# jpe17/TwoTowerMLRetrieval

Hardware: AMD Instinct MI355X
Metric: queries/sec top-k over 10M x 256-d docs (higher is better)
Workload: dtype f32 results (bit-identical to the fp32 FMA chain); f16-MFMA screen + fp32 rescoring; 1 GPU; exact cosine top-10 of B=1024 queries over 10000000 x 256 fp32 unit-norm passages resident in HBM (BASELINE configs[3]; configs[1] batch), row-sharded over 1 GPU(s), screened path (f16-MFMA filter + exact fp32 rescoring, bit-identical to the fp32 kernel); n_docs=10000000, dim=256, batch=1024, k=10, parallelism=rowshard1

## Files before the change

### include/tt.h

```cpp
#ifndef TT_H
#define TT_H

#include <stddef.h>
#include <stdint.h>

#ifdef __cplusplus
extern "C" {
#endif

typedef void *tt_stream_t;

#define TT_TOPK_INVALID_INDEX (1ll << 62)

enum tt_status {
    TT_OK = 0,
    TT_ERR_BAD_SHAPE = 1,
    TT_ERR_BAD_INDEX = 2,
    TT_ERR_ZERO_LENGTH = 3,
    TT_ERR_UNSUPPORTED = 4,
    TT_ERR_WORKSPACE = 5,
    TT_ERR_HIP = 6
};

const char *tt_version(void);
const char *tt_last_error(void);

int tt_event_create(void **ev);
int tt_event_destroy(void *ev);
int tt_event_elapsed_ms(void *start, void *stop, float *ms);


size_t tt_score_topk_redo_flags_offset(int B, int64_t N, int d, int k);
size_t tt_score_topk_pace_timeouts_offset(int B, int64_t N, int d, int k);
size_t tt_score_topk_workspace_bytes(int B, int64_t N, int d, int k);
int tt_score_topk_f32(const float *Q, int B, int d, const float *D, int64_t N, int k,
                      int64_t idx_offset, float *out_val, int64_t *out_idx, void *workspace,
                      size_t workspace_bytes, tt_stream_t stream);

size_t tt_score_topk_bf16_workspace_bytes(int B, int64_t N, int d, int k);
int tt_score_topk_bf16(const float *Q, int B, int d, const void *D_bf16, int64_t N, int k,
                       int64_t idx_offset, float *out_val, int64_t *out_idx, void *workspace,
                       size_t workspace_bytes, tt_stream_t stream);

#define TT_TOPK_LARGE_KMAX 1024
size_t tt_score_topk_large_workspace_bytes(int B, int64_t N, int d, int k, int bf16);
size_t tt_score_topk_large_tier_offset(int B, int64_t N, int d, int k, int bf16);
int tt_score_topk_large_f32(const float *Q, int B, int d, const float *D, int64_t N, int k,
                            int64_t idx_offset, float *out_val, int64_t *out_idx, void *workspace,
                            size_t workspace_bytes, tt_stream_t stream);
int tt_score_topk_large_bf16(const float *Q, int B, int d, const void *D_bf16, int64_t N, int k,
                             int64_t idx_offset, float *out_val, int64_t *out_idx, void *workspace,
                             size_t workspace_bytes, tt_stream_t stream);

size_t tt_score_topk_masked_workspace_bytes(int B, int64_t N, int d, int k, int bf16);
int tt_score_topk_masked_f32(const float *Q, int B, int d, const float *D, int64_t N, const uint32_t *keep, int k,
                             int64_t idx_offset, float *out_val, int64_t *out_idx, void *workspace,
                             size_t workspace_bytes, tt_stream_t stream);
int tt_score_topk_masked_bf16(const float *Q, int B, int d, const void *D_bf16, int64_t N, const uint32_t *keep, int k,
                              int64_t idx_offset, float *out_val, int64_t *out_idx, void *workspace,
                              size_t workspace_bytes, tt_stream_t stream);
int tt_keep_mask_pack(const uint8_t *keep_bool, int64_t N, uint32_t *keep, tt_stream_t stream);
int tt_keep_mask_clear_ids(uint32_t *keep, int64_t N, const int64_t *ids, int64_t n_ids, int64_t idx_offset,
                           tt_stream_t stream);

size_t tt_score_topk_tagged_workspace_bytes(int B, int64_t N, int d, int k, int bf16);
int tt_score_topk_tagged_f32(const float *Q, int B, int d, const float *D, int64_t N, const uint32_t *tags,
                             const uint32_t *match_mask, const uint32_t *match_value, const uint32_t *keep, int k,
                             int64_t idx_offset, float *out_val, int64_t *out_idx, void *workspace, size_t workspace_bytes,
                             tt_stream_t stream);
int tt_score_topk_tagged_bf16(const float *Q, int B, int d, const void *D_bf16, int64_t N, const uint32_t *tags,
                              const uint32_t *match_mask, const uint32_t *match_value, const uint32_t *keep, int k,
                              int64_t idx_offset, float *out_val, int64_t *out_idx, void *workspace, size_t workspace_bytes,
                              tt_stream_t stream);

size_t tt_score_topk_biased_workspace_bytes(int B, int64_t N, int d, int k, int bf16);
int tt_score_topk_biased_f32(const float *Q, int B, int d, const float *D, int64_t N, const float *bias, const uint32_t *keep,
                             int k, int64_t idx_offset, float *out_val, int64_t *out_idx, void *workspace,
                             size_t workspace_bytes, tt_stream_t stream);
int tt_score_topk_biased_bf16(const float *Q, int B, int d, const void *D_bf16, int64_t N, const float *bias,
                              const uint32_t *keep, int k, int64_t idx_offset, float *out_val, int64_t *out_idx, void *workspace,
                              size_t workspace_bytes, tt_stream_t stream);

size_t tt_score_topk_after_workspace_bytes(int B, int64_t N, int d, int k, int bf16);
int tt_score_topk_after_f32(const float *Q, int B, int d, const float *D, int64_t N, const float *after_val,
                            const int64_t *after_idx, const uint32_t *keep, int k, int64_t idx_offset, float *out_val,
                            int64_t *out_idx, void *workspace, size_t workspace_bytes, tt_stream_t stream);
int tt_score_topk_after_bf16(const float *Q, int B, int d, const void *D_bf16, int64_t N, const float *after_val,
                             const int64_t *after_idx, const uint32_t *keep, int k, int64_t idx_offset, float *out_val,
                             int64_t *out_idx, void *workspace, size_t workspace_bytes, tt_stream_t stream);
int tt_after_local_bound(int64_t after_idx, int64_t idx_offset, int N);

size_t tt_score_topk_screened_bf16_workspace_bytes(int B, int64_t N, int d, int k);
int tt_index_stats_bf16(const void *D_bf16, int64_t N, int d, float *stats, int reset_stats, tt_stream_t stream);
int tt_score_topk_screened_bf16(const float *Q, int B, int d, const void *D_bf16, int64_t N, int k, float dmax_norm,
                                int64_t idx_offset, float *out_val, int64_t *out_idx, int32_t *fallback_flag,
                                void *workspace, size_t workspace_bytes, void *const *prof_events, tt_stream_t stream);
int tt_score_topk_screened_seed_list_bf16(const float *Q, int B, int d, const void *D_bf16, int64_t N, int k, int k_seed,
                                          float dmax_norm, int32_t *fallback_flag, float *seed_list, void *workspace,
                                          size_t workspace_bytes, tt_stream_t stream);
int tt_score_topk_screened_seeded_bf16(const float *Q, int B, int d, const void *D_bf16, int64_t N, int k, float dmax_norm,
                                       int64_t idx_offset, float *out_val, int64_t *out_idx, int32_t *fallback_flag,
                                       const float *seed, void *workspace, size_t workspace_bytes,
                                       void *const *prof_events, tt_stream_t stream);

int tt_score_topk_partials_f32(const float *Q, int B, int d, const float *D, int64_t N, int k,
                               int64_t idx_offset, void *workspace, size_t workspace_bytes,
                               const float **part_val , const int64_t **part_idx ,
                               int *part_m , void *const *prof_events ,
                               tt_stream_t stream);

int tt_index_build_f16(const float *D, int64_t N, int d, void *D16, float *stats, tt_stream_t stream);
int tt_index_build_from_bf16(const void *D_bf16, int64_t N, int d, float *D32, void *D16, float *stats,
                             int reset_stats, tt_stream_t stream);
size_t tt_score_topk_screened_workspace_bytes(int B, int64_t N, int d, int k);
size_t tt_score_topk_screened_stats_offset(int B, int64_t N, int d, int k);
int tt_score_topk_screened_f32(const float *Q, int B, int d, const float *D32, const void *D16, int64_t N, int k,
                               float dmax_norm, int64_t idx_offset, float *out_val, int64_t *out_idx,
                               int32_t *fallback_flag, void *workspace, size_t workspace_bytes,
                               void *const *prof_events , tt_stream_t stream);

int tt_score_topk_screened_seed_f32(const float *Q, int B, int d, const void *D16, int64_t N, int k, int k_seed, float dmax_norm,
                                    int32_t *fallback_flag, float *seed , void *workspace, size_t workspace_bytes,
                                    tt_stream_t stream);
int tt_score_topk_screened_seed_list_f32(const float *Q, int B, int d, const void *D16, int64_t N, int k, int k_seed,
                                         float dmax_norm, int32_t *fallback_flag, float *seed_list ,
                                         void *workspace, size_t workspace_bytes, tt_stream_t stream);
int tt_seed_union_f32(const float *lists , int world, int B, int list_len, int kth,
                      float *seed , tt_stream_t stream);
int tt_score_topk_screened_seeded_f32(const float *Q, int B, int d, const float *D32, const void *D16, int64_t N, int k,
                                      float dmax_norm, int64_t idx_offset, float *out_val, int64_t *out_idx,
                                      int32_t *fallback_flag, const float *seed , void *workspace, size_t workspace_bytes,
                                      void *const *prof_events , tt_stream_t stream);

size_t tt_score_topk_screened_masked_workspace_bytes(int B, int64_t N, int d, int k, int bf16);
int tt_score_topk_screened_masked_f32(const float *Q, int B, int d, const float *D32, const void *D16, int64_t N,
                                      const uint32_t *keep, int k, float dmax_norm, int64_t idx_offset, float *out_val,
                                      int64_t *out_idx, int32_t *fallback_flag, void *workspace, size_t workspace_bytes,
                                      void *const *prof_events , tt_stream_t stream);
int tt_score_topk_screened_masked_bf16(const float *Q, int B, int d, const void *D_bf16, int64_t N, const uint32_t *keep,
                                       int k, float dmax_norm, int64_t idx_offset, float *out_val, int64_t *out_idx,
                                       int32_t *fallback_flag, void *workspace, size_t workspace_bytes,
                                       void *const *prof_events , tt_stream_t stream);
int tt_score_topk_screened_seed_list_masked_f32(const float *Q, int B, int d, const void *D16, int64_t N, const uint32_t *keep,
                                                int k, int k_seed, float dmax_norm, int32_t *fallback_flag,
                                                float *seed_list , void *workspace, size_t workspace_bytes,
                                                tt_stream_t stream);
int tt_score_topk_screened_seed_list_masked_bf16(const float *Q, int B, int d, const void *D_bf16, int64_t N,
                                                 const uint32_t *keep, int k, int k_seed, float dmax_norm,
                                                 int32_t *fallback_flag, float *seed_list , void *workspace,
                                                 size_t workspace_bytes, tt_stream_t stream);
int tt_score_topk_screened_seeded_masked_f32(const float *Q, int B, int d, const float *D32, const void *D16, int64_t N,
                                             const uint32_t *keep, int k, float dmax_norm, int64_t idx_offset, float *out_val,
                                             int64_t *out_idx, int32_t *fallback_flag, const float *seed ,
                                             void *workspace, size_t workspace_bytes,
                                             void *const *prof_events , tt_stream_t stream);
int tt_score_topk_screened_seeded_masked_bf16(const float *Q, int B, int d, const void *D_bf16, int64_t N,
                                              const uint32_t *keep, int k, float dmax_norm, int64_t idx_offset, float *out_val,
                                              int64_t *out_idx, int32_t *fallback_flag, const float *seed ,
                                              void *workspace, size_t workspace_bytes,
                                              void *const *prof_events , tt_stream_t stream);

int tt_topk_merge(const float *in_val, const int64_t *in_idx, int B, int M, int k, float *out_val,
                  int64_t *out_idx, tt_stream_t stream);

int tt_topk_merge_shards(const void *gathered, int world, size_t rank_stride, size_t idx_byte_offset,
                         int B, int kp, int k, float *out_val, int64_t *out_idx, tt_stream_t stream);

int tt_topk_merge_large(const float *in_val, const int64_t *in_idx, int B, int M, int k,
                        float *out_val, int64_t *out_idx, tt_stream_t stream);
int tt_topk_merge_shards_large(const void *gathered, int world, size_t rank_stride, size_t idx_byte_offset,
                               int B, int kp, int k, float *out_val, int64_t *out_idx, tt_stream_t stream);

int tt_topk_exclude_ids(const float *in_val, const int64_t *in_idx, int B, int M, const int64_t *exclude , int E,
                        int k, float *out_val, int64_t *out_idx, tt_stream_t stream);

int tt_topk_collapse_table(const float *in_val, const int64_t *in_idx, int B, int M, const int64_t *groups , int64_t N,
                           int64_t idx_offset, int max_per_group, int k, float *out_val, int64_t *out_idx, int64_t *out_gid,
                           int32_t *out_info , tt_stream_t stream);
int tt_topk_collapse_gids(const float *in_val, const int64_t *in_idx, const int64_t *in_gid , int B, int M,
                          int max_per_group, int k, float *out_val, int64_t *out_idx, int64_t *out_gid,
                          int32_t *out_info , tt_stream_t stream);

size_t tt_score_count_workspace_bytes(int B, int64_t N, int d, int bf16);
int tt_score_count_f32(const float *Q, int B, int d, const float *D, int64_t N, const uint32_t *keep,
                       const float *min_score, int64_t *count, int accumulate, void *workspace, size_t workspace_bytes,
                       tt_stream_t stream);
int tt_score_count_bf16(const float *Q, int B, int d, const void *D_bf16, int64_t N, const uint32_t *keep,
                        const float *min_score, int64_t *count, int accumulate, void *workspace, size_t workspace_bytes,
                        tt_stream_t stream);
int tt_topk_cut_below(float *val, int64_t *idx, int B, int k, const float *min_score, tt_stream_t stream);

int tt_score_rank_f32(const float *Q, int B, int d, const float *D, int64_t N, const int64_t *target,
                      int64_t *rank, tt_stream_t stream);

int tt_score_all_f32(const float *Q, int B, int d, const float *D, int64_t N, float *S, tt_stream_t stream);

int tt_score_ids_f32(const float *Q, int B, int d, const float *D, int64_t N, const uint32_t *keep ,
                     const int64_t *ids , int C, int64_t idx_offset, float *out_val ,
                     int64_t *out_idx , tt_stream_t stream);
int tt_score_ids_bf16(const float *Q, int B, int d, const void *D_bf16, int64_t N, const uint32_t *keep ,
                      const int64_t *ids , int C, int64_t idx_offset, float *out_val ,
                      int64_t *out_idx , tt_stream_t stream);

int tt_mmr_select_f32(const float *in_val , const int64_t *in_idx , int B, int C, const float *D, int64_t N,
                      int d, int64_t idx_offset, float lambda, int k, float *out_val , int64_t *out_idx ,
                      int32_t *out_pos , tt_stream_t stream);
int tt_mmr_select_bf16(const float *in_val , const int64_t *in_idx , int B, int C, const void *D_bf16,
                       int64_t N, int d, int64_t idx_offset, float lambda, int k, float *out_val ,
                       int64_t *out_idx , int32_t *out_pos , tt_stream_t stream);
int tt_mmr_select_rows_f32(const float *in_val , const int64_t *in_idx , int B, int C,
                           const float *rows , int d, float lambda, int k, float *out_val ,
                           int64_t *out_idx , int32_t *out_pos , tt_stream_t stream);

#define TT_LEXICAL_FMAX 20480
int tt_lexical_chunk_docs(void);
size_t tt_lexical_workspace_bytes(int B, int64_t N, int k);
int tt_lexical_score_topk_f32(const int64_t *indptr, const int32_t *cols, const float *vals, int64_t N, int F,
                              const int64_t *q_indptr, const int32_t *q_cols, const float *q_vals, int B,
                              const uint32_t *keep , const float *min_score ,
                              const float *base , int64_t base_stride, float w_base,
                              float w_lex, int k, int64_t idx_offset, float *out_val, int64_t *out_idx, void *workspace,
                              size_t workspace_bytes, tt_stream_t stream);
int tt_lexical_score_all_f32(const int64_t *indptr, const int32_t *cols, const float *vals, int64_t N, int F,
                             const int64_t *q_indptr, const int32_t *q_cols, const float *q_vals, int B, float *S ,
                             tt_stream_t stream);


typedef struct tt_enc_sync {
    void *wait_before_recurrence;
    void *record_after_recurrence;
} tt_enc_sync_t;

#define TT_ENC_TRAIN_MASK 0xff
#define TT_ENC_ONE_WORKGROUP 0x100
#define TT_ENC_PHASE_BEGIN 0x200
#define TT_ENC_PHASE_FINISH 0x400
#define TT_ENC_SEED_ON_DEVICE 0x800
#define TT_ENC_F32 0x1000
int tt_encoder_split_workgroups(int B, int H, int bidirectional, int rnn_type);
size_t tt_encoder_workspace_bytes(int B, int T, int E, int H, int num_layers, int bidirectional, int rnn_type,
                                  int train ,
                                  int dropout );
int tt_encoder_forward_f32(const int64_t *ids, int B, int T, const float *table, int64_t V, int E, int H,
                           int num_layers, int bidirectional, int rnn_type, const float *const *weights ,
                           const float *proj_w, const float *proj_b, int normalize, int train, float dropout_p,
                           uint64_t dropout_seed, float *out, void *workspace, size_t workspace_bytes,
                           int32_t *status, const tt_enc_sync_t *sync , tt_stream_t stream);

size_t tt_encoder_prepared_bytes(int E, int H, int num_layers, int bidirectional, int rnn_type);
int tt_encoder_prepare_f32(int E, int H, int num_layers, int bidirectional, int rnn_type,
                           const float *const *weights , void *prepared, size_t prepared_bytes,
                           tt_stream_t stream);
int tt_encoder_forward_prepared_f32(const int64_t *ids, int B, int T, const float *table, int64_t V, int E, int H,
                                    int num_layers, int bidirectional, int rnn_type,
                                    const float *const *weights , const void *prepared,
                                    const float *proj_w, const float *proj_b, int normalize, int opts, float *out,
                                    void *workspace, size_t workspace_bytes, int32_t *status, tt_stream_t stream);

#define TT_ENC_PROJECTED 0x2000
size_t tt_encoder_projected_bytes(int64_t V, int E, int H, int bidirectional, int rnn_type);
int tt_encoder_project_table_f32(const float *table, int64_t V, int E, int H, int num_layers, int bidirectional, int rnn_type,
                                 const float *const *weights , const void *prepared, void *projected,
                                 size_t projected_bytes, tt_stream_t stream);
int tt_encoder_forward_projected_f32(const int64_t *ids, int B, int T, const void *projected, int64_t V, int E, int H,
                                     int num_layers, int bidirectional, int rnn_type, const float *const *weights ,
                                     const void *prepared, const float *proj_w, const float *proj_b, int normalize, int opts,
                                     float *out, void *workspace, size_t workspace_bytes, int32_t *status, tt_stream_t stream);

int tt_concat_ids_i64(const int64_t *a, int Ba, int Ta, const int64_t *b, int Bb, int Tb, int64_t *out, int T,
                      tt_stream_t stream);

int tt_encoder_backward_f32(const int64_t *ids, int B, int T, const float *table, int64_t V, int E, int H,
// ... 82 lines not shown
```

### include/tt_debug.h

```cpp
#ifndef TT_DEBUG_H
#define TT_DEBUG_H

#include "tt.h"

#ifdef __cplusplus
extern "C" {
#endif

size_t tt_debug_screen_s16_workspace_bytes(int B, int64_t N, int form);
int tt_debug_screen_s16(const float *Q, int B, const void *D16, int64_t N, float dmax_norm, const float *thr, int form,
                        float *out_t, void *workspace, size_t workspace_bytes, tt_stream_t stream);

int tt_debug_screen_s16_bf16(const float *Q, int B, const void *D_bf16, int64_t N, float dmax_norm, const float *thr, int form,
                             float *out_t, void *workspace, size_t workspace_bytes, tt_stream_t stream);

#ifdef __cplusplus
}
#endif
#endif
```

### twotowermlretrieval_amd/_lib.py

```python
from __future__ import annotations

import ctypes as C
from pathlib import Path

_PKG = Path(__file__).resolve().parent
LIB_PATH = _PKG / "libtt.so"

TT_OK, TT_ERR_BAD_SHAPE, TT_ERR_BAD_INDEX, TT_ERR_ZERO_LENGTH, TT_ERR_UNSUPPORTED, TT_ERR_WORKSPACE, TT_ERR_HIP = range(7)
TT_ENC_ONE_WORKGROUP = 0x100
TT_ENC_PHASE_BEGIN, TT_ENC_PHASE_FINISH = 0x200, 0x400
TT_ENC_SEED_ON_DEVICE = 0x800
TT_ENC_F32 = 0x1000
TT_ENC_PROJECTED = 0x2000
TT_STEP_GATE_WORDS = 4


class EncSync(C.Structure):
    _fields_ = [("wait_before_recurrence", C.c_void_p), ("record_after_recurrence", C.c_void_p)]
TT_TOPK_INVALID_INDEX = 1 << 62


class TTError(RuntimeError):
    def __init__(self, code: int, msg: str):
        super().__init__(f"libtt error {code}: {msg}")
        self.code = code


_vp, _i, _i64, _sz, _f, _u64 = C.c_void_p, C.c_int, C.c_int64, C.c_size_t, C.c_float, C.c_uint64

SIGNATURES = {
    "tt_version": (C.c_char_p, []),
    "tt_last_error": (C.c_char_p, []),
    "tt_score_topk_workspace_bytes": (_sz, [_i, _i64, _i, _i]),
    "tt_score_topk_pace_timeouts_offset": (_sz, [_i, _i64, _i, _i]),
    "tt_score_topk_redo_flags_offset": (_sz, [_i, _i64, _i, _i]),
    "tt_score_topk_f32": (_i, [_vp, _i, _i, _vp, _i64, _i, _i64, _vp, _vp, _vp, _sz, _vp]),
    "tt_score_topk_bf16_workspace_bytes": (_sz, [_i, _i64, _i, _i]),
    "tt_score_topk_bf16": (_i, [_vp, _i, _i, _vp, _i64, _i, _i64, _vp, _vp, _vp, _sz, _vp]),
    "tt_score_topk_large_workspace_bytes": (_sz, [_i, _i64, _i, _i, _i]),
    "tt_score_topk_large_tier_offset": (_sz, [_i, _i64, _i, _i, _i]),
    "tt_score_topk_large_f32": (_i, [_vp, _i, _i, _vp, _i64, _i, _i64, _vp, _vp, _vp, _sz, _vp]),
    "tt_score_topk_large_bf16": (_i, [_vp, _i, _i, _vp, _i64, _i, _i64, _vp, _vp, _vp, _sz, _vp]),
    "tt_score_topk_masked_workspace_bytes": (_sz, [_i, _i64, _i, _i, _i]),
    "tt_score_topk_masked_f32": (_i, [_vp, _i, _i, _vp, _i64, _vp, _i, _i64, _vp, _vp, _vp, _sz, _vp]),
    "tt_score_topk_masked_bf16": (_i, [_vp, _i, _i, _vp, _i64, _vp, _i, _i64, _vp, _vp, _vp, _sz, _vp]),
    "tt_keep_mask_pack": (_i, [_vp, _i64, _vp, _vp]),
    "tt_keep_mask_clear_ids": (_i, [_vp, _i64, _vp, _i64, _i64, _vp]),
    "tt_score_topk_tagged_workspace_bytes": (_sz, [_i, _i64, _i, _i, _i]),
    "tt_score_topk_tagged_f32": (_i, [_vp, _i, _i, _vp, _i64, _vp, _vp, _vp, _vp, _i, _i64, _vp, _vp, _vp, _sz, _vp]),
    "tt_score_topk_tagged_bf16": (_i, [_vp, _i, _i, _vp, _i64, _vp, _vp, _vp, _vp, _i, _i64, _vp, _vp, _vp, _sz, _vp]),
    "tt_score_topk_biased_workspace_bytes": (_sz, [_i, _i64, _i, _i, _i]),
    "tt_score_topk_biased_f32": (_i, [_vp, _i, _i, _vp, _i64, _vp, _vp, _i, _i64, _vp, _vp, _vp, _sz, _vp]),
    "tt_score_topk_biased_bf16": (_i, [_vp, _i, _i, _vp, _i64, _vp, _vp, _i, _i64, _vp, _vp, _vp, _sz, _vp]),
    "tt_score_topk_after_workspace_bytes": (_sz, [_i, _i64, _i, _i, _i]),
    "tt_score_topk_after_f32": (_i, [_vp, _i, _i, _vp, _i64, _vp, _vp, _vp, _i, _i64, _vp, _vp, _vp, _sz, _vp]),
    "tt_score_topk_after_bf16": (_i, [_vp, _i, _i, _vp, _i64, _vp, _vp, _vp, _i, _i64, _vp, _vp, _vp, _sz, _vp]),
    "tt_after_local_bound": (_i, [_i64, _i64, _i]),
    "tt_score_topk_screened_bf16_workspace_bytes": (_sz, [_i, _i64, _i, _i]),
    "tt_index_stats_bf16": (_i, [_vp, _i64, _i, _vp, _i, _vp]),
    "tt_score_topk_screened_bf16": (_i, [_vp, _i, _i, _vp, _i64, _i, _f, _i64, _vp, _vp, _vp, _vp, _sz, _vp, _vp]),
    "tt_score_topk_screened_seed_list_bf16": (_i, [_vp, _i, _i, _vp, _i64, _i, _i, _f, _vp, _vp, _vp, _sz, _vp]),
    "tt_score_topk_screened_seeded_bf16": (_i, [_vp, _i, _i, _vp, _i64, _i, _f, _i64, _vp, _vp, _vp, _vp, _vp, _sz, _vp, _vp]),
    "tt_score_topk_partials_f32": (_i, [_vp, _i, _i, _vp, _i64, _i, _i64, _vp, _sz, _vp, _vp, _vp, _vp, _vp]),
    "tt_index_build_f16": (_i, [_vp, _i64, _i, _vp, _vp, _vp]),
    "tt_index_build_from_bf16": (_i, [_vp, _i64, _i, _vp, _vp, _vp, _i, _vp]),
    "tt_score_topk_screened_workspace_bytes": (_sz, [_i, _i64, _i, _i]),
    "tt_score_topk_screened_stats_offset": (_sz, [_i, _i64, _i, _i]),
    "tt_score_topk_screened_seed_f32": (_i, [_vp, _i, _i, _vp, _i64, _i, _i, _f, _vp, _vp, _vp, _sz, _vp]),
    "tt_score_topk_screened_seed_list_f32": (_i, [_vp, _i, _i, _vp, _i64, _i, _i, _f, _vp, _vp, _vp, _sz, _vp]),
    "tt_seed_union_f32": (_i, [_vp, _i, _i, _i, _i, _vp, _vp]),
    "tt_score_topk_screened_seeded_f32": (_i, [_vp, _i, _i, _vp, _vp, _i64, _i, _f, _i64, _vp, _vp, _vp, _vp, _vp, _sz, _vp, _vp]),
    "tt_score_topk_screened_f32": (_i, [_vp, _i, _i, _vp, _vp, _i64, _i, _f, _i64, _vp, _vp, _vp, _vp, _sz, _vp, _vp]),
    "tt_score_topk_screened_masked_workspace_bytes": (_sz, [_i, _i64, _i, _i, _i]),
    "tt_score_topk_screened_masked_f32": (_i, [_vp, _i, _i, _vp, _vp, _i64, _vp, _i, _f, _i64, _vp, _vp, _vp, _vp, _sz, _vp, _vp]),
    "tt_score_topk_screened_masked_bf16": (_i, [_vp, _i, _i, _vp, _i64, _vp, _i, _f, _i64, _vp, _vp, _vp, _vp, _sz, _vp, _vp]),
    "tt_score_topk_screened_seed_list_masked_f32": (_i, [_vp, _i, _i, _vp, _i64, _vp, _i, _i, _f, _vp, _vp, _vp, _sz, _vp]),
    "tt_score_topk_screened_seed_list_masked_bf16": (_i, [_vp, _i, _i, _vp, _i64, _vp, _i, _i, _f, _vp, _vp, _vp, _sz, _vp]),
    "tt_score_topk_screened_seeded_masked_f32": (_i, [_vp, _i, _i, _vp, _vp, _i64, _vp, _i, _f, _i64, _vp, _vp, _vp, _vp, _vp, _sz, _vp, _vp]),
    "tt_score_topk_screened_seeded_masked_bf16": (_i, [_vp, _i, _i, _vp, _i64, _vp, _i, _f, _i64, _vp, _vp, _vp, _vp, _vp, _sz, _vp, _vp]),
    "tt_event_create": (_i, [_vp]),
    "tt_event_destroy": (_i, [_vp]),
    "tt_event_elapsed_ms": (_i, [_vp, _vp, _vp]),
    "tt_topk_merge": (_i, [_vp, _vp, _i, _i, _i, _vp, _vp, _vp]),
    "tt_topk_merge_shards": (_i, [_vp, _i, _sz, _sz, _i, _i, _i, _vp, _vp, _vp]),
    "tt_topk_merge_large": (_i, [_vp, _vp, _i, _i, _i, _vp, _vp, _vp]),
    "tt_topk_merge_shards_large": (_i, [_vp, _i, _sz, _sz, _i, _i, _i, _vp, _vp, _vp]),
    "tt_topk_exclude_ids": (_i, [_vp, _vp, _i, _i, _vp, _i, _i, _vp, _vp, _vp]),
    "tt_topk_collapse_table": (_i, [_vp, _vp, _i, _i, _vp, _i64, _i64, _i, _i, _vp, _vp, _vp, _vp, _vp]),
    "tt_topk_collapse_gids": (_i, [_vp, _vp, _vp, _i, _i, _i, _i, _vp, _vp, _vp, _vp, _vp]),
    "tt_score_count_workspace_bytes": (_sz, [_i, _i64, _i, _i]),
    "tt_score_count_f32": (_i, [_vp, _i, _i, _vp, _i64, _vp, _vp, _vp, _i, _vp, _sz, _vp]),
    "tt_score_count_bf16": (_i, [_vp, _i, _i, _vp, _i64, _vp, _vp, _vp, _i, _vp, _sz, _vp]),
    "tt_topk_cut_below": (_i, [_vp, _vp, _i, _i, _vp, _vp]),
    "tt_score_rank_f32": (_i, [_vp, _i, _i, _vp, _i64, _vp, _vp, _vp]),
    "tt_score_all_f32": (_i, [_vp, _i, _i, _vp, _i64, _vp, _vp]),
    "tt_score_ids_f32": (_i, [_vp, _i, _i, _vp, _i64, _vp, _vp, _i, _i64, _vp, _vp, _vp]),
    "tt_score_ids_bf16": (_i, [_vp, _i, _i, _vp, _i64, _vp, _vp, _i, _i64, _vp, _vp, _vp]),
    "tt_mmr_select_f32": (_i, [_vp, _vp, _i, _i, _vp, _i64, _i, _i64, _f, _i, _vp, _vp, _vp, _vp]),
    "tt_mmr_select_bf16": (_i, [_vp, _vp, _i, _i, _vp, _i64, _i, _i64, _f, _i, _vp, _vp, _vp, _vp]),
    "tt_mmr_select_rows_f32": (_i, [_vp, _vp, _i, _i, _vp, _i, _f, _i, _vp, _vp, _vp, _vp]),
    "tt_lexical_chunk_docs": (_i, []),
    "tt_lexical_workspace_bytes": (_sz, [_i, _i64, _i]),
    "tt_lexical_score_topk_f32": (_i, [_vp, _vp, _vp, _i64, _i, _vp, _vp, _vp, _i, _vp, _vp, _vp, _i64, _f, _f, _i, _i64,
                                       _vp, _vp, _vp, _sz, _vp]),
    "tt_lexical_score_all_f32": (_i, [_vp, _vp, _vp, _i64, _i, _vp, _vp, _vp, _i, _vp, _vp]),
    "tt_tok_create": (_i, [_vp, _vp, _vp, _i64, _i64, _vp]),
    "tt_tok_destroy": (None, [_vp]),
    "tt_tok_encode": (_i, [_vp, _vp, _vp, _i64, _vp, _vp, _vp, _i]),
    "tt_tok_encode_sep": (_i, [_vp, _vp, _i64, C.c_char, _i64, _vp, _vp, _vp, _vp, _i]),
    "tt_tok_encode_ptrs": (_i, [_vp, _vp, _vp, _i64, _vp, _vp, _vp, _vp, _i]),
    "tt_tok_set_unicode": (_i, [_vp, _vp, _vp, _i64]),
    "tt_tok_encode_units": (_i, [_vp, _vp, _vp, _vp, _i64, _vp, _vp, _vp, _vp, _i]),
    "tt_tok_pad": (_i, [_vp, _vp, _vp, _i64, _i64, _vp, _i]),
    "tt_tok_pad_i32": (_i, [_vp, _vp, _vp, _i64, _i64, _vp, _i]),
    "tt_encoder_split_workgroups": (_i, [_i, _i, _i, _i]),
    "tt_encoder_workspace_bytes": (_sz, [_i, _i, _i, _i, _i, _i, _i, _i, _i]),
    "tt_encoder_forward_f32": (_i, [_vp, _i, _i, _vp, _i64, _i, _i, _i, _i, _i, _vp, _vp, _vp, _i, _i, _f, _u64, _vp, _vp,
                                    _sz, _vp, _vp, _vp]),
    "tt_concat_ids_i64": (_i, [_vp, _i, _i, _vp, _i, _i, _vp, _i, _vp]),
    "tt_encoder_prepared_bytes": (_sz, [_i, _i, _i, _i, _i]),
    "tt_encoder_prepare_f32": (_i, [_i, _i, _i, _i, _i, _vp, _vp, _sz, _vp]),
    "tt_encoder_forward_prepared_f32": (_i, [_vp, _i, _i, _vp, _i64, _i, _i, _i, _i, _i, _vp, _vp, _vp, _vp, _i, _i, _vp, _vp,
                                             _sz, _vp, _vp]),
    "tt_encoder_projected_bytes": (_sz, [_i64, _i, _i, _i, _i]),
    "tt_encoder_project_table_f32": (_i, [_vp, _i64, _i, _i, _i, _i, _i, _vp, _vp, _vp, _sz, _vp]),
    "tt_encoder_forward_projected_f32": (_i, [_vp, _i, _i, _vp, _i64, _i, _i, _i, _i, _i, _vp, _vp, _vp, _vp, _i, _i, _vp, _vp,
                                              _sz, _vp, _vp]),
    "tt_encoder_backward_f32": (_i, [_vp, _i, _i, _vp, _i64, _i, _i, _i, _i, _i, _vp, _vp, _vp, _i, _f, _u64, _vp, _vp,
                                     _vp, _vp, _vp, _vp, _sz, _i, _vp, _vp, _vp]),
    "tt_triplet_loss_f32": (_i, [_vp, _vp, _vp, _i, _i, _f, _vp, _vp, _vp, _vp, _vp, _vp]),
    "tt_in_batch_loss_workspace_bytes": (_sz, [_i, _i]),
    "tt_in_batch_loss_f32": (_i, [_vp, _vp, _vp, _i, _i, _f, _vp, _vp, _vp, _vp, _vp, _sz, _vp]),
    "tt_contrastive_loss_workspace_bytes": (_sz, [_i, _i, _i]),
    "tt_contrastive_loss_f32": (_i, [_vp, _i, _vp, _i, _i, _i, _f, _vp, _vp, _vp, _vp, _sz, _vp]),
    "tt_contrastive_loss_grouped_f32": (_i, [_vp, _i, _vp, _i, _i, _i, _vp, _vp, _f, _vp, _vp, _vp, _vp, _sz, _vp]),
    "tt_contrastive_loss_soft_workspace_bytes": (_sz, [_i, _i, _i]),
    "tt_contrastive_loss_soft_f32": (_i, [_vp, _i, _vp, _i, _i, _vp, _f, _vp, _vp, _vp, _vp, _sz, _vp]),
    "tt_contrastive_loss_sym_workspace_bytes": (_sz, [_i, _i, _i]),
    "tt_contrastive_loss_sym_f32": (_i, [_vp, _i, _vp, _i, _i, _i, _vp, _vp, _f, _f, _vp, _vp, _vp, _vp, _vp, _sz, _vp]),
    "tt_allgather_topk":(_i, [_vp, _vp, _vp, _sz, _vp]),
    "tt_allreduce_grads": (_i, [_vp, _vp, _i64, _vp]),
    "tt_comm_library": (C.c_char_p, []),
    "tt_comm_unique_id": (_i, [_vp]),
    "tt_comm_init_rank": (_i, [_vp, _i, _vp, _i]),
    "tt_comm_info": (_i, [_vp, _vp, _vp]),
    "tt_comm_destroy": (_i, [_vp]),
    "tt_clip_adam_scratch_bytes": (_sz, []),
    "tt_clip_adam_step_f32": (_i, [_vp, _vp, _vp, _vp, _i64, _i64, _f, _f, _f, _f, _f, _f, _vp, _vp, _vp]),
    "tt_clip_adam_step_gated_f32": (_i, [_vp, _vp, _vp, _vp, _i64, _vp, _f, _f, _f, _f, _f, _f, _vp, _vp, _vp, _vp]),
    "tt_step_gate_f32": (_i, [_vp, _i, _vp, _vp]),
}

_lib = None


def lib() -> C.CDLL:
    global _lib
    if _lib is None:
        if not LIB_PATH.exists():
            raise ImportError(
                f"{LIB_PATH} is missing: build it with `python -m twotowermlretrieval_amd.build` "
                "(hipcc, gfx950).  There is no CPU or PyTorch fallback for this path.")
        l = C.CDLL(str(LIB_PATH))
        for name, (res, args) in SIGNATURES.items():
            fn = getattr(l, name)
            fn.restype = res
            fn.argtypes = args
        _lib = l
    return _lib


def check(rc: int) -> None:
    if rc != TT_OK:
        msg = lib().tt_last_error().decode("utf-8", "replace")
        if rc == TT_ERR_BAD_INDEX:
            raise IndexError(msg)
        if rc == TT_ERR_BAD_SHAPE:
            raise ValueError(msg)
        raise TTError(rc, msg)
```

### twotowermlretrieval_amd/csrc/screen.hip

```cpp
#include "score_topk.h"
#include "keep_word.h"
#include <cmath>

#include <hip/hip_fp16.h>
#include <limits.h>
#include <math.h>

namespace {

typedef _Float16 h8 __attribute__((ext_vector_type(8)));
typedef _Float16 h4 __attribute__((ext_vector_type(4)));
typedef unsigned u32x4 __attribute__((ext_vector_type(4)));
typedef __attribute__((address_space(3))) void lds_void;
typedef const __attribute__((address_space(1))) void gbl_void;

#ifndef TT_SCREEN_STAGGER
#define TT_SCREEN_STAGGER 1
#endif
constexpr int SW = 8;
constexpr int STILE_BYTES = 32 * 512;
constexpr int SRING = 8;
constexpr int STPB = 2;
constexpr int SCAP = 128;
constexpr int SURV_MAX = 1024;
constexpr int POOL_MAX = 8192;
constexpr int FIN_MAX_CHUNKS = 2048;
constexpr int STOP = 2;
constexpr int STOP_MIN_CHUNKS = 64;
constexpr int REFRESH_LEVELS = 16;
constexpr int REFRESH_STEP = 2;
constexpr int REFRESH_FIRST_SHIFT = 5;
constexpr int REFRESH_MIN_TILES = 1024;

struct SCand {
    float v;
    int x;
};

__device__ __forceinline__ float screen_eps(float qnorm, float dmax)
{
    return 1.10e-3f * qnorm * dmax + 1e-6f * (qnorm + dmax);
}

template <int NCH>
__device__ __forceinline__ void bf16_to_f16_lds(char *base, int lane)
{
    uint4 v[NCH];
#pragma unroll
    for (int i = 0; i < NCH; ++i)
        v[i] = *(const uint4 *)(base + (i * 64 + lane) * 16);
#pragma unroll
    for (int i = 0; i < NCH; ++i) {
        unsigned w[4] = {v[i].x, v[i].y, v[i].z, v[i].w};
#pragma unroll
        for (int e = 0; e < 4; ++e) {
            const _Float16 lo = (_Float16)__uint_as_float(w[e] << 16);
            const _Float16 hi = (_Float16)__uint_as_float(w[e] & 0xffff0000u);
            w[e] = (unsigned)__builtin_bit_cast(unsigned short, lo) | ((unsigned)__builtin_bit_cast(unsigned short, hi) << 16);
        }
        *(uint4 *)(base + (i * 64 + lane) * 16) = uint4{w[0], w[1], w[2], w[3]};
    }
}

__device__ __forceinline__ SCand scand_load_l2(const SCand *p)
{
    unsigned long long u = __hip_atomic_load((const unsigned long long *)p, __ATOMIC_RELAXED, __HIP_MEMORY_SCOPE_AGENT);
    SCand c;
    c.v = __uint_as_float((unsigned)u);
    c.x = (int)(u >> 32);
    return c;
}

struct ScreenParams {
    const float *Q = nullptr;
    const _Float16 *D16 = nullptr;
    int B = 0, N = 0, k = 0;
    int n_chunks = 0, tiles_per_chunk = 0, n_tiles = 0;
    int static_tiles = 0, tail_g = 1, tail_blocks = 0;
    int *tail_ctr = nullptr;
    unsigned *hist = nullptr;
    float dmax = 0.0f;
    SCand *cand = nullptr;
    int *pcnt = nullptr;
    int *flag = nullptr;
    float *max_val = nullptr;
    float *top_val = nullptr;
    const float *thr0 = nullptr;
    int thr0_stride = 1;
    const h8 *qimg = nullptr;
    const float *qnorm = nullptr;
    const float *dbg_thr = nullptr;
    const unsigned *keep = nullptr;
};

__device__ __forceinline__ void scand_store_async(const SCand *base, unsigned byte_off, float v, int x)
{
    const unsigned long long bits = ((unsigned long long)(unsigned)x << 32) | (unsigned long long)__float_as_uint(v);
    asm volatile("global_store_dwordx2 %0, %1, %2\n\ts_nop 1" ::"v"(byte_off), "v"(bits), "s"(base) : "memory");
}

__device__ __forceinline__ void u32_inc_async(const unsigned *base, unsigned byte_off)
{
    asm volatile("global_atomic_add %0, %1, %2\n\ts_nop 0" ::"v"(byte_off), "v"(1u), "s"(base) : "memory");
}

__device__ __forceinline__ float refresh_edge(int j, float width, float base) { return __fmaf_rn((float)j - 0.25f, width, base); }
__device__ __forceinline__ int refresh_level(float v, float base, float inv_width)
{
    return (int)fminf((v - base) * inv_width, (float)(REFRESH_LEVELS - 1));
}
constexpr float REFRESH_MIN_WIDTH = 1e-30f;

__device__ __forceinline__ void f32_store_async(float *dst, float v)
{
    asm volatile("global_store_dword %0, %1, off\n\ts_nop 0" ::"v"(dst), "v"(v) : "memory");
}

constexpr int SQUART = SCAP / 4;
constexpr int SQ_TRIGGER = SQUART - 10;
constexpr int SQ_KEEP_MAX = 4 * SQ_TRIGGER - 4;

__device__ __forceinline__ void screen_compact(SCand *base, const int (&n)[4], int k, float slack, int lane, int &n_new,
                                               float &thr_new, bool &have, bool &overflow)
{
    float v[2];
    int x[2], rank[2];
    bool live[2];
#pragma unroll
    for (int i = 0; i < 2; ++i) {
        v[i] = -INFINITY;
        x[i] = INT_MAX;
        rank[i] = 0;
        live[i] = (lane & 31) < ((lane >> 5) ? n[2 * i + 1] : n[2 * i]);
        if (live[i]) {
            const SCand c = scand_load_l2(base + 64 * i + lane);
            v[i] = c.v;
            x[i] = c.x;
        }
    }
#pragma unroll
    for (int i2 = 0; i2 < 2; ++i2) {
#pragma unroll
        for (int sub = 0; sub < 2; ++sub) {
            const int lim = n[2 * i2 + sub];
            for (int l2 = 0; l2 < lim; ++l2) {
                const float sv = __builtin_bit_cast(float, __builtin_amdgcn_readlane(__builtin_bit_cast(int, v[i2]), 32 * sub + l2));
                const int sx = __builtin_amdgcn_readlane(x[i2], 32 * sub + l2);
#pragma unroll
                for (int i = 0; i < 2; ++i)
                    rank[i] += (sv > v[i] || (sv == v[i] && sx < x[i])) ? 1 : 0;
            }
        }
    }
    const int total = n[0] + n[1] + n[2] + n[3];
    have = total >= k;
    overflow = false;
    n_new = total;
    thr_new = -INFINITY;
    if (have) {
        float kth = -INFINITY;
#pragma unroll
        for (int i = 0; i < 2; ++i) {
            const unsigned long long bk = __ballot(live[i] && rank[i] == k - 1);
            if (bk)
                kth = __builtin_bit_cast(float, __builtin_amdgcn_readlane(__builtin_bit_cast(int, v[i]), __ffsll((long long)bk) - 1));
        }
        thr_new = kth - slack;
        n_new = 0;
#pragma unroll
        for (int i = 0; i < 2; ++i)
            n_new += __popcll(__ballot(live[i] && v[i] >= thr_new));
        if (n_new > SQ_KEEP_MAX) {
            overflow = true;
            n_new = k;
        }
    }
#pragma unroll
    for (int i = 0; i < 2; ++i)
        if (live[i] && rank[i] < n_new) {
            SCand c;
            c.v = v[i];
            c.x = x[i];
            base[SQUART * (rank[i] & 3) + (rank[i] >> 2)] = c;
        }
}

__global__ __launch_bounds__(128) void q_image_kernel(const float *__restrict__ Q, int B, h8 *__restrict__ img,
                                                      float *__restrict__ qnorm, int *__restrict__ flag, int n_flags,
                                                      int *__restrict__ tail_ctr, int n_ctr, unsigned *__restrict__ hist)
{
    __shared__ int any_bad[2];
    if (blockIdx.x == 0)
        for (int i = threadIdx.x; i < n_ctr; i += 128)
            tail_ctr[i] = 0;
    if (hist)
        for (int i = threadIdx.x; i < 32 * REFRESH_LEVELS; i += 128)
            hist[(size_t)blockIdx.x * (32 * REFRESH_LEVELS) + i] = 0u;
    const int lane = threadIdx.x & 63, wv = threadIdx.x >> 6;
    const int S = blockIdx.x * 2 + wv;
    const int g = lane >> 4, n = lane & 15;
    const int qrow = 16 * S + n;
    const bool live = qrow < B;
    const float *qp = Q + (size_t)min(qrow, B - 1) * 256 + 8 * g;
    float ss = 0.0f;
    bool bad = false;
#pragma unroll
    for (int s = 0; s < 8; ++s) {
        const f32x4 a = *(const f32x4 *)(qp + 32 * s);
        const f32x4 b = *(const f32x4 *)(qp + 32 * s + 4);
        h8 hv;
#pragma unroll
        for (int e = 0; e < 4; ++e) {
            const float x0 = live ? a[e] : 0.0f, x1 = live ? b[e] : 0.0f;
            ss += x0 * x0 + x1 * x1;
            bad |= !(fabsf(x0) <= 60000.0f) || !(fabsf(x1) <= 60000.0f);
            hv[e] = (_Float16)x0;
            hv[4 + e] = (_Float16)x1;
        }
        img[((size_t)S * 8 + s) * 64 + lane] = hv;
    }
    ss += __shfl_xor(ss, 16);
    ss += __shfl_xor(ss, 32);
    if (g == 0)
        qnorm[qrow] = sqrtf(ss);
    const bool wave_bad = __ballot(bad && live) != 0ull;
    if (lane == 0)
        any_bad[wv] = wave_bad ? 1 : 0;
    __syncthreads();
    if (threadIdx.x == 0 && (int)blockIdx.x < n_flags)
        flag[blockIdx.x] = (any_bad[0] | any_bad[1]) ? 2 : 0;
}

template <bool MAXONLY, int NSET, bool BF = false, bool MASKED = false, bool ONCHIP = false>
__global__ __launch_bounds__(SW * 64, 2) void screen_kernel(ScreenParams p)
{
    extern __shared__ __attribute__((aligned(16))) char ring[];
    constexpr int DMA_AUX = NSET < 3 ? 2 : 0;
    const int lane = threadIdx.x & 63;
    const int w = __builtin_amdgcn_readfirstlane(threadIdx.x >> 6);
    const int chunk = blockIdx.x % p.n_chunks;
    const int qgroup = blockIdx.x / p.n_chunks;
    int t0 = chunk * p.tiles_per_chunk;
    int t1 = min(t0 + p.tiles_per_chunk, p.static_tiles);
    __shared__ int next_block;
    const int k = p.k;
    const int g = lane >> 4, n = lane & 15;
    constexpr int QW = 16 * NSET, QB = SW * QW;
    const int qbase = qgroup * QB + w * QW;
    const bool wave_live = qbase < p.B;
    __shared__ float ladder_base[SW * 64];
    const bool refresh = !MAXONLY && p.hist != nullptr;
    const unsigned *const hwave = p.hist + (size_t)qbase * REFRESH_LEVELS;

    h8 qreg[NSET][8];
    float eps2[NSET];
    f32x4 negthr[NSET];
    int cnt[NSET];
#pragma unroll
    for (int c = 0; c < NSET; ++c)
        cnt[c] = 0;
#pragma unroll
    for (int c = 0; c < NSET; ++c) {
        const int qrow = qbase + 16 * c + n;
        const bool live = qrow < p.B;
        float qn = 0.0f;
        if (wave_live) {
            const h8 *src = p.qimg + ((size_t)(qbase / 16 + c) * 8) * 64 + lane;
#pragma unroll
            for (int s = 0; s < 8; ++s)
                qreg[c][s] = src[s * 64];
            qn = p.qnorm[qrow];
        }
        eps2[c] = 2.0f * screen_eps(qn, p.dmax);
        const float floor_thr = -(1.01f * qn * p.dmax + 1e-30f);
        const float t_init = live ? ((!MAXONLY && p.thr0) ? fmaxf(p.thr0[(size_t)qrow * p.thr0_stride + p.thr0_stride - 1] - eps2[c], floor_thr)
                                                    : floor_thr)
                            : INFINITY;
        float c_init = -t_init;
        if (MAXONLY)
            c_init = (p.dbg_thr && live) ? -p.dbg_thr[qrow] : 0.0f;
        negthr[c] = f32x4{c_init, c_init, c_init, c_init};
        if (!MAXONLY && g == 0)
            ladder_base[w * QW + 16 * c + n] = t_init + eps2[c];
    }

    SCand *const cwave = p.cand + ((size_t)blockIdx.x * QB + w * QW) * SCAP;

    auto compact_where = [&](int c, unsigned qmask) {
        asm volatile("s_waitcnt vmcnt(0)" ::: "memory");
        while (qmask) {
            const int q = __ffs((int)qmask) - 1;
            qmask &= qmask - 1;
            const int nq[4] = {__builtin_amdgcn_readlane(cnt[c], q), __builtin_amdgcn_readlane(cnt[c], q + 16),
                               __builtin_amdgcn_readlane(cnt[c], q + 32), __builtin_amdgcn_readlane(cnt[c], q + 48)};
            const float slack = __builtin_bit_cast(float, __builtin_amdgcn_readlane(__builtin_bit_cast(int, eps2[c]), q));
            int n_new;
            float tn;
            bool have, ovf;
            screen_compact(cwave + (size_t)(16 * c + q) * SCAP, nq, k, slack, lane, n_new, tn, have, ovf);
            if (ovf && lane == 0)
                atomicOr(p.flag + ((qbase + 16 * c) >> 5), 1);
            if (n == q) {
                cnt[c] = (n_new - g + 3) >> 2;
                if (have) {
                    const float nt = fminf(negthr[c][0], -tn);
                    negthr[c] = f32x4{nt, nt, nt, nt};
                }
            }
        }
    };

    auto refresh_thresholds = [&]() {
        asm volatile("s_waitcnt vmcnt(0)" ::: "memory");
        int ln = lane;
        asm volatile("" : "+v"(ln));
        const int n = ln & 15, g = ln >> 4;
#pragma unroll
        for (int c = 0; c < NSET; ++c) {
            const unsigned *hp = hwave + (unsigned)((16 * c + n) * REFRESH_LEVELS + 4 * g);
            int sfx[4];
            int run = 0;
#pragma unroll
            for (int i = 3; i >= 0; --i) {
                run += (int)__hip_atomic_load(hp + i, __ATOMIC_RELAXED, __HIP_MEMORY_SCOPE_AGENT);
                sfx[i] = run;
            }
            const int x16 = (ln ^ 16) << 2, x32 = (ln ^ 32) << 2;
            const int t16 = __builtin_amdgcn_ds_bpermute(x16, run), t32 = __builtin_amdgcn_ds_bpermute(x32, run),
                      t48 = __builtin_amdgcn_ds_bpermute(x32, t16);
            const int above = ((g ^ 1) > g ? t16 : 0) + ((g ^ 2) > g ? t32 : 0) + ((g ^ 3) > g ? t48 : 0);
            int jtop = -1;
#pragma unroll
            for (int i = 0; i < 4; ++i)
                if (above + sfx[i] >= k)
                    jtop = 4 * g + i;
            jtop = max(jtop, __builtin_amdgcn_ds_bpermute(x16, jtop));
            jtop = max(jtop, __builtin_amdgcn_ds_bpermute(x32, jtop));
            if (jtop > 0) {
                const float base = ladder_base[w * QW + 16 * c + n];
                float le = eps2[c];
                asm volatile("" : "+v"(le));
                const float nt = fminf(negthr[c][0], le - refresh_edge(jtop, (float)REFRESH_STEP * le, base));
                negthr[c] = f32x4{nt, nt, nt, nt};
            }
            __builtin_amdgcn_sched_barrier(0);
        }
    };

    const char *D = (const char *)p.D16;
    const char *rowp[2];
    auto set_rows = [&](int tile) {
#pragma unroll
        for (int i = 0; i < 2; ++i) {
            const int row = 2 * (2 * w + i) + (lane >> 5);
            const int doc = min(tile * 32 + row, p.N - 1);
            const int chunk16 = (lane & 31) ^ (row & 15);
            rowp[i] = D + (size_t)doc * 512 + chunk16 * 16;
        }
    };
    auto dma_issue = [&](int tile, int stage) {
        set_rows(min(tile, t1 - 1));
        char *dst = ring + stage * STILE_BYTES + (2 * w) * 1024;
        __builtin_amdgcn_global_load_lds((gbl_void *)rowp[0], (lds_void *)dst, 16, 0, DMA_AUX);
        __builtin_amdgcn_global_load_lds((gbl_void *)rowp[1], (lds_void *)(dst + 1024), 16, 0, DMA_AUX);
    };
    auto dma_piece = [&](int i, int stage) {
        char *dst = ring + stage * STILE_BYTES + (2 * w + i) * 1024;
        __builtin_amdgcn_global_load_lds((gbl_void *)rowp[i], (lds_void *)dst, 16, 0, DMA_AUX);
    };

    float top[ONCHIP ? NSET : 1][STOP];
#pragma unroll
    for (int c = 0; c < (ONCHIP ? NSET : 1); ++c)
#pragma unroll
        for (int j = 0; j < STOP; ++j)
            top[c][j] = -INFINITY;

    for (;;) {
    if (t0 < t1) {
#pragma unroll
        for (int gi = 0; gi < SRING - STPB; ++gi)
            dma_issue(t0 + gi, gi);
        int stage = 0;
        const int rd_base = n * 512;
        f32x4 acc[2][NSET];
        const bool late = TT_SCREEN_STAGGER && w >= 4;
        bool pending = false;
        int ptile = 0;
        unsigned pkw = 0xffffffffu;
        auto epilogue = [&](int tile, unsigned kw) {
                const int tile_base = tile * 32;
            const bool partial = tile_base + 32 > p.N;
            const bool holes = MASKED && kw != 0xffffffffu;
            const unsigned kwg = MASKED ? kw >> (4 * g) : 0xffffffffu;
            auto dropped = [&](int u, int r) {
                return tile_base + 16 * u + 4 * g + r >= p.N || (MASKED && ((kwg >> (16 * u + r)) & 1u) == 0u);
            };
            if (!MAXONLY) {
                if (partial || holes) {
#pragma unroll
                    for (int u = 0; u < 2; ++u)
#pragma unroll
                        for (int r = 0; r < 4; ++r)
                            if (dropped(u, r)) {
#pragma unroll
                                for (int c = 0; c < NSET; ++c)
                                    acc[u][c][r] = -INFINITY;
                            }
                }
                int mall = INT_MIN;
#pragma unroll
                for (int u = 0; u < 2; ++u)
#pragma unroll
                    for (int c = 0; c < NSET; ++c)
#pragma unroll
                        for (int r = 0; r < 4; ++r)
                            mall = max(mall, __float_as_int(acc[u][c][r]));
                if (__ballot(mall >= 0) != 0ull) {
#pragma unroll
                    for (int c = 0; c < NSET; ++c) {
                        int mu[2];
#pragma unroll
                        for (int u = 0; u < 2; ++u)
                            mu[u] = max(max(__float_as_int(acc[u][c][0]), __float_as_int(acc[u][c][1])),
                                        max(__float_as_int(acc[u][c][2]), __float_as_int(acc[u][c][3])));
                        if (__ballot(max(mu[0], mu[1]) >= 0) == 0ull)
                            continue;
                        const unsigned mine = (unsigned)(((16 * c + n) * SCAP + SQUART * g) * sizeof(SCand));
                        const float thr_c = -negthr[c][0];
#pragma unroll
                        for (int u = 0; u < 2; ++u) {
                            if (__ballot(mu[u] >= 0) == 0ull)
                                continue;
// ... 55 lines not shown
                            t = hi;
                        }
                        continue;
                    }
                    m = fmaxf(m, __shfl_xor(m, 16));
                    m = fmaxf(m, __shfl_xor(m, 32));
                    const int qrow = qbase + 16 * c + n;
                    if (g == 0 && qrow < p.B)
                        f32_store_async(p.max_val + (size_t)qrow * p.n_tiles + tile, m);
                }
            }
                };
        int cp_shift = refresh && t0 < p.static_tiles ? REFRESH_FIRST_SHIFT : 0;
        int tile = t0;
        for (;;) {
        int tend = t1;
        while (cp_shift > 0) {
            const int cp = t0 + (((t1 - t0) >> cp_shift) & ~(STPB - 1));
            --cp_shift;
            if (cp > tile) {
                tend = cp;
                break;
            }
        }
        for (; tile < tend; ++tile) {
            if ((tile - t0) % STPB == 0) {
                asm volatile("s_waitcnt vmcnt(%0)" ::"n"(2 * (SRING - 2 * STPB)) : "memory");
                if (BF && tile == t0) {
#pragma unroll
                    for (int i = 0; i < STPB; ++i)
                        bf16_to_f16_lds<2>(ring + ((stage + i) % SRING) * STILE_BYTES + (2 * w) * 1024, lane);
                    asm volatile("s_waitcnt lgkmcnt(0)" ::: "memory");
                }
                __builtin_amdgcn_s_barrier();
            } else if (BF && (tile - t0) % STPB == STPB - 1) {
                asm volatile("s_waitcnt vmcnt(%0)" ::"n"(2 * (SRING - 3 * STPB + 1)) : "memory");
#pragma unroll
                for (int i = 1; i <= STPB; ++i)
                    bf16_to_f16_lds<2>(ring + ((stage + i) % SRING) * STILE_BYTES + (2 * w) * 1024, lane);
                asm volatile("s_waitcnt lgkmcnt(0)" ::: "memory");
            }
            const int fill_stage = (stage + SRING - STPB) % SRING;
            set_rows(min(tile + SRING - STPB, t1 - 1));
            if (!wave_live) {
                dma_piece(0, fill_stage);
                dma_piece(1, fill_stage);
            }
            if (wave_live) {
                if (late && pending)
                    epilogue(ptile, pkw);
                const char *buf = ring + stage * STILE_BYTES + rd_base;
                h8 a0[3], a1[3];
                auto a_read = [&](int s) {
                    const int off = ((4 * s + g) ^ n) << 4;
                    a0[s % 3] = *(const h8 *)(buf + off);
                    a1[s % 3] = *(const h8 *)(buf + 16 * 512 + off);
                };
                a_read(0);
                a_read(1);
                unsigned kw = 0xffffffffu;
#pragma unroll
                for (int s = 0; s < 8; ++s) {
                    if (s + 2 < 8)
                        a_read(s + 2);
                    if (MASKED && s == 0)
                        keep_word_issue(p.keep + __builtin_amdgcn_readfirstlane(tile), kw, a0[0]);
                    if (s == 2)
                        dma_piece(0, fill_stage);
                    if (s == 6)
                        dma_piece(1, fill_stage);
                    __builtin_amdgcn_sched_barrier(0);
#pragma unroll
                    for (int c = 0; c < NSET; ++c) {
                        const f32x4 c0 = s == 0 ? negthr[c] : acc[0][c];
                        const f32x4 c1 = s == 0 ? negthr[c] : acc[1][c];
                        acc[0][c] = __builtin_amdgcn_mfma_f32_16x16x32_f16(a0[s % 3], qreg[c][s], c0, 0, 0, 0);
                        acc[1][c] = __builtin_amdgcn_mfma_f32_16x16x32_f16(a1[s % 3], qreg[c][s], c1, 0, 0, 0);
                    }
                    __builtin_amdgcn_sched_barrier(0);
                }
                if (MASKED)
                    keep_word_wait(kw, acc[1][NSET - 1]);
                if (late) {
                    pending = true;
                    ptile = tile;
                    pkw = kw;
                } else {
                    epilogue(tile, kw);
                }
            }
            stage = (stage + 1) % SRING;
        }
        if (wave_live && late && pending) {
            epilogue(ptile, pkw);
            pending = false;
        }
        if (tend == t1)
            break;
        if (wave_live)
            refresh_thresholds();
        }
    }
    if (MAXONLY || p.tail_blocks == 0)
        break;
    asm volatile("s_waitcnt vmcnt(0)" ::: "memory");
    __builtin_amdgcn_s_barrier();
    if (refresh && wave_live)
        refresh_thresholds();
    if (threadIdx.x == 0)
        next_block = atomicAdd(p.tail_ctr + qgroup, 1);
    __syncthreads();
    const int blk = next_block;
    if (blk >= p.tail_blocks)
        break;
    t0 = p.static_tiles + blk * p.tail_g;
    t1 = min(t0 + p.tail_g, p.n_tiles);
    }
    asm volatile("s_waitcnt vmcnt(0)" ::: "memory");
    __builtin_amdgcn_s_barrier();

    if (MAXONLY) {
        if (ONCHIP) {
#pragma unroll
            for (int c = 0; c < NSET; ++c) {
                const int qrow = qbase + 16 * c + n;
                if (qrow < p.B) {
                    float *dst = p.top_val + ((size_t)qrow * p.n_chunks + chunk) * (4 * STOP) + g * STOP;
#pragma unroll
                    for (int j = 0; j < STOP; ++j)
                        dst[j] = top[ONCHIP ? c : 0][j];
                }
            }
        }
        return;
    }
    int nf = n;
    asm volatile("" : "+v"(nf));
#pragma unroll
    for (int c = 0; c < NSET; ++c) {
        int tot = cnt[c] + __shfl_xor(cnt[c], 16);
        tot += __shfl_xor(tot, 32);
        const unsigned long long over = __ballot(tot > k) & 0xffffull;
        if (over)
            compact_where(c, (unsigned)over);
        int packed = cnt[c] << (8 * g);
        packed |= __shfl_xor(packed, 16);
        packed |= __shfl_xor(packed, 32);
        const int qrow = qbase + 16 * c + nf;
        if (g == 0 && qrow < p.B)
            p.pcnt[(size_t)qrow * p.n_chunks + chunk] = packed;
    }
}

constexpr int TW = 4;
constexpr int TSLAB_BYTES = 32 * 128;
constexpr int TSTAGE = 4;
constexpr int TDMA = 4;
constexpr int TSTREAM_AUX = 2;

template <bool MAXONLY, int NQS = 2, bool BF = false, bool MASKED = false>
__global__ __launch_bounds__(TW * 64, 2) void screen_stream_kernel(ScreenParams p)
{
    constexpr int QPT = 16 * NQS;
    extern __shared__ __attribute__((aligned(16))) char ring_all[];
    const int lane = threadIdx.x & 63;
    const int w = __builtin_amdgcn_readfirstlane(threadIdx.x >> 6);
    char *const ring = ring_all + w * (TSTAGE * TSLAB_BYTES);
    const int task = blockIdx.x * TW + w;
    const int n_qtiles = (p.B + QPT - 1) / QPT;
    if (task >= n_qtiles * p.n_chunks)
        return;
    const int qtile = task / p.n_chunks, chunk = task % p.n_chunks;
    const int t0 = chunk * p.tiles_per_chunk;
    const int t1 = min(t0 + p.tiles_per_chunk, p.n_tiles);
    const int k = p.k;
    const int g = lane >> 4, n = lane & 15;
    const int qbase = qtile * QPT;

    h8 qreg[NQS][8];
    float eps2[NQS];
    f32x4 negthr[NQS];
    int cnt[NQS];
#pragma unroll
    for (int c = 0; c < NQS; ++c) {
        cnt[c] = 0;
        const int qrow = qbase + 16 * c + n;
        const bool live = qrow < p.B;
        const h8 *src = p.qimg + ((size_t)(qbase / 16 + c) * 8) * 64 + lane;
#pragma unroll
        for (int s = 0; s < 8; ++s)
            qreg[c][s] = src[s * 64];
        const float qn = p.qnorm[qrow];
        eps2[c] = 2.0f * screen_eps(qn, p.dmax);
        const float floor_thr = -(1.01f * qn * p.dmax + 1e-30f);
        const float t_init = live ? ((!MAXONLY && p.thr0) ? fmaxf(p.thr0[(size_t)qrow * p.thr0_stride + p.thr0_stride - 1] - eps2[c], floor_thr)
                                                    : floor_thr)
                            : INFINITY;
        float c_init = -t_init;
        if (MAXONLY)
            c_init = (p.dbg_thr && live) ? -p.dbg_thr[qrow] : 0.0f;
        negthr[c] = f32x4{c_init, c_init, c_init, c_init};
    }

    SCand *const cwave = p.cand + (size_t)task * QPT * SCAP;

    auto compact_where = [&](int c, unsigned qmask) {
        asm volatile("s_waitcnt vmcnt(0)" ::: "memory");
        while (qmask) {
            const int q = __ffs((int)qmask) - 1;
            qmask &= qmask - 1;
            const int nq[4] = {__builtin_amdgcn_readlane(cnt[c], q), __builtin_amdgcn_readlane(cnt[c], q + 16),
                               __builtin_amdgcn_readlane(cnt[c], q + 32), __builtin_amdgcn_readlane(cnt[c], q + 48)};
            const float slack = __builtin_bit_cast(float, __builtin_amdgcn_readlane(__builtin_bit_cast(int, eps2[c]), q));
            int n_new;
            float tn;
            bool have, ovf;
            screen_compact(cwave + (size_t)(16 * c + q) * SCAP, nq, k, slack, lane, n_new, tn, have, ovf);
            if (ovf && lane == 0)
                atomicOr(p.flag + ((qbase + 16 * c) >> 5), 1);
            if (n == q) {
                cnt[c] = (n_new - g + 3) >> 2;
                if (have)
                    negthr[c] = f32x4{-tn, -tn, -tn, -tn};
            }
        }
    };

    const char *D = (const char *)p.D16;
    int dma_tile = t0, dma_kq = 0;
    const char *rowp[TDMA];
    auto set_rows = [&](int tile) {
#pragma unroll
        for (int jj = 0; jj < TDMA; ++jj) {
            const int row = 8 * jj + (lane >> 3);
            const int doc = min(tile * 32 + row, p.N - 1);
            rowp[jj] = D + (size_t)doc * 512 + (((lane & 7) ^ (row & 7)) << 4);
        }
    };
    auto dma_issue = [&](int stage) {
        char *dst = ring + stage * TSLAB_BYTES;
#pragma unroll
        for (int jj = 0; jj < TDMA; ++jj)
            __builtin_amdgcn_global_load_lds((gbl_void *)(rowp[jj] + dma_kq * 128), (lds_void *)(dst + jj * 1024), 16, 0, TSTREAM_AUX);
        if (++dma_kq == 4) {
            dma_kq = 0;
            dma_tile = min(dma_tile + 1, t1 - 1);
            set_rows(dma_tile);
        }
    };

    if (t0 < t1) {
        set_rows(t0);
#pragma unroll
        for (int i = 0; i < TSTAGE - 1; ++i)
            dma_issue(i);
        int stage = 0;
        const char *rd_row = ring + n * 128;
        const int rsw = n & 7;
        for (int tile = t0; tile < t1; ++tile) {
            f32x4 acc[2][NQS];
            unsigned kw = 0xffffffffu;
#pragma unroll
            for (int kq = 0; kq < 4; ++kq) {
                asm volatile("s_waitcnt vmcnt(%0)" ::"n"(TDMA * (TSTAGE - 2)) : "memory");
                if (BF) {
                    bf16_to_f16_lds<TSLAB_BYTES / 1024>(ring + stage * TSLAB_BYTES, lane);
                    asm volatile("s_waitcnt lgkmcnt(0)" ::: "memory");
                }
                const char *buf = rd_row + stage * TSLAB_BYTES;
                h8 a[2][2];
#pragma unroll
                for (int s2 = 0; s2 < 2; ++s2)
#pragma unroll
                    for (int u = 0; u < 2; ++u)
                        a[u][s2] = *(const h8 *)(buf + u * 2048 + (((4 * s2 + g) ^ rsw) << 4));
                asm volatile("s_waitcnt lgkmcnt(0)" ::: "memory");
                if (MASKED && kq == 3)
                    keep_word_issue(p.keep + tile, kw, a[0][0]);
                dma_issue((stage + TSTAGE - 1) % TSTAGE);
#pragma unroll
                for (int s2 = 0; s2 < 2; ++s2)
#pragma unroll
                    for (int c = 0; c < NQS; ++c)
#pragma unroll
                        for (int u = 0; u < 2; ++u) {
                            const f32x4 cin = (kq == 0 && s2 == 0) ? negthr[c] : acc[u][c];
                            acc[u][c] = __builtin_amdgcn_mfma_f32_16x16x32_f16(a[u][s2], qreg[c][2 * kq + s2], cin, 0, 0, 0);
                        }
                stage = (stage + 1) % TSTAGE;
            }
            const int tile_base = tile * 32;
            const bool partial = tile_base + 32 > p.N;
            if (MASKED)
                keep_word_wait(kw, acc[1][NQS - 1]);
            const bool holes = MASKED && kw != 0xffffffffu;
            const unsigned kwg = MASKED ? kw >> (4 * g) : 0xffffffffu;
            auto dropped = [&](int u, int r) {
                return tile_base + 16 * u + 4 * g + r >= p.N || (MASKED && ((kwg >> (16 * u + r)) & 1u) == 0u);
            };
            if (!MAXONLY) {
                if (MASKED && kw == 0u)
                    continue;
                if (partial || holes) {
#pragma unroll
                    for (int u = 0; u < 2; ++u)
#pragma unroll
// ... 259 lines not shown
    for (int sidx = tid; sidx < ns; sidx += 256) {
        float acc = 0.0f;
        if (p.Dbf) {
            const unsigned *brow = p.Dbf + (size_t)sv_x[sidx] * 128;
#pragma unroll 1
            for (int x0 = 0; x0 < 256; x0 += 64) {
                u32x4 dv[8];
#pragma unroll
                for (int i = 0; i < 8; ++i)
                    dv[i] = __builtin_nontemporal_load((const u32x4 *)(brow + x0 / 2 + 4 * i));
#pragma unroll
                for (int i = 0; i < 8; ++i) {
                    const unsigned wv[4] = {dv[i].x, dv[i].y, dv[i].z, dv[i].w};
#pragma unroll
                    for (int e = 0; e < 4; ++e) {
                        acc = fmaf(qs[x0 + 8 * i + 2 * e], __uint_as_float(wv[e] << 16), acc);
                        acc = fmaf(qs[x0 + 8 * i + 2 * e + 1], __uint_as_float(wv[e] & 0xffff0000u), acc);
                    }
                }
            }
            sv_v[sidx] = acc;
            continue;
        }
        const float *drow = p.D32 + (size_t)sv_x[sidx] * 256;
#pragma unroll 1
        for (int x0 = 0; x0 < 256; x0 += 64) {
            f32x4 dv[16];
#pragma unroll
            for (int i = 0; i < 16; ++i)
                dv[i] = __builtin_nontemporal_load((const f32x4 *)(drow + x0 + 4 * i));
#pragma unroll
            for (int i = 0; i < 16; ++i) {
                acc = fmaf(qs[x0 + 4 * i], dv[i].x, acc);
                acc = fmaf(qs[x0 + 4 * i + 1], dv[i].y, acc);
                acc = fmaf(qs[x0 + 4 * i + 2], dv[i].z, acc);
                acc = fmaf(qs[x0 + 4 * i + 3], dv[i].w, acc);
            }
        }
        sv_v[sidx] = acc;
    }
    if (tid == 0) {
        p.stats[2 * row] = n_pool;
        p.stats[2 * row + 1] = n_surv;
    }
    if (__syncthreads_or(too_many) && tid == 0)
        atomicOr(p.flag + (row >> 5), 4);
    __syncthreads();
    for (int sidx = tid; sidx < ns; sidx += 256) {
        const float mv = sv_v[sidx];
        const int mx = sv_x[sidx];
        int rank = 0;
        for (int u = 0; u < ns; ++u)
            rank += before_f(sv_v[u], sv_x[u], mv, mx) ? 1 : 0;
        if (rank < p.k) {
            p.out_val[(size_t)row * p.k + rank] = mv;
            p.out_idx[(size_t)row * p.k + rank] = p.idx_offset + mx;
        }
    }
    for (int r = ns + tid; r < p.k; r += 256) {
        p.out_val[(size_t)row * p.k + r] = -INFINITY;
        p.out_idx[(size_t)row * p.k + r] = -1;
    }
}

__global__ __launch_bounds__(256) void build_f16_kernel(const float *__restrict__ D, int64_t N, int d,
                                                        _Float16 *__restrict__ out, unsigned *__restrict__ stats)
{
    __shared__ float red[8];
    const int lane = threadIdx.x & 63, wave = threadIdx.x >> 6;
    float nmax = 0.0f, amax = 0.0f;
    for (int64_t row = (int64_t)blockIdx.x * 4 + wave; row < N; row += (int64_t)gridDim.x * 4) {
        float ss = 0.0f;
        for (int x = lane * 4; x < d; x += 256) {
            const f32x4 v = *(const f32x4 *)(D + row * d + x);
            h4 hv;
#pragma unroll
            for (int e = 0; e < 4; ++e) {
                ss += v[e] * v[e];
                amax = fmaxf(amax, fabsf(v[e]));
                if (!(fabsf(v[e]) <= 3.0e38f))
                    amax = INFINITY;
                hv[e] = (_Float16)v[e];
            }
            *(h4 *)(out + row * d + x) = hv;
        }
#pragma unroll
        for (int off = 32; off >= 1; off >>= 1)
            ss += __shfl_xor(ss, off);
        nmax = fmaxf(nmax, sqrtf(ss));
    }
#pragma unroll
    for (int off = 32; off >= 1; off >>= 1)
        amax = fmaxf(amax, __shfl_xor(amax, off));
    if (lane == 0) {
        red[wave] = nmax;
        red[4 + wave] = amax;
    }
    __syncthreads();
    if (threadIdx.x == 0) {
        atomicMax(stats, __float_as_uint(fmaxf(fmaxf(red[0], red[1]), fmaxf(red[2], red[3]))));
        atomicMax(stats + 1, __float_as_uint(fmaxf(fmaxf(red[4], red[5]), fmaxf(red[6], red[7]))));
    }
}

__global__ __launch_bounds__(256) void build_from_bf16_kernel(const unsigned short *__restrict__ S, int64_t N, int d,
                                                              float *__restrict__ out32, _Float16 *__restrict__ out16,
                                                              unsigned *__restrict__ stats)
{
    __shared__ float red[8];
    const int lane = threadIdx.x & 63, wave = threadIdx.x >> 6;
    float nmax = 0.0f, amax = 0.0f;
    for (int64_t row = (int64_t)blockIdx.x * 4 + wave; row < N; row += (int64_t)gridDim.x * 4) {
        float ss = 0.0f;
        for (int x = lane * 4; x < d; x += 256) {
            const uint2 raw = *(const uint2 *)(S + row * d + x);
            f32x4 v;
            v[0] = __uint_as_float(raw.x << 16);
            v[1] = __uint_as_float(raw.x & 0xffff0000u);
            v[2] = __uint_as_float(raw.y << 16);
            v[3] = __uint_as_float(raw.y & 0xffff0000u);
            h4 hv;
#pragma unroll
            for (int e = 0; e < 4; ++e) {
                ss += v[e] * v[e];
                amax = fmaxf(amax, fabsf(v[e]));
                if (!(fabsf(v[e]) <= 3.0e38f))
                    amax = INFINITY;
                hv[e] = (_Float16)v[e];
            }
            if (out32)
                *(f32x4 *)(out32 + row * d + x) = v;
            if (out16)
                *(h4 *)(out16 + row * d + x) = hv;
        }
#pragma unroll
        for (int off = 32; off >= 1; off >>= 1)
            ss += __shfl_xor(ss, off);
        nmax = fmaxf(nmax, sqrtf(ss));
    }
#pragma unroll
    for (int off = 32; off >= 1; off >>= 1)
        amax = fmaxf(amax, __shfl_xor(amax, off));
    if (lane == 0) {
        red[wave] = nmax;
        red[4 + wave] = amax;
    }
    __syncthreads();
    if (threadIdx.x == 0 && stats) {
        atomicMax(stats, __float_as_uint(fmaxf(fmaxf(red[0], red[1]), fmaxf(red[2], red[3]))));
        atomicMax(stats + 1, __float_as_uint(fmaxf(fmaxf(red[4], red[5]), fmaxf(red[6], red[7]))));
    }
}

struct SPlan {
    bool stream;
    int nset;
    int n_qgroups;
    int q_per_block;
    int n_tiles, n_chunks, tiles_per_chunk;
    int static_tiles, tail_g, tail_blocks;
    size_t tailctr_off;
    bool refresh;
    size_t hist_off;
    bool sample;
    int s_tiles, s_chunks, s_tiles_per_chunk;
    int64_t s_docs;
    bool s_onchip;
    int s_vals;
    size_t cand_off, pcnt_off, smax_val_off, sthr_val_off, qimg_off, qnorm_off, stats_off, ws_bytes;
    int rows_pad;
};

constexpr int64_t SAMPLE_MIN_N = 65536;
constexpr int STREAM_MAX_B = 64;

int one_round(bool stream, int n_qgroups)
{
    return stream ? (tt_device_cus() * 2 * TW + n_qgroups - 1) / n_qgroups : (tt_device_cus() + n_qgroups - 1) / n_qgroups;
}

SPlan make_splan(int B, int64_t N, int k)
{
    SPlan pl;
    pl.stream = B <= STREAM_MAX_B;
    if (B <= SW * 32) {
        pl.nset = B <= SW * 16 ? 1 : 2;
    } else {
        const int groups = (B + SW * 64 - 1) / (SW * 64);
        pl.nset = (B + groups - 1) / groups <= SW * 48 ? 3 : 4;
    }
    pl.q_per_block = pl.stream ? (B <= 32 ? 32 : 64) : SW * 16 * pl.nset;
    pl.n_qgroups = (B + pl.q_per_block - 1) / pl.q_per_block;
    pl.n_tiles = (int)((N + 31) / 32);
    int max_chunks = pl.stream && N >= SAMPLE_MIN_N ? FIN_MAX_CHUNKS : POOL_MAX / (k + 16);
    if (!pl.stream)
        max_chunks = max_chunks > 255 ? 255 : max_chunks;
    const TTChunks c = tt_chunks(pl.n_tiles, one_round(pl.stream, pl.n_qgroups), max_chunks);
    pl.n_chunks = c.n_chunks;
    const TTTailSplit t = tt_tail_split(c.tiles_per_chunk, c.n_chunks, pl.n_tiles,
                                        pl.stream ? 0 : TT_AB_SWITCH(TT_SCREEN_TAIL_DIV, 8), 16, 8, 32);
    pl.tiles_per_chunk = t.own;
    pl.static_tiles = t.static_tiles;
    pl.tail_g = t.tail_g;
    pl.tail_blocks = t.tail_blocks;
    const int n_tasks = pl.n_qgroups * pl.n_chunks;
    const size_t rows = (size_t)pl.n_qgroups * pl.q_per_block;
    pl.rows_pad = (int)rows;
    pl.sample = N >= SAMPLE_MIN_N;
    int64_t s_docs = N / 64;
    const int per_k = k <= 16 ? 4096 : 2048;
    const int64_t s_min = (int64_t)k * per_k < N / 4 ? (int64_t)k * per_k : N / 4;
    s_docs = s_docs < s_min ? s_min : s_docs;
    s_docs = s_docs < 32 ? 32 : s_docs;
    pl.s_docs = (s_docs + 31) / 32 * 32;
    pl.s_tiles = (int)(pl.s_docs / 32);
    const TTChunks sc = tt_chunks(pl.s_tiles, one_round(pl.stream, pl.n_qgroups), INT_MAX);
    pl.s_tiles_per_chunk = sc.tiles_per_chunk;
    pl.s_chunks = pl.sample ? sc.n_chunks : 0;
    const size_t cand_bytes = (size_t)n_tasks * pl.q_per_block * SCAP * sizeof(SCand);
    pl.s_onchip = pl.sample && !pl.stream && pl.s_chunks >= STOP_MIN_CHUNKS && TT_AB_SWITCH(TT_SCREEN_SAMPLE_ONCHIP, 1) != 0 &&
                  rows * (size_t)pl.s_chunks * 4 * STOP * sizeof(float) <= cand_bytes;
    pl.s_vals = pl.s_onchip ? pl.s_chunks * 4 * STOP : pl.s_tiles;
    TTWorkspace ws;
    pl.cand_off = ws.take(cand_bytes);
    pl.pcnt_off = ws.take(rows * pl.n_chunks * sizeof(int));
    pl.sthr_val_off = ws.take(rows * sizeof(float));
    pl.qimg_off = ws.take(rows * 256 * sizeof(_Float16));
    pl.qnorm_off = ws.take(rows * sizeof(float));
    pl.tailctr_off = ws.take((size_t)pl.n_qgroups * sizeof(int));
    pl.stats_off = ws.take(rows * 2 * sizeof(int));
    pl.hist_off = pl.stream ? 0 : ws.take(rows * REFRESH_LEVELS * sizeof(unsigned));
    const int refresh_min = TT_AB_SWITCH(TT_SCREEN_REFRESH_MIN_TILES, REFRESH_MIN_TILES);
    pl.refresh = !pl.stream && TT_AB_SWITCH(TT_SCREEN_THR_REFRESH, 1) != 0 && c.tiles_per_chunk >= (refresh_min < 8 ? 8 : refresh_min);
    pl.smax_val_off = pl.s_onchip ? pl.cand_off : ws.take(rows * (size_t)(pl.sample ? pl.s_tiles : 1) * sizeof(float));
    pl.ws_bytes = ws.off;
    return pl;
}

enum ScreenKind { KIND_MAIN, KIND_MAXONLY, KIND_ONCHIP };
#define SCREEN_FORMS(MAXONLY, BF, MASKED, ONCHIP)                                                                             \
    {(const void *)screen_stream_kernel<MAXONLY, 2, BF, MASKED>, (const void *)screen_stream_kernel<MAXONLY, 4, BF, MASKED>, \
     (const void *)screen_kernel<MAXONLY, 1, BF, MASKED, ONCHIP>, (const void *)screen_kernel<MAXONLY, 2, BF, MASKED, ONCHIP>, \
     (const void *)screen_kernel<MAXONLY, 3, BF, MASKED, ONCHIP>, (const void *)screen_kernel<MAXONLY, 4, BF, MASKED, ONCHIP>}
#define SCREEN_KIND(MAXONLY, ONCHIP)                                                             \
    {{SCREEN_FORMS(MAXONLY, false, false, ONCHIP), SCREEN_FORMS(MAXONLY, false, true, ONCHIP)}, \
     {SCREEN_FORMS(MAXONLY, true, false, ONCHIP), SCREEN_FORMS(MAXONLY, true, true, ONCHIP)}}
const void *const SCREEN_FN[3][2][2][6] = {SCREEN_KIND(false, false), SCREEN_KIND(true, false), SCREEN_KIND(true, true)};
#undef SCREEN_KIND
#undef SCREEN_FORMS

int launch_screen(const SPlan &pl, ScreenParams p, bool bf16, hipStream_t st)
{
    if (p.top_val && pl.stream)
        return tt_fail(TT_ERR_UNSUPPORTED, "launch_screen: top_val outside the shared-tile sample pass");
    const ScreenKind kind = p.top_val ? KIND_ONCHIP : p.max_val ? KIND_MAXONLY : KIND_MAIN;
    const void *fn = SCREEN_FN[kind][bf16][p.keep != nullptr][pl.stream ? pl.q_per_block == 64 : 1 + pl.nset];
    const int n_tasks = pl.n_qgroups * p.n_chunks;
    const size_t lds = pl.stream ? (size_t)TW * TSTAGE * TSLAB_BYTES : (size_t)SRING * STILE_BYTES;
    const int blocks = pl.stream ? (n_tasks + TW - 1) / TW : n_tasks;
    TT_HIP_CHECK(hipFuncSetAttribute(fn, hipFuncAttributeMaxDynamicSharedMemorySize, (int)lds));
    void *args[] = {&p};
    TT_HIP_CHECK(hipLaunchKernel(fn, dim3(blocks), dim3((pl.stream ? TW : SW) * 64), args, lds, st));
    return TT_OK;
}

size_t fallback_ws_bytes(int B, int64_t N, int d, int k, bool bf16)
{
    return bf16 ? tt_score_topk_bf16_workspace_bytes(B, N, d, k) : tt_score_topk_workspace_bytes(B, N, d, k);
}

size_t splan_query(int B, int64_t N, int k, size_t SPlan::*what, size_t behind)
{
    return B <= 0 || N <= 0 ? 0 : make_splan(B, N, k).*what + behind;
}

}

TT_EXPORT int tt_index_build_f16(const float *D, int64_t N, int d, void *D16, float *stats, tt_stream_t stream)
{
    if (N < 0 || d <= 0 || (d & 3))
        return tt_fail(TT_ERR_BAD_SHAPE, "tt_index_build_f16: N=%lld d=%d", (long long)N, d);
    if (!stats || (N > 0 && (!D || !D16)))
        return tt_fail(TT_ERR_BAD_SHAPE, "tt_index_build_f16: null pointer");
    hipStream_t st = (hipStream_t)stream;
    TT_RC_CHECK(tt_zero_async(stats, 2 * sizeof(float), st));
    if (N == 0)
        return TT_OK;
    const int64_t want_blocks = (N + 3) / 4;
    hipLaunchKernelGGL(build_f16_kernel, dim3((unsigned)(want_blocks > 8192 ? 8192 : want_blocks)), dim3(256), 0, st, D,
                       N, d, (_Float16 *)D16, (unsigned *)stats);
    TT_LAUNCH_CHECK();
    return TT_OK;
}

TT_EXPORT int tt_index_build_from_bf16(const void *D_bf16, int64_t N, int d, float *D32, void *D16, float *stats,
                                       int reset_stats, tt_stream_t stream)
{
    if (N < 0 || d <= 0 || (d & 3))
        return tt_fail(TT_ERR_BAD_SHAPE, "tt_index_build_from_bf16: N=%lld d=%d", (long long)N, d);
    if (N > 0 && (!D_bf16 || !D32))
        return tt_fail(TT_ERR_BAD_SHAPE, "tt_index_build_from_bf16: null pointer");
    hipStream_t st = (hipStream_t)stream;
    if (stats && reset_stats)
        TT_RC_CHECK(tt_zero_async(stats, 2 * sizeof(float), st));
    if (N == 0)
        return TT_OK;
    const int64_t want_blocks = (N + 3) / 4;
    hipLaunchKernelGGL(build_from_bf16_kernel, dim3((unsigned)(want_blocks > 8192 ? 8192 : want_blocks)), dim3(256), 0,
                       st, (const unsigned short *)D_bf16, N, d, D32, (_Float16 *)D16, (unsigned *)stats);
    TT_LAUNCH_CHECK();
    return TT_OK;
}

TT_EXPORT size_t tt_score_topk_screened_workspace_bytes(int B, int64_t N, int d, int k)
{
    return splan_query(B, N, k, &SPlan::ws_bytes, fallback_ws_bytes(B, N, d, k, false));
}

TT_EXPORT size_t tt_score_topk_screened_bf16_workspace_bytes(int B, int64_t N, int d, int k)
{
    return splan_query(B, N, k, &SPlan::ws_bytes, fallback_ws_bytes(B, N, d, k, true));
}

TT_EXPORT size_t tt_score_topk_screened_masked_workspace_bytes(int B, int64_t N, int d, int k, int bf16)
{
    return splan_query(B, N, k, &SPlan::ws_bytes, fallback_ws_bytes(B, N, d, k, bf16 != 0));
}

TT_EXPORT size_t tt_score_topk_screened_stats_offset(int B, int64_t N, int d, int k)
{
    (void)d;
    return splan_query(B, N, k, &SPlan::stats_off, 0);
}

namespace {
__global__ void seed_fill_kernel(float *seed, int n)
{
    const int i = blockIdx.x * 256 + threadIdx.x;
    if (i < n)
        seed[i] = -3.0e38f;
}

enum class Phase {
    Whole,
    SeedThreshold,
    SeedList,
    Seeded,
};

struct QueryArgs { const float *Q; int B, d, k; float dmax_norm; };
struct RowArgs {
    const void *D16;
    const void *D32;
    bool bf16;
    int64_t N;
    const unsigned *keep;
};
struct OutArgs { int64_t idx_offset; float *out_val; int64_t *out_idx; void *const *prof_events; };
struct ScratchArgs { int32_t *fallback_flag; void *workspace; size_t workspace_bytes; hipStream_t stream; };
struct ScreenedCall : QueryArgs, RowArgs, OutArgs, ScratchArgs {
    const char *who;
    Phase phase;
    int k_seed;
    float *seed;
};

RowArgs f32_rows(const float *D32, const void *D16, int64_t N, const unsigned *keep) { return {D16, D32, false, N, keep}; }
RowArgs bf16_rows(const void *D_bf16, int64_t N, const unsigned *keep) { return {D_bf16, D_bf16, true, N, keep}; }

int screened_validate(const ScreenedCall &c, SPlan *pl)
{
    const char *who = c.who;
    if (c.B <= 0 || c.N <= 0 || c.k <= 0)
        return tt_fail(TT_ERR_BAD_SHAPE, "%s: B=%d N=%lld k=%d", who, c.B, (long long)c.N, c.k);
    if (c.d != 256)
        return tt_fail(TT_ERR_UNSUPPORTED, "%s: d=%d (supported: 256)", who, c.d);
    if (c.k > 64)
        return tt_fail(TT_ERR_UNSUPPORTED, "%s: k=%d > 64", who, c.k);
    if (c.N >= (int64_t)INT_MAX - 64)
        return tt_fail(TT_ERR_UNSUPPORTED, "%s: N too large; shard the corpus", who);
    if (!(c.dmax_norm >= 0.0f) || !(c.dmax_norm < 60000.0f))
        return tt_fail(TT_ERR_UNSUPPORTED, "%s: corpus norm %g outside the fp16 range", who, c.dmax_norm);
    const bool seed_only = c.phase == Phase::SeedThreshold || c.phase == Phase::SeedList;
    if (!c.Q || !c.D16 || !c.fallback_flag || (!seed_only && (!c.D32 || !c.out_val || !c.out_idx)) ||
        (c.phase != Phase::Whole && !c.seed))
        return tt_fail(TT_ERR_BAD_SHAPE, "%s: null pointer", who);
    if (seed_only && (c.k_seed < 1 || c.k_seed > c.k))
        return tt_fail(TT_ERR_BAD_SHAPE, "%s: k_seed=%d outside [1, k=%d]", who, c.k_seed, c.k);
    if ((uintptr_t)c.keep & 3)
        return tt_fail(TT_ERR_BAD_SHAPE, "%s: keep must be 4-byte aligned", who);
    *pl = make_splan(c.B, c.N, c.k);
    const size_t need = pl->ws_bytes + fallback_ws_bytes(c.B, c.N, c.d, c.k, c.bf16);
    if (!c.workspace || c.workspace_bytes < need || ((uintptr_t)c.workspace & 255) || (c.bf16 && ((uintptr_t)c.D16 & 15)))
        return tt_fail(TT_ERR_WORKSPACE, "%s: workspace %zu < %zu bytes", who, c.workspace_bytes, need);
    return TT_OK;
}

ScreenParams screen_params(const ScreenedCall &c, const SPlan &pl)
{
    char *ws = (char *)c.workspace;
    ScreenParams sp;
    sp.Q = c.Q;
    sp.D16 = (const _Float16 *)c.D16;
    sp.B = c.B;
    sp.N = (int)c.N;
    sp.k = c.k;
    sp.n_chunks = pl.n_chunks;
    sp.tiles_per_chunk = pl.tiles_per_chunk;
    sp.n_tiles = pl.n_tiles;
    sp.static_tiles = pl.static_tiles;
    sp.tail_g = pl.tail_g;
    sp.tail_blocks = pl.tail_blocks;
    sp.dmax = c.dmax_norm;
    sp.flag = c.fallback_flag;
    sp.thr0_stride = c.k;
    sp.qimg = (const h8 *)(ws + pl.qimg_off);
    sp.qnorm = (const float *)(ws + pl.qnorm_off);
    sp.keep = c.keep;
    return sp;
}

ScreenParams search_params(const ScreenedCall &c, const SPlan &pl)
{
    char *ws = (char *)c.workspace;
    ScreenParams sp = screen_params(c, pl);
    sp.tail_ctr = (int *)(ws + pl.tailctr_off);
    sp.hist = pl.refresh && (pl.sample || c.phase == Phase::Seeded) ? (unsigned *)(ws + pl.hist_off) : nullptr;
    sp.cand = (SCand *)(ws + pl.cand_off);
    sp.pcnt = (int *)(ws + pl.pcnt_off);
    return sp;
}

int query_image(const ScreenedCall &c, const SPlan &pl)
{
    char *ws = (char *)c.workspace;
    hipLaunchKernelGGL(q_image_kernel, dim3(pl.rows_pad / 32), dim3(128), 0, c.stream, c.Q, c.B, (h8 *)(ws + pl.qimg_off),
                       (float *)(ws + pl.qnorm_off), c.fallback_flag, (c.B + 31) / 32, (int *)(ws + pl.tailctr_off),
                       pl.n_qgroups, pl.hist_off ? (unsigned *)(ws + pl.hist_off) : nullptr);
    TT_LAUNCH_CHECK();
    return TT_OK;
}

float *sample_values(const ScreenedCall &c, const SPlan &pl) { return (float *)((char *)c.workspace + pl.smax_val_off); }

ScreenParams sample_params(ScreenParams ss, const SPlan &pl, float *s_val)
{
    ss.N = (int)pl.s_docs;
    ss.n_tiles = pl.s_tiles;
    ss.n_chunks = pl.s_chunks;
    ss.tiles_per_chunk = pl.s_tiles_per_chunk;
    ss.static_tiles = pl.s_tiles;
    ss.tail_blocks = 0;
    (pl.s_onchip ? ss.top_val : ss.max_val) = s_val;
    return ss;
}

int sample_pass(const ScreenedCall &c, const SPlan &pl, const ScreenParams &sp)
{
    return launch_screen(pl, sample_params(sp, pl, sample_values(c, pl)), c.bf16, c.stream);
}

int select_thresholds(const ScreenedCall &c, const SPlan &pl)
{
    const bool list = c.phase == Phase::SeedList;
    if (!pl.sample) {
        if (c.phase == Phase::Whole)
            return TT_OK;
        const int n = list ? c.B * c.k_seed : c.B;
        hipLaunchKernelGGL(seed_fill_kernel, dim3((n + 255) / 256), dim3(256), 0, c.stream, c.seed, n);
        TT_LAUNCH_CHECK();
        return TT_OK;
    }
    if (list)
        return tt_k_largest_list(sample_values(c, pl), c.B, pl.s_vals, c.k_seed, c.seed, c.stream);
    float *thr = c.phase == Phase::SeedThreshold ? c.seed : (float *)((char *)c.workspace + pl.sthr_val_off);
    return tt_kth_largest(sample_values(c, pl), c.B, pl.s_vals, c.phase == Phase::SeedThreshold ? c.k_seed : c.k, thr, c.stream);
}

int main_pass(const ScreenedCall &c, const SPlan &pl, ScreenParams sp)
{
    if (c.phase == Phase::Seeded || pl.sample) {
        sp.thr0 = c.phase == Phase::Seeded ? c.seed : (const float *)((char *)c.workspace + pl.sthr_val_off);
        sp.thr0_stride = 1;
    }
    if (c.prof_events)
        TT_HIP_CHECK(hipEventRecord((hipEvent_t)c.prof_events[0], c.stream));
    TT_RC_CHECK(launch_screen(pl, sp, c.bf16, c.stream));
    if (c.prof_events)
        TT_HIP_CHECK(hipEventRecord((hipEvent_t)c.prof_events[1], c.stream));
    return TT_OK;
}

int finish(const ScreenedCall &c, const SPlan &pl)
{
    char *ws = (char *)c.workspace;
    FinishParams fp;
    fp.Q = c.Q;
    fp.D32 = c.bf16 ? nullptr : (const float *)c.D32;
    fp.Dbf = c.bf16 ? (const unsigned *)c.D32 : nullptr;
    fp.B = c.B;
    fp.N = (int)c.N;
    fp.k = c.k;
    fp.n_chunks = pl.n_chunks;
    fp.q_per_block = pl.q_per_block;
    fp.dmax = c.dmax_norm;
    fp.cand = (const SCand *)(ws + pl.cand_off);
    fp.pcnt = (const int *)(ws + pl.pcnt_off);
    fp.flag = c.fallback_flag;
    fp.idx_offset = c.idx_offset;
    fp.out_val = c.out_val;
    fp.out_idx = c.out_idx;
    fp.stats = (int *)(ws + pl.stats_off);
    hipLaunchKernelGGL(screen_finish_kernel, dim3(c.B), dim3(256), (size_t)(2 * pl.n_chunks + 1) * sizeof(int), c.stream, fp);
    TT_LAUNCH_CHECK();
    return TT_OK;
}

int fallback(const ScreenedCall &c, const SPlan &pl)
{
    const char *who = c.keep ? (c.bf16 ? "tt_score_topk_masked_bf16" : "tt_score_topk_masked_f32")
                             : (c.bf16 ? "tt_score_topk_bf16" : "tt_score_topk_f32");
    return exact_small(ExactCall{c.Q, c.B, c.d, c.D32, c.bf16, c.N, c.k, c.idx_offset, c.keep, c.out_val, c.out_idx,
                                 (char *)c.workspace + pl.ws_bytes, c.workspace_bytes - pl.ws_bytes, c.stream, who},
                       c.fallback_flag);
}

int screened(const ScreenedCall &c)
{
    SPlan pl;
    TT_RC_CHECK(screened_validate(c, &pl));
    const ScreenParams sp = search_params(c, pl);
    if (c.phase != Phase::Seeded) {
        TT_RC_CHECK(query_image(c, pl));
        if (pl.sample)
            TT_RC_CHECK(sample_pass(c, pl, sp));
        TT_RC_CHECK(select_thresholds(c, pl));
    }
    if (c.phase == Phase::SeedThreshold || c.phase == Phase::SeedList)
        return TT_OK;
    TT_RC_CHECK(main_pass(c, pl, sp));
    TT_RC_CHECK(finish(c, pl));
    return fallback(c, pl);
}

int whole_call(const char *who, const QueryArgs &q, const RowArgs &rows, const OutArgs &out, const ScratchArgs &s)
{
    return screened(ScreenedCall{q, rows, out, s, who, Phase::Whole, q.k, nullptr});
}

int seed_list_call(const char *who, const QueryArgs &q, const RowArgs &rows, int k_seed, float *list, const ScratchArgs &s)
{
    return screened(ScreenedCall{q, rows, OutArgs{}, s, who, Phase::SeedList, k_seed, list});
}

int seeded_call(const char *who, const QueryArgs &q, const RowArgs &rows, const OutArgs &out, const float *seed, const ScratchArgs &s)
{
    return screened(ScreenedCall{q, rows, out, s, who, Phase::Seeded, q.k, (float *)seed});
}
}

TT_EXPORT int tt_index_stats_bf16(const void *D_bf16, int64_t N, int d, float *stats, int reset_stats, tt_stream_t stream)
{
    hipStream_t st = (hipStream_t)stream;
    if (N < 0 || d <= 0 || d % 4 != 0 || d > 4096)
        return tt_fail(TT_ERR_BAD_SHAPE, "tt_index_stats_bf16: N=%lld d=%d", (long long)N, d);
    if (!stats || (N > 0 && !D_bf16))
        return tt_fail(TT_ERR_BAD_SHAPE, "tt_index_stats_bf16: null pointer");
    if (reset_stats)
        TT_RC_CHECK(tt_zero_async(stats, 2 * sizeof(float), st));
    if (N == 0)
        return TT_OK;
    const int64_t want_blocks = (N + 3) / 4;
    hipLaunchKernelGGL(build_from_bf16_kernel, dim3((unsigned)(want_blocks > 8192 ? 8192 : want_blocks)), dim3(256), 0,
                       st, (const unsigned short *)D_bf16, N, d, (float *)nullptr, (_Float16 *)nullptr, (unsigned *)stats);
    TT_LAUNCH_CHECK();
    return TT_OK;
}

TT_EXPORT int tt_score_topk_screened_f32(const float *Q, int B, int d, const float *D32, const void *D16, int64_t N,
                                         int k, float dmax_norm, int64_t idx_offset, float *out_val, int64_t *out_idx,
                                         int32_t *fallback_flag, void *workspace, size_t workspace_bytes,
                                         void *const *prof_events, tt_stream_t stream)
{
    return whole_call("tt_score_topk_screened_f32", {Q, B, d, k, dmax_norm}, f32_rows(D32, D16, N, nullptr),
                 {idx_offset, out_val, out_idx, prof_events}, {fallback_flag, workspace, workspace_bytes, (hipStream_t)stream});
}

TT_EXPORT int tt_score_topk_screened_seed_f32(const float *Q, int B, int d, const void *D16, int64_t N, int k, int k_seed,
                                              float dmax_norm, int32_t *fallback_flag, float *seed, void *workspace,
                                              size_t workspace_bytes, tt_stream_t stream)
{
    return screened(ScreenedCall{{Q, B, d, k, dmax_norm}, f32_rows(nullptr, D16, N, nullptr), OutArgs{},
                                 {fallback_flag, workspace, workspace_bytes, (hipStream_t)stream},
                                 "tt_score_topk_screened_seed_f32", Phase::SeedThreshold, k_seed, seed});
}

TT_EXPORT int tt_score_topk_screened_seed_list_f32(const float *Q, int B, int d, const void *D16, int64_t N, int k, int k_seed,
                                                   float dmax_norm, int32_t *fallback_flag, float *seed_list, void *workspace,
                                                   size_t workspace_bytes, tt_stream_t stream)
{
    return seed_list_call("tt_score_topk_screened_seed_list_f32", {Q, B, d, k, dmax_norm}, f32_rows(nullptr, D16, N, nullptr), k_seed,
                       seed_list, {fallback_flag, workspace, workspace_bytes, (hipStream_t)stream});
}

TT_EXPORT int tt_score_topk_screened_seeded_f32(const float *Q, int B, int d, const float *D32, const void *D16, int64_t N,
                                                int k, float dmax_norm, int64_t idx_offset, float *out_val, int64_t *out_idx,
                                                int32_t *fallback_flag, const float *seed, void *workspace,
                                                size_t workspace_bytes, void *const *prof_events, tt_stream_t stream)
{
    return seeded_call("tt_score_topk_screened_seeded_f32", {Q, B, d, k, dmax_norm}, f32_rows(D32, D16, N, nullptr),
                  {idx_offset, out_val, out_idx, prof_events}, seed, {fallback_flag, workspace, workspace_bytes, (hipStream_t)stream});
}

TT_EXPORT int tt_score_topk_screened_bf16(const float *Q, int B, int d, const void *D_bf16, int64_t N, int k, float dmax_norm,
                                          int64_t idx_offset, float *out_val, int64_t *out_idx, int32_t *fallback_flag,
                                          void *workspace, size_t workspace_bytes, void *const *prof_events, tt_stream_t stream)
{
    return whole_call("tt_score_topk_screened_bf16", {Q, B, d, k, dmax_norm}, bf16_rows(D_bf16, N, nullptr),
                 {idx_offset, out_val, out_idx, prof_events}, {fallback_flag, workspace, workspace_bytes, (hipStream_t)stream});
}

TT_EXPORT int tt_score_topk_screened_seed_list_bf16(const float *Q, int B, int d, const void *D_bf16, int64_t N, int k,
                                                    int k_seed, float dmax_norm, int32_t *fallback_flag, float *seed_list,
                                                    void *workspace, size_t workspace_bytes, tt_stream_t stream)
{
    return seed_list_call("tt_score_topk_screened_seed_list_bf16", {Q, B, d, k, dmax_norm}, bf16_rows(D_bf16, N, nullptr), k_seed,
                       seed_list, {fallback_flag, workspace, workspace_bytes, (hipStream_t)stream});
}

TT_EXPORT int tt_score_topk_screened_seeded_bf16(const float *Q, int B, int d, const void *D_bf16, int64_t N, int k,
                                                 float dmax_norm, int64_t idx_offset, float *out_val, int64_t *out_idx,
                                                 int32_t *fallback_flag, const float *seed, void *workspace,
                                                 size_t workspace_bytes, void *const *prof_events, tt_stream_t stream)
{
    return seeded_call("tt_score_topk_screened_seeded_bf16", {Q, B, d, k, dmax_norm}, bf16_rows(D_bf16, N, nullptr),
                  {idx_offset, out_val, out_idx, prof_events}, seed, {fallback_flag, workspace, workspace_bytes, (hipStream_t)stream});
}

TT_EXPORT int tt_score_topk_screened_masked_f32(const float *Q, int B, int d, const float *D32, const void *D16, int64_t N,
                                                const uint32_t *keep, int k, float dmax_norm, int64_t idx_offset, float *out_val,
                                                int64_t *out_idx, int32_t *fallback_flag, void *workspace, size_t workspace_bytes,
                                                void *const *prof_events, tt_stream_t stream)
{
    return whole_call("tt_score_topk_screened_masked_f32", {Q, B, d, k, dmax_norm}, f32_rows(D32, D16, N, keep),
                 {idx_offset, out_val, out_idx, prof_events}, {fallback_flag, workspace, workspace_bytes, (hipStream_t)stream});
}

TT_EXPORT int tt_score_topk_screened_masked_bf16(const float *Q, int B, int d, const void *D_bf16, int64_t N, const uint32_t *keep,
                                                 int k, float dmax_norm, int64_t idx_offset, float *out_val, int64_t *out_idx,
                                                 int32_t *fallback_flag, void *workspace, size_t workspace_bytes,
                                                 void *const *prof_events, tt_stream_t stream)
{
    return whole_call("tt_score_topk_screened_masked_bf16", {Q, B, d, k, dmax_norm}, bf16_rows(D_bf16, N, keep),
                 {idx_offset, out_val, out_idx, prof_events}, {fallback_flag, workspace, workspace_bytes, (hipStream_t)stream});
}

TT_EXPORT int tt_score_topk_screened_seed_list_masked_f32(const float *Q, int B, int d, const void *D16, int64_t N,
                                                          const uint32_t *keep, int k, int k_seed, float dmax_norm,
                                                          int32_t *fallback_flag, float *seed_list, void *workspace,
                                                          size_t workspace_bytes, tt_stream_t stream)
{
    return seed_list_call("tt_score_topk_screened_seed_list_masked_f32", {Q, B, d, k, dmax_norm}, f32_rows(nullptr, D16, N, keep), k_seed,
                       seed_list, {fallback_flag, workspace, workspace_bytes, (hipStream_t)stream});
}

TT_EXPORT int tt_score_topk_screened_seed_list_masked_bf16(const float *Q, int B, int d, const void *D_bf16, int64_t N,
                                                           const uint32_t *keep, int k, int k_seed, float dmax_norm,
                                                           int32_t *fallback_flag, float *seed_list, void *workspace,
                                                           size_t workspace_bytes, tt_stream_t stream)
{
    return seed_list_call("tt_score_topk_screened_seed_list_masked_bf16", {Q, B, d, k, dmax_norm}, bf16_rows(D_bf16, N, keep), k_seed,
                       seed_list, {fallback_flag, workspace, workspace_bytes, (hipStream_t)stream});
}

TT_EXPORT int tt_score_topk_screened_seeded_masked_f32(const float *Q, int B, int d, const float *D32, const void *D16, int64_t N,
                                                       const uint32_t *keep, int k, float dmax_norm, int64_t idx_offset,
                                                       float *out_val, int64_t *out_idx, int32_t *fallback_flag, const float *seed,
                                                       void *workspace, size_t workspace_bytes, void *const *prof_events,
                                                       tt_stream_t stream)
{
    return seeded_call("tt_score_topk_screened_seeded_masked_f32", {Q, B, d, k, dmax_norm}, f32_rows(D32, D16, N, keep),
                  {idx_offset, out_val, out_idx, prof_events}, seed, {fallback_flag, workspace, workspace_bytes, (hipStream_t)stream});
}

TT_EXPORT int tt_score_topk_screened_seeded_masked_bf16(const float *Q, int B, int d, const void *D_bf16, int64_t N,
                                                        const uint32_t *keep, int k, float dmax_norm, int64_t idx_offset,
                                                        float *out_val, int64_t *out_idx, int32_t *fallback_flag,
                                                        const float *seed, void *workspace, size_t workspace_bytes,
                                                        void *const *prof_events, tt_stream_t stream)
{
    return seeded_call("tt_score_topk_screened_seeded_masked_bf16", {Q, B, d, k, dmax_norm}, bf16_rows(D_bf16, N, keep),
                  {idx_offset, out_val, out_idx, prof_events}, seed, {fallback_flag, workspace, workspace_bytes, (hipStream_t)stream});
}

namespace {
struct DbgPlan {
    SPlan s;
    size_t flag_off;
};
bool make_dbg_plan(int B, int64_t N, int form, DbgPlan *dp)
{
    if (B <= 0 || N <= 0 || (form != 0 && form != 1 && form != 2 && form != 4))
        return false;
    SPlan pl = {};
    pl.stream = form == 0;
    pl.nset = form;
    pl.q_per_block = form == 0 ? 32 : SW * 16 * form;
    pl.n_qgroups = (B + pl.q_per_block - 1) / pl.q_per_block;
    pl.rows_pad = pl.n_qgroups * pl.q_per_block;
    pl.n_tiles = (int)((N + 31) / 32);
    const TTChunks c = tt_chunks(pl.n_tiles, one_round(pl.stream, pl.n_qgroups), INT_MAX);
    pl.tiles_per_chunk = c.tiles_per_chunk;
    pl.n_chunks = c.n_chunks;
    pl.static_tiles = pl.n_tiles;
    pl.tail_g = 1;
    TTWorkspace ws;
    pl.qimg_off = ws.take((size_t)pl.rows_pad * 256 * sizeof(_Float16));
    pl.qnorm_off = ws.take((size_t)pl.rows_pad * sizeof(float));
    dp->flag_off = ws.take((size_t)(pl.rows_pad / 32 + 1) * sizeof(int));
    pl.ws_bytes = ws.off;
    dp->s = pl;
    return true;
}

int debug_screen(const QueryArgs &q, const RowArgs &rows, const ScratchArgs &s, const float *thr, int form, float *out_t)
{
    DbgPlan dp;
    if (rows.N >= (int64_t)INT_MAX - 64 || !make_dbg_plan(q.B, rows.N, form, &dp))
        return tt_fail(TT_ERR_BAD_SHAPE, "tt_debug_screen_s16: B=%d N=%lld form=%d", q.B, (long long)rows.N, form);
    if (!q.Q || !rows.D16 || !out_t)
        return tt_fail(TT_ERR_BAD_SHAPE, "tt_debug_screen_s16: null pointer");
    if (!s.workspace || s.workspace_bytes < dp.s.ws_bytes || ((uintptr_t)s.workspace & 255))
        return tt_fail(TT_ERR_WORKSPACE, "tt_debug_screen_s16: workspace %zu < %zu bytes", s.workspace_bytes, dp.s.ws_bytes);
    char *ws = (char *)s.workspace;
    ScreenParams sp = screen_params(ScreenedCall{q, rows, OutArgs{}, s, "tt_debug_screen_s16", Phase::Whole, q.k, nullptr}, dp.s);
    sp.flag = (int *)(ws + dp.flag_off);
    sp.max_val = out_t;
    sp.dbg_thr = thr;
    hipLaunchKernelGGL(q_image_kernel, dim3(dp.s.rows_pad / 32), dim3(128), 0, s.stream, q.Q, q.B, (h8 *)(ws + dp.s.qimg_off),
                       (float *)(ws + dp.s.qnorm_off), sp.flag, dp.s.rows_pad / 32, (int *)nullptr, 0, (unsigned *)nullptr);
    TT_LAUNCH_CHECK();
    return launch_screen(dp.s, sp, rows.bf16, s.stream);
}
}

TT_EXPORT size_t tt_debug_screen_s16_workspace_bytes(int B, int64_t N, int form)
{
    DbgPlan dp;
    return make_dbg_plan(B, N, form, &dp) ? dp.s.ws_bytes : 0;
}

TT_EXPORT int tt_debug_screen_s16(const float *Q, int B, const void *D16, int64_t N, float dmax_norm, const float *thr,
                                  int form, float *out_t, void *workspace, size_t workspace_bytes, tt_stream_t stream)
{
    return debug_screen({Q, B, 256, 1, dmax_norm}, {D16, nullptr, false, N, nullptr},
                        {nullptr, workspace, workspace_bytes, (hipStream_t)stream}, thr, form, out_t);
}

TT_EXPORT int tt_debug_screen_s16_bf16(const float *Q, int B, const void *D_bf16, int64_t N, float dmax_norm, const float *thr,
                                       int form, float *out_t, void *workspace, size_t workspace_bytes, tt_stream_t stream)
{
    return debug_screen({Q, B, 256, 1, dmax_norm}, {D_bf16, nullptr, true, N, nullptr},
                        {nullptr, workspace, workspace_bytes, (hipStream_t)stream}, thr, form, out_t);
}
```

### twotowermlretrieval_amd/index.py

```python
from __future__ import annotations

from functools import lru_cache
from typing import Callable, NamedTuple, Optional, Tuple

import torch

from . import _lib

__all__ = ["GraphedSearch", "score_topk", "pack_keep_mask", "topk_merge", "topk_exclude", "score_rank", "score_all", "score_ids", "mmr_select", "topk_collapse", "BruteForceIndex", "ShardedIndex", "PendingSearch", "StreamedIndex",
           "shard_bounds", "seed_union", "score_count", "topk_cut_below", "score_topk_tagged", "score_topk_biased", "l2_bias", "l2_distances", "score_topk_after"]


def _stream(t: torch.Tensor) -> int:
    return torch.cuda.current_stream(t.device).cuda_stream


def _need_cuda(*ts: torch.Tensor) -> None:
    for t in ts:
        if not t.is_cuda:
            raise RuntimeError("twotowermlretrieval_amd: this path runs only on an AMD GPU via libtt.so; "
                               f"got a {t.device} tensor (no CPU fallback exists)")


def _f32c(t: torch.Tensor) -> torch.Tensor:
    if t.dtype != torch.float32:
        raise TypeError(f"expected float32, got {t.dtype}")
    return t if t.is_contiguous() else t.contiguous()


def _docs_c(t: torch.Tensor) -> torch.Tensor:
    if t.dtype == torch.bfloat16:
        return t if t.is_contiguous() else t.contiguous()
    return _f32c(t)


SMALL_KMAX = 64


class _ExactRoute(NamedTuple):
    fn: str
    ws_fn: str
    ws_takes_dtype: bool
    masked: bool

    def workspace_bytes(self, B: int, N: int, d: int, k: int, dtype: torch.dtype) -> int:
        tail = (int(dtype == torch.bfloat16),) if self.ws_takes_dtype else ()
        return getattr(_lib.lib(), self.ws_fn)(B, N, d, k, *tail)

    def args(self, q_ptr: int, B: int, d: int, docs_ptr: int, N: int, keep_ptr: Optional[int], k: int, tail: tuple) -> tuple:
        return (q_ptr, B, d, docs_ptr, N, *((keep_ptr,) if self.masked else ()), k, *tail)


@lru_cache(maxsize=None)
def _exact_route(dtype: torch.dtype, k: int, masked: bool) -> _ExactRoute:
    t = "bf16" if dtype == torch.bfloat16 else "f32"
    if masked:
        return _ExactRoute(f"tt_score_topk_masked_{t}", "tt_score_topk_masked_workspace_bytes", True, True)
    if k > SMALL_KMAX:
        return _ExactRoute(f"tt_score_topk_large_{t}", "tt_score_topk_large_workspace_bytes", True, False)
    return _ExactRoute(f"tt_score_topk_{t}", "tt_score_topk_bf16_workspace_bytes" if t == "bf16" else "tt_score_topk_workspace_bytes",
                       False, False)


def _merge_fn(k: int, kp: int = 0, shards: bool = False) -> str:
    large = k > SMALL_KMAX or kp > SMALL_KMAX
    if shards:
        return "tt_topk_merge_shards_large" if large else "tt_topk_merge_shards"
    return "tt_topk_merge_large" if large else "tt_topk_merge"


@lru_cache(maxsize=None)
def _screened_fn(phase: str, bf16: bool, masked: bool = False) -> str:
    infix = {"whole": "", "seed_list": "seed_list_", "seeded": "seeded_"}[phase]
    return f"tt_score_topk_screened_{infix}{'masked_' if masked else ''}{'bf16' if bf16 else 'f32'}"


def _out_pair(B: int, k: int, device, out=None) -> Tuple[torch.Tensor, torch.Tensor]:
    if out is not None:
        return out
    return (torch.empty((B, k), dtype=torch.float32, device=device), torch.empty((B, k), dtype=torch.int64, device=device))


def _squeezed(search: Callable, q: torch.Tensor, *args) -> Tuple[torch.Tensor, torch.Tensor]:
    vals, idx = search(q.unsqueeze(0), *args)
    return vals[0], idx[0]


def _keep_words(n: int) -> int:
    return (n + 31) // 32


_KEEP_DTYPES = tuple(t for t in (torch.int32, getattr(torch, "uint32", None)) if t is not None)


def _check_keep(keep: torch.Tensor, n: int, device) -> torch.Tensor:
    if keep.dtype not in _KEEP_DTYPES:
        raise TypeError(f"keep must be a packed int32 / uint32 bitmask (pack_keep_mask), got {keep.dtype}")
    if keep.device != device:
        raise ValueError(f"keep on {keep.device} but the documents live on {device}")
    if keep.dim() != 1 or keep.numel() != _keep_words(n):
        raise ValueError(f"keep must hold exactly ceil(N/32) = {_keep_words(n)} words for N = {n}, got {tuple(keep.shape)}")
    keep = keep if keep.is_contiguous() else keep.contiguous()
    return keep if keep.dtype == torch.int32 else keep.view(torch.int32)


def pack_keep_mask(keep_bool: torch.Tensor) -> torch.Tensor:
    _need_cuda(keep_bool)
    if keep_bool.dim() != 1:
        raise ValueError(f"pack_keep_mask wants a [N] vector, got {tuple(keep_bool.shape)}")
    b = keep_bool if keep_bool.dtype in (torch.bool, torch.uint8) else keep_bool != 0
    b = b.contiguous().view(torch.uint8)
    n = b.numel()
    keep = torch.empty(_keep_words(n), dtype=torch.int32, device=b.device)
    with torch.cuda.device(b.device):
        _lib.check(_lib.lib().tt_keep_mask_pack(b.data_ptr(), n, keep.data_ptr(), _stream(b)))
    return keep


def _clear_ids(keep: Optional[torch.Tensor], n: int, device, ids, idx_offset: int) -> torch.Tensor:
    if keep is None:
        keep = torch.full((_keep_words(n),), -1, dtype=torch.int32, device=device)
        if n % 32:
            keep[-1] = (1 << (n % 32)) - 1
    ids = torch.as_tensor(ids, dtype=torch.int64, device=device).reshape(-1).contiguous()
    with torch.cuda.device(device):
        _lib.check(_lib.lib().tt_keep_mask_clear_ids(keep.data_ptr(), n, ids.data_ptr(), ids.numel(), idx_offset, _stream(keep)))
    return keep


def _and_keep(persistent: Optional[torch.Tensor], keep: Optional[torch.Tensor], n: int, device) -> Optional[torch.Tensor]:
    if keep is None:
        return persistent
    keep = _check_keep(keep, n, device)
    return keep if persistent is None else keep & persistent


def score_topk(q: torch.Tensor, docs: torch.Tensor, k: int, idx_offset: int = 0,
               workspace: Optional[torch.Tensor] = None, keep: Optional[torch.Tensor] = None) -> Tuple[torch.Tensor, torch.Tensor]:
    if q.dim() == 1:
        return _squeezed(score_topk, q, docs, k, idx_offset, workspace, keep)
    _need_cuda(q, docs)
    q, docs = _f32c(q), _docs_c(docs)
    B, d = q.shape
    N = docs.shape[0]
    if docs.dim() != 2 or docs.shape[1] != d:
        raise ValueError(f"shape mismatch: q {tuple(q.shape)} vs docs {tuple(docs.shape)}")
    if keep is not None:
        keep = _check_keep(keep, N, docs.device)
    vals, idx = _out_pair(B, k, q.device)
    with torch.cuda.device(q.device):
        route = _exact_route(docs.dtype, k, keep is not None)
        need = route.workspace_bytes(B, N, d, k, docs.dtype)
        if workspace is None or workspace.numel() < need:
            workspace = torch.empty(max(need, 16), dtype=torch.uint8, device=q.device)
# ... 601 lines not shown
    if src.dtype != torch.int64 or src.device != vals.device:
        raise ValueError(f"topk_collapse wants int64 group ids on {vals.device}, got {src.dtype} on {src.device}")
    if gids is not None and tuple(gids.shape) != (B, M):
        raise ValueError(f"gids must be [B,M] = [{B},{M}] (one id per entry), got {tuple(gids.shape)}")
    if groups is not None and groups.dim() != 1:
        raise ValueError(f"groups must be [N] (one id per row of the index), got {tuple(groups.shape)}")
    src = src.contiguous()
    dev = vals.device
    if out is None:
        out = (*_out_pair(B, k, dev), torch.empty((B, k), dtype=torch.int64, device=dev),
               torch.empty((B, 2), dtype=torch.int32, device=dev))
    ov, oi, og, info = out
    L = _lib.lib()
    with torch.cuda.device(dev):
        if gids is None:
            _lib.check(L.tt_topk_collapse_table(vals.data_ptr(), idx.data_ptr(), B, M, src.data_ptr() if src.numel() else None,
                                                src.numel(), int(idx_offset), m, k, ov.data_ptr(), oi.data_ptr(), og.data_ptr(),
                                                info.data_ptr(), _stream(vals)))
        else:
            _lib.check(L.tt_topk_collapse_gids(vals.data_ptr(), idx.data_ptr(), src.data_ptr(), B, M, m, k, ov.data_ptr(),
                                               oi.data_ptr(), og.data_ptr(), info.data_ptr(), _stream(vals)))
    return ov, oi, og, info


def _collapse_fetch_k(k: int, ntotal: Optional[int] = None, fetch_k: Optional[int] = None, E: int = 0) -> int:
    k = int(k)
    if k < 1:
        raise ValueError(f"collapsed_search: k = {k} < 1")
    if fetch_k is None:
        fk = max(k, min(SMALL_KMAX, 4 * k)) if k <= SMALL_KMAX else min(COLLAPSE_MMAX, 2 * k)
        fk = max(k, min(fk, COLLAPSE_MMAX - E))
        if ntotal is not None:
            fk = min(fk, max(int(ntotal), 1))
    else:
        fk = int(fetch_k)
        if fk < k:
            raise ValueError(f"collapsed_search needs fetch_k >= k, got fetch_k = {fk} < k = {k}")
    if fk + E > COLLAPSE_MMAX:
        raise ValueError(f"collapsed_search: fetch_k + E = {fk} + {E} = {fk + E} > {COLLAPSE_MMAX}")
    return fk


def _collapse_rounds(search_fn: Callable, collapse_fn: Callable, mask_fn: Callable, max_per_group: int, fetch_k: int, E: int,
                     ntotal: Optional[int], exact: bool, stats: Optional[dict] = None):
    width = COLLAPSE_MMAX - E
    whole = (lambda kk: ntotal is not None and kk >= ntotal)
    counts = {"batched_rounds": 1, "masked_rounds": 0}
    ov, oi, og, info = collapse_fn(*search_fn(None, fetch_k, None))
    complete = info[:, 1].clone()
    if whole(fetch_k):
        complete.fill_(1)
    if exact:
        todo = torch.nonzero(complete == 0).flatten()
        if todo.numel() and width > fetch_k:
            counts["batched_rounds"] += 1
            rv, ri, rg, rinfo = collapse_fn(*search_fn(todo, width, None))
            ov[todo], oi[todo], og[todo], info[todo] = rv, ri, rg, rinfo
            done = rinfo[:, 1] != 0 if not whole(width) else torch.ones_like(rinfo[:, 1], dtype=torch.bool)
            complete[todo] = done.to(complete.dtype)
            todo = todo[~done]
        for b in todo.tolist():
            while True:
                j = int(info[b, 0])
                g = og[b, :j]
                uniq, cnt = torch.unique(g[g >= 0], return_counts=True)
                kk = width - j
                nv, ni = search_fn(todo.new_tensor([b]), kk, mask_fn(uniq[cnt >= max_per_group], oi[b, :j]))
                counts["masked_rounds"] += 1
                rv, ri, rg, rinfo = collapse_fn(torch.cat([ov[b:b + 1, :j], nv], 1), torch.cat([oi[b:b + 1, :j], ni], 1))
                ov[b], oi[b], og[b], info[b] = rv[0], ri[0], rg[0], rinfo[0]
                if whole(kk) or int(rinfo[0, 1]):
                    complete[b] = 1
                    break
    if stats is not None:
        stats.update(counts)
    return ov, oi, og, complete


def _owned_gids(groups: torch.Tensor, ids: torch.Tensor, idx_offset: int) -> torch.Tensor:
    N = groups.numel()
    n = ids - idx_offset
    own = (ids >= 0) & (n >= 0) & (n < N)
    if N == 0:
        return torch.zeros_like(ids)
    return groups[torch.where(own, n, torch.zeros_like(n))].masked_fill_(~own, 0)


def _collapsed_search(index, q: torch.Tensor, k: int, max_per_group: int, fetch_k: Optional[int], keep, exclude, exact: bool,
                      groups: Optional[torch.Tensor], n_rows: int, idx_offset: int, device, ntotal: Optional[int], gid_fn=None):
    if groups is None:
        raise ValueError("collapsed_search: this index has no groups (set_groups)")
    if q.dim() == 1:
        res = _collapsed_search(index, q.unsqueeze(0), k, max_per_group, fetch_k, keep, _exclude_row(exclude), exact, groups, n_rows,
                                idx_offset, device, ntotal, gid_fn)
        return tuple(t[0] for t in res)
    _need_cuda(q)
    k, m = int(k), int(max_per_group)
    if m < 1:
        raise ValueError(f"collapsed_search: max_per_group = {m} < 1")
    E = 0
    if exclude is not None:
        exclude, _ = _check_exclude(exclude, q.shape[0], 1, device)
        E = exclude.shape[1]
    fk = _collapse_fetch_k(k, ntotal, fetch_k, E)
    if exact and k + E > COLLAPSE_EXACT_KMAX:
        raise ValueError(f"an exact collapsed search answers k + E <= {COLLAPSE_EXACT_KMAX}, got {k} + {E} (exact=False has no such bound)")

    def search_fn(rows, kk, keep_r):
        return index.search(q if rows is None else q[rows], kk, keep=keep if keep_r is None else keep_r,
                            exclude=exclude if exclude is None or rows is None else exclude[rows])

    def collapse_fn(v, i):
        if v.shape[1] < k:
            pad = k - v.shape[1]
            v = torch.cat([v, v.new_full((v.shape[0], pad), float("-inf"))], 1)
            i = torch.cat([i, i.new_full((i.shape[0], pad), -1)], 1)
        if gid_fn is not None:
            return topk_collapse(v, i, k, gids=gid_fn(i), max_per_group=m)
        return topk_collapse(v, i, k, groups=groups, max_per_group=m, idx_offset=idx_offset)

    def mask_fn(saturated, selected):
        keep_r = pack_keep_mask(~torch.isin(groups, saturated))
        if keep is not None:
            keep_r &= _check_keep(keep, n_rows, device)
        return _clear_ids(keep_r, n_rows, device, selected, idx_offset)

    stats = {}
    res = _collapse_rounds(search_fn, collapse_fn, mask_fn, m, fk, E, ntotal, exact, stats)
    index.collapse_rounds = (stats["batched_rounds"], stats["masked_rounds"])
    return res


_COLLAPSED_DOC = """(values f32 [B,k], ids int64 [B,k], group ids int64 [B,k], complete int32 [B]): the best k rows with at most
        max_per_group rows per document group (set_groups; a negative group id = ungrouped, never collapsed) -- field collapsing.
        The eligible rows (not removed, kept by keep=, not in exclude=) in (score desc, index asc) order are walked, a row is
        kept if it is ungrouped or fewer than max_per_group rows of its group were kept before it, and the result is the
        first k kept rows, tail (-inf, -1, -1).  Values and ids are the search's own, copied.  It is search(q, fetch_k, keep=,
        exclude=) followed by one filter launch (topk_collapse).  fetch_k defaults to min(ntotal, max(k, min(64, 4 k))) up to
        k = 64 and to min(ntotal, 1024, 2 k) above; fetch_k + E <= 1024.
        exact=False returns that one round and does NOT synchronise with the host: complete[b] = 1 says the row is the answer
        (k rows kept, or the fetch saw every eligible row), 0 that it is an exact PREFIX of it (a group owned the head of the
        list; values beyond `kept` are the tail).  exact=True (the default) goes on by rounds until every query is complete,
        and SYNCHRONISES with the host once per round: the incomplete queries once more as a batch for 1024 - E rows, then
        each still incomplete query alone under a keep-bitmask without its saturated groups and selected rows (torch.isin
        over the group table: a pass over N ids per round).  It needs k + E <= 512.  collapse_rounds afterwards holds
        (batched rounds, masked rounds) of the most recent call."""


SCREEN_MIN_BATCH = 1
SCREEN_PADDED_MIN_BATCH = 33
SCREEN_MIN_DOCS = 65536


def _fp16_range_ok(dmax: float, amax: float) -> bool:
    return dmax == dmax and amax < 6.0e4 and dmax < 6.0e4


class _Screen:

    def __init__(self, rows: torch.Tensor, filt: torch.Tensor, bf16: bool, dmax_norm: float):
        self.rows, self.filt, self.bf16, self.dmax_norm = rows, filt, bool(bf16), float(dmax_norm)
        self.n = rows.shape[0]

    @classmethod
    def for_f32(cls, docs: torch.Tensor) -> Optional["_Screen"]:
        N, d = docs.shape
        if not (d == 256 or (d < 256 and d % 4 == 0)):
            return None
        rows = docs
        if d < 256:
            rows = torch.zeros((N, 256), dtype=torch.float32, device=docs.device)
            rows[:, :d] = docs
        filt = torch.empty((N, 256), dtype=torch.float16, device=docs.device)
        stats = torch.zeros(2, dtype=torch.float32, device=docs.device)
        with torch.cuda.device(docs.device):
            _lib.check(_lib.lib().tt_index_build_f16(rows.data_ptr(), N, 256, filt.data_ptr(), stats.data_ptr(), _stream(docs)))
        dmax, amax = (float(x) for x in stats.tolist())
        return cls(rows, filt, False, dmax) if _fp16_range_ok(dmax, amax) else None

    @classmethod
    def for_bf16(cls, docs: torch.Tensor) -> Optional["_Screen"]:
        N, d = docs.shape
        if d == 256:
            stats = torch.zeros(2, dtype=torch.float32, device=docs.device)
            with torch.cuda.device(docs.device):
                _lib.check(_lib.lib().tt_index_stats_bf16(docs.data_ptr(), N, d, stats.data_ptr(), 1, _stream(docs)))
            dmax, amax = (float(x) for x in stats.tolist())
            if _fp16_range_ok(dmax, amax):
                return cls(docs, docs, True, dmax)
        import warnings
        warnings.warn(f"BruteForceIndex: a bf16 [{N},{d}] corpus is screened only at d = 256 within the fp16 range; "
                      "this index runs the exact bf16 kernel", RuntimeWarning, stacklevel=3)
        return None

    def workspace_bytes(self, B: int, k: int, masked: bool = False) -> int:
        if masked:
            return _lib.lib().tt_score_topk_screened_masked_workspace_bytes(B, self.n, 256, k, int(self.bf16))
        name = "tt_score_topk_screened_bf16_workspace_bytes" if self.bf16 else "tt_score_topk_screened_workspace_bytes"
        return getattr(_lib.lib(), name)(B, self.n, 256, k)

    def seed_list(self, q: torch.Tensor, k: int, ks: int, flags: torch.Tensor, ws: torch.Tensor,
                  keep: Optional[torch.Tensor] = None) -> torch.Tensor:
        B, d = q.shape
        lst = torch.empty((B, ks), dtype=torch.float32, device=q.device)
        fn = getattr(_lib.lib(), _screened_fn("seed_list", self.bf16, keep is not None))
        mask = () if keep is None else (keep.data_ptr(),)
        _lib.check(fn(q.data_ptr(), B, d, self.filt.data_ptr(), self.n, *mask, k, ks, self.dmax_norm, flags.data_ptr(),
                      lst.data_ptr(), ws.data_ptr(), ws.numel(), _stream(q)))
        return lst

    def run(self, q: torch.Tensor, k: int, idx_offset: int, vals: torch.Tensor, idx: torch.Tensor, flags: torch.Tensor,
            ws: torch.Tensor, seed: Optional[torch.Tensor] = None, prof_events=None, keep: Optional[torch.Tensor] = None) -> None:
        B, d = q.shape
        fn = getattr(_lib.lib(), _screened_fn("whole" if seed is None else "seeded", self.bf16, keep is not None))
        corpus = (self.rows.data_ptr(),) if self.bf16 else (self.rows.data_ptr(), self.filt.data_ptr())
        mask = () if keep is None else (keep.data_ptr(),)
        thr = () if seed is None else (seed.data_ptr(),)
        _lib.check(fn(q.data_ptr(), B, d, *corpus, self.n, *mask, k, self.dmax_norm, idx_offset, vals.data_ptr(),
                      idx.data_ptr(), flags.data_ptr(), *thr, ws.data_ptr(), ws.numel(), prof_events, _stream(q)))


class BruteForceIndex(_CursorSearch):

    def __init__(self, doc_embeddings: torch.Tensor, idx_offset: int = 0, screen: bool = False, screen_masked: bool = False):
        _need_cuda(doc_embeddings)
        self.docs = _docs_c(doc_embeddings)
        self.idx_offset = int(idx_offset)
        if not isinstance(screen, _Screen):
            build = _Screen.for_bf16 if self.docs.dtype == torch.bfloat16 else _Screen.for_f32
            screen = build(self.docs) if screen and self.docs.shape[0] > 0 else None
        self._screen: Optional[_Screen] = screen
        self.screen_masked = bool(screen_masked)
        self.docs16 = screen.filt if screen is not None and not screen.bf16 else None
        self.dmax_norm = screen.dmax_norm if screen is not None else float("nan")
        self.fallback_flags = torch.zeros(1, dtype=torch.int32, device=self.docs.device)
        self.keep_stats = False
        self._last_ws = None
        self._keep: Optional[torch.Tensor] = None
        self._tags: Optional[torch.Tensor] = None
        self._bias: Optional[torch.Tensor] = None
        self._groups: Optional[torch.Tensor] = None
        self.collapse_rounds = (0, 0)

    @classmethod
    def _from_buffers(cls, docs32: torch.Tensor, docs16: Optional[torch.Tensor], dmax_norm: float, idx_offset: int,
                      screen_masked: bool = False):
        return cls(docs32, idx_offset, _Screen(docs32, docs16, False, dmax_norm) if docs16 is not None else False,
                   screen_masked=screen_masked)

    @property
    def _screen_bf16(self) -> bool:
        return self._screen is not None and self._screen.bf16

    @property
    def ntotal(self) -> int:
        return self.docs.shape[0]

    @property
    def device(self) -> torch.device:
        return self.docs.device

    @property
    def keep_mask(self) -> Optional[torch.Tensor]:
        return self._keep

    def remove_ids(self, ids) -> None:
        self._keep = _clear_ids(self._keep, self.docs.shape[0], self.docs.device, ids, self.idx_offset)

    def search_stats(self) -> Optional[torch.Tensor]:
        if self._last_ws is None:
            return None
        ws, B, k = self._last_ws
        with torch.cuda.device(self.docs.device):
            off = _lib.lib().tt_score_topk_screened_stats_offset(B, self.docs.shape[0], 256, k)
        return ws[off:off + 8 * B].view(torch.int32).view(B, 2).clone()

    def search(self, q: torch.Tensor, k: int = 10, _prof_events=None, out=None, _seed_union=None,
               _k_seed: int = 0, _k_list: int = 0, keep: Optional[torch.Tensor] = None,
               exclude: Optional[torch.Tensor] = None, candidates: Optional[torch.Tensor] = None) -> Tuple[torch.Tensor, torch.Tensor]:
        if q.dim() == 1:
            return _squeezed(self.search, q, k, _prof_events, None, None, 0, 0, keep, _exclude_row(exclude),
                             _ids_row(candidates, "candidates"))
        _need_cuda(q)
        if q.device != self.docs.device:
            raise ValueError(f"queries on {q.device} but the index lives on {self.docs.device}")
        if q.shape[-1] != self.docs.shape[1]:
            raise ValueError(f"shape mismatch: q {tuple(q.shape)} vs docs {tuple(self.docs.shape)}")
        if exclude is not None:
            exclude, kk = _check_exclude(exclude, q.shape[0], k, self.docs.device)
            v, i = self.search(q, kk, _prof_events, None, _seed_union, _k_seed, _k_list, keep, None, candidates)
            return topk_exclude(v, i, exclude, k, out)
        keep = _and_keep(self._keep, keep, self.docs.shape[0], self.docs.device)
        if candidates is not None:
            return _merge_candidates(*self._score_ids(q, candidates, keep, True, "candidates"), k, out)
        if self._screens(q.shape[0], k, keep is not None):
            return self._search_screened(q, k, _prof_events, out, _seed_union, _k_seed, _k_list, keep)
        if keep is not None and self._screen is not None:
            self.fallback_flags = torch.ones((q.shape[0] + 31) // 32, dtype=torch.int32, device=self.docs.device)
        v, i = score_topk(q, self.docs, k, self.idx_offset, keep=keep)
        if out is not None:
            out[0].copy_(v)
            out[1].copy_(i)
            return out
        return v, i

    @property
    def tags(self) -> Optional[torch.Tensor]:
        return self._tags

    def set_tags(self, tags: torch.Tensor) -> None:
        self._tags = _check_tags(tags, self.docs.shape[0], self.docs.device)

    def tagged_search(self, q: torch.Tensor, k: int = 10, match_mask=0xffffffff, match_value=0,
                      keep: Optional[torch.Tensor] = None, out=None) -> Tuple[torch.Tensor, torch.Tensor]:
        if self._tags is None:
            raise ValueError("tagged_search: this index has no tags (set_tags)")
        if q.dim() == 1:
            return _squeezed(self.tagged_search, q, k, match_mask, match_value, keep)
        _need_cuda(q)
        if q.device != self.docs.device:
            raise ValueError(f"queries on {q.device} but the index lives on {self.docs.device}")
        if q.shape[-1] != self.docs.shape[1]:
            raise ValueError(f"shape mismatch: q {tuple(q.shape)} vs docs {tuple(self.docs.shape)}")
        B = q.shape[0]
        mm = _match_words(match_mask, B, self.docs.device, "match_mask")
        mv = _match_words(match_value, B, self.docs.device, "match_value")
        keep = _and_keep(self._keep, keep, self.docs.shape[0], self.docs.device)
        res = _tagged_into(_f32c(q), self.docs, self._tags, mm, mv, keep, k, self.idx_offset, out)
        if self._screen is not None:
            self.fallback_flags = torch.ones((B + 31) // 32, dtype=torch.int32, device=self.docs.device)
        return res

    @property
    def bias(self) -> Optional[torch.Tensor]:
        return self._bias

    def set_bias(self, bias: Optional[torch.Tensor]) -> None:
        if bias is None:
            self._bias = None
            return
        bias = _check_bias(bias, self.docs.shape[0], self.docs.device)
        _finite_bias(bias, self.docs.shape[0])
        self._bias = bias

    def biased_search(self, q: torch.Tensor, k: int = 10, keep: Optional[torch.Tensor] = None,
                      exclude: Optional[torch.Tensor] = None, out=None, candidates=None) -> Tuple[torch.Tensor, torch.Tensor]:
        if self._bias is None:
            raise ValueError("biased_search: this index has no bias (set_bias)")
        if candidates is not None:
            raise ValueError("biased_search takes no candidates=: the candidate scores (score_ids) carry no bias")
        if q.dim() == 1:
            return _squeezed(self.biased_search, q, k, keep, _exclude_row(exclude))
        _need_cuda(q)
        if q.device != self.docs.device:
            raise ValueError(f"queries on {q.device} but the index lives on {self.docs.device}")
        if q.shape[-1] != self.docs.shape[1]:
            raise ValueError(f"shape mismatch: q {tuple(q.shape)} vs docs {tuple(self.docs.shape)}")
        B = q.shape[0]
        if exclude is not None:
            exclude, kk = _check_exclude(exclude, B, k, self.docs.device)
            if kk > BIASED_KMAX:
                raise ValueError(f"a biased search with an exclusion list runs for k + E = {kk} > {BIASED_KMAX}")
            v, i = self.biased_search(q, kk, keep)
            return topk_exclude(v, i, exclude, k, out)
        keep = _and_keep(self._keep, keep, self.docs.shape[0], self.docs.device)
        res = _biased_into(_f32c(q), self.docs, self._bias, keep, k, self.idx_offset, out)
        if self._screen is not None:
            self.fallback_flags = torch.ones((B + 31) // 32, dtype=torch.int32, device=self.docs.device)
        return res

    def _cursor_device(self) -> torch.device:
        return self.docs.device

    def _search_after(self, q: torch.Tensor, k: int, av: torch.Tensor, ai: torch.Tensor, keep: Optional[torch.Tensor], out=None):
        if q.device != self.docs.device:
            raise ValueError(f"queries on {q.device} but the index lives on {self.docs.device}")
        if q.shape[-1] != self.docs.shape[1]:
            raise ValueError(f"shape mismatch: q {tuple(q.shape)} vs docs {tuple(self.docs.shape)}")
        keep = _and_keep(self._keep, keep, self.docs.shape[0], self.docs.device)
        res = _after_into(_f32c(q), self.docs, av, ai, keep, k, self.idx_offset, out)
        if self._screen is not None:
            self.fallback_flags = torch.ones((q.shape[0] + 31) // 32, dtype=torch.int32, device=self.docs.device)
        return res

    def _score_ids(self, q: torch.Tensor, ids: torch.Tensor, keep: Optional[torch.Tensor], want_idx: bool, what: str = "ids"):
        q = _f32c(q)
        ids = _check_ids(ids, q.shape[0], self.docs.device, what)
        vals = torch.empty(ids.shape, dtype=torch.float32, device=q.device)
        idx = torch.empty_like(ids) if want_idx else None
        _score_ids_into(q, self.docs, ids, self.idx_offset, keep, vals, idx)
        return vals, idx

    def score_ids(self, q: torch.Tensor, ids: torch.Tensor, keep: Optional[torch.Tensor] = None) -> torch.Tensor:
        if q.dim() == 1:
            return self.score_ids(q.unsqueeze(0), _ids_row(ids), keep)[0]
        _need_cuda(q)
        if q.device != self.docs.device:
            raise ValueError(f"queries on {q.device} but the index lives on {self.docs.device}")
        if q.shape[-1] != self.docs.shape[1]:
            raise ValueError(f"shape mismatch: q {tuple(q.shape)} vs docs {tuple(self.docs.shape)}")
        return self._score_ids(q, ids, _and_keep(self._keep, keep, self.docs.shape[0], self.docs.device), False)[0]

    def diverse_search(self, q: torch.Tensor, k: int = 10, lambda_: float = 0.5, fetch_k: Optional[int] = None,
                       keep: Optional[torch.Tensor] = None, exclude: Optional[torch.Tensor] = None) -> Tuple[torch.Tensor, torch.Tensor]:
        if q.dim() == 1:
            return _squeezed(self.diverse_search, q, k, lambda_, fetch_k, keep, _exclude_row(exclude))
        fk, lam = _mmr_fetch_k(k, fetch_k), _check_lambda(lambda_)
        v, i = self.search(q, fk, keep=keep, exclude=exclude)
        return mmr_select(v, i, self.docs, k, lam, self.idx_offset)

    def _candidate_rows(self, ids: torch.Tensor) -> torch.Tensor:
        return _owned_rows(self.docs, ids, self.idx_offset)

    diverse_search.__doc__ = _DIVERSE_DOC + """
        The candidates' rows are gathered from this index's own rows (fp32, or bf16 widened exactly) by the kernel, whichever
        layout searched: the screened and the exact route return the same list, so the result does not depend on it."""

    @property
    def groups(self) -> Optional[torch.Tensor]:
        return self._groups

    def set_groups(self, groups: Optional[torch.Tensor]) -> None:
        self._groups = None if groups is None else _check_groups(groups, self.docs.shape[0], self.docs.device)

    def collapsed_search(self, q: torch.Tensor, k: int = 10, max_per_group: int = 1, fetch_k: Optional[int] = None,
                         keep: Optional[torch.Tensor] = None, exclude: Optional[torch.Tensor] = None, exact: bool = True):
        return _collapsed_search(self, q, k, max_per_group, fetch_k, keep, exclude, exact, self._groups, self.docs.shape[0],
                                 self.idx_offset, self.docs.device, self.docs.shape[0])
# ... 934 lines not shown
```

Before: 268,200 queries/s.

## Add int8 pre-screen gating ahead of f16 MFMA screen with resume fallback

Builds an int8-quantized copy of the corpus and a per-query int8 image with error bounds, then runs an int8 dot-product screen that gates tiles before the f16 screen and exact fp32 rescoring. The aim is to cut HBM bytes read per document (256 B instead of 512 B) and use faster int8 matrix ops for most tiles. Candidates that cannot be ruled out are handed to the existing f16 screen through a resumable screen body. It adds a one-time index build, extra memory for the int8 copy, more complex error bounds, and abandon/fallback paths.

```diff
diff --git a/include/tt.h b/include/tt.h
--- a/include/tt.h
+++ b/include/tt.h
@@ -118,6 +118,14 @@
                                float dmax_norm, int64_t idx_offset, float *out_val, int64_t *out_idx,
                                int32_t *fallback_flag, void *workspace, size_t workspace_bytes,
                                void *const *prof_events , tt_stream_t stream);
+
+int tt_index_build_i8(const void *D16, int64_t N, int d, const float *stats16, void *D8, float *stats8, tt_stream_t stream);
+int tt_score_topk_screened_i8_eligible(int B, int64_t N, int d, int k);
+size_t tt_score_topk_screened_i8_stats_offset(int B, int64_t N, int d, int k);
+int tt_score_topk_screened_i8_f32(const float *Q, int B, int d, const float *D32, const void *D16, const void *D8, int64_t N,
+                                  int k, float dmax_norm, float delta_d, float e8, float dn8, int64_t idx_offset,
+                                  float *out_val, int64_t *out_idx, int32_t *fallback_flag, void *workspace,
+                                  size_t workspace_bytes, void *const *prof_events , tt_stream_t stream);
 
 int tt_score_topk_screened_seed_f32(const float *Q, int B, int d, const void *D16, int64_t N, int k, int k_seed, float dmax_norm,
                                     int32_t *fallback_flag, float *seed , void *workspace, size_t workspace_bytes,
diff --git a/include/tt_debug.h b/include/tt_debug.h
--- a/include/tt_debug.h
+++ b/include/tt_debug.h
@@ -14,6 +14,11 @@
 int tt_debug_screen_s16_bf16(const float *Q, int B, const void *D_bf16, int64_t N, float dmax_norm, const float *thr, int form,
                              float *out_t, void *workspace, size_t workspace_bytes, tt_stream_t stream);
 
+size_t tt_debug_screen_s8_workspace_bytes(int B);
+int tt_debug_screen_s8(const float *Q, int B, const void *D8, int64_t N, float dmax_norm, float delta_d, float e8, float dn8,
+                       const float *thr, int32_t *out_s8, float *out_aux, int32_t *out_gate, void *workspace,
+                       size_t workspace_bytes, tt_stream_t stream);
+
 #ifdef __cplusplus
 }
 #endif
diff --git a/twotowermlretrieval_amd/_lib.py b/twotowermlretrieval_amd/_lib.py
--- a/twotowermlretrieval_amd/_lib.py
+++ b/twotowermlretrieval_amd/_lib.py
@@ -71,6 +71,10 @@
     "tt_seed_union_f32": (_i, [_vp, _i, _i, _i, _i, _vp, _vp]),
     "tt_score_topk_screened_seeded_f32": (_i, [_vp, _i, _i, _vp, _vp, _i64, _i, _f, _i64, _vp, _vp, _vp, _vp, _vp, _sz, _vp, _vp]),
     "tt_score_topk_screened_f32": (_i, [_vp, _i, _i, _vp, _vp, _i64, _i, _f, _i64, _vp, _vp, _vp, _vp, _sz, _vp, _vp]),
+    "tt_index_build_i8": (_i, [_vp, _i64, _i, _vp, _vp, _vp, _vp]),
+    "tt_score_topk_screened_i8_eligible": (_i, [_i, _i64, _i, _i]),
+    "tt_score_topk_screened_i8_stats_offset": (_sz, [_i, _i64, _i, _i]),
+    "tt_score_topk_screened_i8_f32": (_i, [_vp, _i, _i, _vp, _vp, _vp, _i64, _i, _f, _f, _f, _f, _i64, _vp, _vp, _vp, _vp, _sz, _vp, _vp]),
     "tt_score_topk_screened_masked_workspace_bytes": (_sz, [_i, _i64, _i, _i, _i]),
     "tt_score_topk_screened_masked_f32": (_i, [_vp, _i, _i, _vp, _vp, _i64, _vp, _i, _f, _i64, _vp, _vp, _vp, _vp, _sz, _vp, _vp]),
     "tt_score_topk_screened_masked_bf16": (_i, [_vp, _i, _i, _vp, _i64, _vp, _i, _f, _i64, _vp, _vp, _vp, _vp, _sz, _vp, _vp]),
diff --git a/twotowermlretrieval_amd/csrc/screen.hip b/twotowermlretrieval_amd/csrc/screen.hip
--- a/twotowermlretrieval_amd/csrc/screen.hip
+++ b/twotowermlretrieval_amd/csrc/screen.hip
@@ -11,6 +11,7 @@
 typedef _Float16 h8 __attribute__((ext_vector_type(8)));
 typedef _Float16 h4 __attribute__((ext_vector_type(4)));
 typedef unsigned u32x4 __attribute__((ext_vector_type(4)));
+typedef int i32x4 __attribute__((ext_vector_type(4)));
 typedef __attribute__((address_space(3))) void lds_void;
 typedef const __attribute__((address_space(1))) void gbl_void;
 
@@ -41,6 +42,12 @@
 {
     return 1.10e-3f * qnorm * dmax + 1e-6f * (qnorm + dmax);
 }
+
+__device__ __forceinline__ float screen_eps8(float q16n, float eqn, float qn, float e8, float dn8, float dmax)
+{
+    return 1.0001f * (q16n * e8 + eqn * dn8) + 3.1e-5f * qn * dmax + 2e-6f * (qn + dmax);
+}
+constexpr int I8_NSTATS = 8;
 
 template <int NCH>
 __device__ __forceinline__ void bf16_to_f16_lds(char *base, int lane)
@@ -91,6 +98,7 @@
     const float *qnorm = nullptr;
     const float *dbg_thr = nullptr;
     const unsigned *keep = nullptr;
+    int *resume = nullptr;
 };
 
 __device__ __forceinline__ void scand_store_async(const SCand *base, unsigned byte_off, float v, int x)
@@ -185,14 +193,25 @@
         }
 }
 
+struct QImageI8 {
+    i32x4 *img8 = nullptr;
+    float2 *qaux = nullptr;
+    int *i8stats = nullptr;
+    float dd = 0.0f, e8 = 0.0f, dn8 = 0.0f, dmax = 0.0f;
+};
+
 __global__ __launch_bounds__(128) void q_image_kernel(const float *__restrict__ Q, int B, h8 *__restrict__ img,
                                                       float *__restrict__ qnorm, int *__restrict__ flag, int n_flags,
-                                                      int *__restrict__ tail_ctr, int n_ctr, unsigned *__restrict__ hist)
+                                                      int *__restrict__ tail_ctr, int n_ctr, unsigned *__restrict__ hist,
+                                                      QImageI8 q8)
 {
     __shared__ int any_bad[2];
-    if (blockIdx.x == 0)
+    if (blockIdx.x == 0) {
         for (int i = threadIdx.x; i < n_ctr; i += 128)
             tail_ctr[i] = 0;
+        if (q8.i8stats && threadIdx.x < I8_NSTATS)
+            q8.i8stats[threadIdx.x] = 0;
+    }
     if (hist)
         for (int i = threadIdx.x; i < 32 * REFRESH_LEVELS; i += 128)
             hist[(size_t)blockIdx.x * (32 * REFRESH_LEVELS) + i] = 0u;
@@ -202,7 +221,7 @@
     const int qrow = 16 * S + n;
     const bool live = qrow < B;
     const float *qp = Q + (size_t)min(qrow, B - 1) * 256 + 8 * g;
-    float ss = 0.0f;
+    float ss = 0.0f, ss16 = 0.0f, amax16 = 0.0f;
     bool bad = false;
 #pragma unroll
     for (int s = 0; s < 8; ++s) {
@@ -216,6 +235,9 @@
             bad |= !(fabsf(x0) <= 60000.0f) || !(fabsf(x1) <= 60000.0f);
             hv[e] = (_Float16)x0;
             hv[4 + e] = (_Float16)x1;
+            const float h0 = (float)hv[e], h1 = (float)hv[4 + e];
+            ss16 += h0 * h0 + h1 * h1;
+            amax16 = fmaxf(amax16, fmaxf(fabsf(h0), fabsf(h1)));
         }
         img[((size_t)S * 8 + s) * 64 + lane] = hv;
     }
@@ -223,6 +245,39 @@
     ss += __shfl_xor(ss, 32);
     if (g == 0)
         qnorm[qrow] = sqrtf(ss);
+    if (q8.img8) {
+        ss16 += __shfl_xor(ss16, 16);
+        ss16 += __shfl_xor(ss16, 32);
+        amax16 = fmaxf(amax16, __shfl_xor(amax16, 16));
+        amax16 = fmaxf(amax16, __shfl_xor(amax16, 32));
+        const float dq = amax16 / 127.0f;
+        const float inv = dq > 0.0f && dq < 3.0e38f ? 1.0f / dq : 0.0f;
+        const float *qp8 = Q + (size_t)min(qrow, B - 1) * 256 + 16 * g;
+        float se = 0.0f;
+#pragma unroll
+        for (int s = 0; s < 4; ++s) {
+            i32x4 pk;
+#pragma unroll
+            for (int j = 0; j < 4; ++j) {
+                const f32x4 a = *(const f32x4 *)(qp8 + 64 * s + 4 * j);
+                unsigned wd = 0u;
+#pragma unroll
+                for (int e = 0; e < 4; ++e) {
+                    const float x16 = (float)(_Float16)(live ? a[e] : 0.0f);
+                    const float qi = fminf(fmaxf(rintf(x16 * inv), -127.0f), 127.0f);
+                    const float err = __fmaf_rn(-dq, qi, x16);
+                    se += err * err;
+                    wd |= ((unsigned)(int)qi & 0xffu) << (8 * e);
+                }
+                pk[j] = (int)wd;
+            }
+            q8.img8[((size_t)S * 4 + s) * 64 + lane] = pk;
+        }
+        se += __shfl_xor(se, 16);
+        se += __shfl_xor(se, 32);
+        if (g == 0)
+            q8.qaux[qrow] = float2{dq * q8.dd, screen_eps8(sqrtf(ss16), sqrtf(se), sqrtf(ss), q8.e8, q8.dn8, q8.dmax)};
+    }
     const bool wave_bad = __ballot(bad && live) != 0ull;
     if (lane == 0)
         any_bad[wv] = wave_bad ? 1 : 0;
@@ -231,10 +286,15 @@
         flag[blockIdx.x] = (any_bad[0] | any_bad[1]) ? 2 : 0;
 }
 
-template <bool MAXONLY, int NSET, bool BF = false, bool MASKED = false, bool ONCHIP = false>
-__global__ __launch_bounds__(SW * 64, 2) void screen_kernel(ScreenParams p)
-{
-    extern __shared__ __attribute__((aligned(16))) char ring[];
+struct ScreenResume {
+    int t0 = 0, t1 = 0;
+    int cnt[4] = {};
+    float negthr[4] = {};
+};
+
+template <bool MAXONLY, int NSET, bool BF, bool MASKED, bool ONCHIP, bool RESUME = false>
+__device__ __forceinline__ void screen_body(const ScreenParams &p, char *ring , const ScreenResume &rs)
+{
     constexpr int DMA_AUX = NSET < 3 ? 2 : 0;
     const int lane = threadIdx.x & 63;
     const int w = __builtin_amdgcn_readfirstlane(threadIdx.x >> 6);
@@ -242,6 +302,10 @@
     const int qgroup = blockIdx.x / p.n_chunks;
     int t0 = chunk * p.tiles_per_chunk;
     int t1 = min(t0 + p.tiles_per_chunk, p.static_tiles);
+    if (RESUME) {
+        t0 = rs.t0;
+        t1 = rs.t1;
+    }
     __shared__ int next_block;
     const int k = p.k;
     const int g = lane >> 4, n = lane & 15;
@@ -258,7 +322,7 @@
     int cnt[NSET];
 #pragma unroll
     for (int c = 0; c < NSET; ++c)
-        cnt[c] = 0;
+        cnt[c] = RESUME ? rs.cnt[c < 4 ? c : 0] : 0;
 #pragma unroll
     for (int c = 0; c < NSET; ++c) {
         const int qrow = qbase + 16 * c + n;
@@ -279,6 +343,8 @@
         float c_init = -t_init;
         if (MAXONLY)
             c_init = (p.dbg_thr && live) ? -p.dbg_thr[qrow] : 0.0f;
+        if (RESUME)
+            c_init = rs.negthr[c < 4 ? c : 0];
         negthr[c] = f32x4{c_init, c_init, c_init, c_init};
         if (!MAXONLY && g == 0)
             ladder_base[w * QW + 16 * c + n] = t_init + eps2[c];
@@ -640,6 +706,495 @@
     }
 }
 
+template <bool MAXONLY, int NSET, bool BF = false, bool MASKED = false, bool ONCHIP = false>
+__global__ __launch_bounds__(SW * 64, 2) void screen_kernel(ScreenParams p)
+{
+    extern __shared__ __attribute__((aligned(16))) char ring[];
+    screen_body<MAXONLY, NSET, BF, MASKED, ONCHIP>(p, ring, ScreenResume{});
+}
+
+constexpr int I8_TILE_BYTES = 32 * 256;
+constexpr int I8_LCAP = 2048;
+constexpr int I8_MAX_K = 16;
+constexpr int I8_ABANDON_DIV = 8;
+constexpr int I8_RW = 4;
+
+struct I8Params {
+    const signed char *D8 = nullptr;
+    const i32x4 *qimg8 = nullptr;
+    const float2 *qaux = nullptr;
+    int *i8stats = nullptr;
+    int gate_lower = 0;
+};
+
+__device__ __forceinline__ int i8_gate_c(float thr, float eps8, float scale, bool live)
+{
+    if (!live)
+        return -(1 << 30);
+    if (!(scale > 0.0f))
+        return 1 << 30;
+    const float x = fminf(fmaxf((thr - eps8) / scale, -1.0e9f), 1.0e9f);
+    return 2 - (int)floorf(x);
+}
+
+__global__ __launch_bounds__(SW * 64, 2) void screen_i8_kernel(ScreenParams p, I8Params p8)
+{
+    extern __shared__ __attribute__((aligned(16))) char ring[];
+    constexpr int NSET = 4;
+    const int lane = threadIdx.x & 63;
+    const int w = __builtin_amdgcn_readfirstlane(threadIdx.x >> 6);
+    unsigned *const list = (unsigned *)(ring + SRING * I8_TILE_BYTES) + w * I8_LCAP;
+    const int chunk = blockIdx.x % p.n_chunks;
+    const int qgroup = blockIdx.x / p.n_chunks;
+    int t0 = chunk * p.tiles_per_chunk;
+    int t1 = min(t0 + p.tiles_per_chunk, p.static_tiles);
+    __shared__ int next_block;
+    const int k = p.k;
+    const int g = lane >> 4, n = lane & 15;
+    constexpr int QW = 16 * NSET, QB = SW * QW;
+    const int qbase = qgroup * QB + w * QW;
+    const bool wave_live = qbase < p.B;
+    __shared__ float ladder_base[SW * 64];
+    __shared__ int wg_blocks[2];
+    if (threadIdx.x == 0)
+        wg_blocks[0] = wg_blocks[1] = 0;
+    const bool refresh = p.hist != nullptr;
+    const unsigned *const hwave = p.hist + (size_t)qbase * REFRESH_LEVELS;
+
+    i32x4 q8reg[NSET][4];
+    float eps2[NSET], negthr[NSET], eps8[NSET], scale[NSET];
+    int cnt[NSET], gate_c[NSET];
+    auto load_q8 = [&]() {
+        int ln = lane;
+        asm volatile("" : "+v"(ln));
+        const i32x4 *src = p8.qimg8 + ((size_t)(qbase / 16) * 4) * 64 + ln;
+#pragma unroll
+        for (int c = 0; c < NSET; ++c)
+#pragma unroll
+            for (int s = 0; s < 4; ++s)
+                q8reg[c][s] = src[(c * 4 + s) * 64];
+#pragma unroll
+        for (int c = 0; c < NSET; ++c)
+#pragma unroll
+            for (int s = 0; s < 4; ++s)
+                asm volatile("" : "+v"(q8reg[c][s]));
+    };
+#pragma unroll
+    for (int c = 0; c < NSET; ++c) {
+        cnt[c] = 0;
+        const int qrow = qbase + 16 * c + n;
+        const bool live = qrow < p.B;
+        float qn = 0.0f;
+        float2 aux = float2{0.0f, 0.0f};
+        if (wave_live) {
+            qn = p.qnorm[qrow];
+            aux = p8.qaux[qrow];
+        }
+        eps2[c] = 2.0f * screen_eps(qn, p.dmax);
+        const float floor_thr = -(1.01f * qn * p.dmax + 1e-30f);
+        const float t_init = live ? (p.thr0 ? fmaxf(p.thr0[(size_t)qrow * p.thr0_stride + p.thr0_stride - 1] - eps2[c], floor_thr) : floor_thr)
+                                  : INFINITY;
+        negthr[c] = -t_init;
+        scale[c] = aux.x;
+        eps8[c] = aux.y;
+        gate_c[c] = i8_gate_c(t_init, eps8[c], scale[c], live) + p8.gate_lower;
+        if (g == 0)
+            ladder_base[w * QW + 16 * c + n] = t_init + eps2[c];
+    }
+    if (wave_live)
+        load_q8();
+
+    SCand *const cwave = p.cand + ((size_t)blockIdx.x * QB + w * QW) * SCAP;
+
+    auto compact_where = [&](int c, unsigned qmask) {
+        asm volatile("s_waitcnt vmcnt(0)" ::: "memory");
+        while (qmask) {
+            const int q = __ffs((int)qmask) - 1;
+            qmask &= qmask - 1;
+            const int nq[4] = {__builtin_amdgcn_readlane(cnt[c], q), __builtin_amdgcn_readlane(cnt[c], q + 16),
+                               __builtin_amdgcn_readlane(cnt[c], q + 32), __builtin_amdgcn_readlane(cnt[c], q + 48)};
+            const float slack = __builtin_bit_cast(float, __builtin_amdgcn_readlane(__builtin_bit_cast(int, eps2[c]), q));
+            int n_new;
+            float tn;
+            bool have, ovf;
+            screen_compact(cwave + (size_t)(16 * c + q) * SCAP, nq, k, slack, lane, n_new, tn, have, ovf);
+            if (ovf && lane == 0)
+                atomicOr(p.flag + ((qbase + 16 * c) >> 5), 1);
+            if (n == q) {
+                cnt[c] = (n_new - g + 3) >> 2;
+                if (have)
+                    negthr[c] = fminf(negthr[c], -tn);
+            }
+        }
+    };
+
+    auto refresh_thresholds = [&]() {
+        asm volatile("s_waitcnt vmcnt(0)" ::: "memory");
+        int ln = lane;
+        asm volatile("" : "+v"(ln));
+        const int n = ln & 15, g = ln >> 4, lane = ln;
+#pragma unroll
+        for (int c = 0; c < NSET; ++c) {
+            __builtin_amdgcn_sched_barrier(0);
+            if (refresh) {
+                const unsigned *hp = hwave + (unsigned)((16 * c + n) * REFRESH_LEVELS + 4 * g);
+                int sfx[4];
+                int run = 0;
+#pragma unroll
+                for (int i = 3; i >= 0; --i) {
+                    run += (int)__hip_atomic_load(hp + i, __ATOMIC_RELAXED, __HIP_MEMORY_SCOPE_AGENT);
+                    sfx[i] = run;
+                }
+                const int x16 = (lane ^ 16) << 2, x32 = (lane ^ 32) << 2;
+                const int t16 = __builtin_amdgcn_ds_bpermute(x16, run), t32 = __builtin_amdgcn_ds_bpermute(x32, run),
+                          t48 = __builtin_amdgcn_ds_bpermute(x32, t16);
+                const int above = ((g ^ 1) > g ? t16 : 0) + ((g ^ 2) > g ? t32 : 0) + ((g ^ 3) > g ? t48 : 0);
+                int jtop = -1;
+#pragma unroll
+                for (int i = 0; i < 4; ++i)
+                    if (above + sfx[i] >= k)
+                        jtop = 4 * g + i;
+                jtop = max(jtop, __builtin_amdgcn_ds_bpermute(x16, jtop));
+                jtop = max(jtop, __builtin_amdgcn_ds_bpermute(x32, jtop));
+                if (jtop > 0) {
+                    const float base = ladder_base[w * QW + 16 * c + n];
+                    negthr[c] = fminf(negthr[c], eps2[c] - refresh_edge(jtop, (float)REFRESH_STEP * eps2[c], base));
+                }
+            }
+            gate_c[c] = i8_gate_c(-negthr[c], eps8[c], scale[c], qbase + 16 * c + n < p.B) + p8.gate_lower;
+        }
+    };
+
+    auto select_set = [&](int c, int tile, f32x4 a0, f32x4 a1) {
+        const int tile_base = tile * 32;
+        f32x4 acc[2] = {a0, a1};
+        if (tile_base + 32 > p.N) {
+#pragma unroll
+            for (int u = 0; u < 2; ++u)
+#pragma unroll
+                for (int r = 0; r < 4; ++r)
+                    if (tile_base + 16 * u + 4 * g + r >= p.N)
+                        acc[u][r] = -INFINITY;
+        }
+        int mu[2];
+#pragma unroll
+        for (int u = 0; u < 2; ++u)
+            mu[u] = max(max(__float_as_int(acc[u][0]), __float_as_int(acc[u][1])), max(__float_as_int(acc[u][2]), __float_as_int(acc[u][3])));
+        if (__ballot(max(mu[0], mu[1]) >= 0) == 0ull)
+            return;
+        const unsigned mine = (unsigned)(((16 * c + n) * SCAP + SQUART * g) * sizeof(SCand));
+        const float thr_c = -negthr[c];
+#pragma unroll
+        for (int u = 0; u < 2; ++u) {
+#pragma unroll
+            for (int r = 0; r < 4; ++r) {
+                if (__float_as_int(acc[u][r]) >= 0) {
+                    scand_store_async(cwave, mine + (unsigned)cnt[c] * (unsigned)sizeof(SCand), acc[u][r] + thr_c,
+                                      tile_base + 16 * u + 4 * g + r);
+                    ++cnt[c];
+                }
+            }
+        }
+        if (refresh) {
+            const int mbest = max(mu[0], mu[1]);
+            if (mbest >= 0) {
+                const int lq = 16 * c + n;
+                const float lwidth = (float)REFRESH_STEP * eps2[c];
+                const float lbase = ladder_base[w * QW + lq];
+                const float v = __int_as_float(mbest) + thr_c;
+                if (lwidth >= REFRESH_MIN_WIDTH && v >= lbase)
+                    u32_inc_async(hwave, (unsigned)((lq * REFRESH_LEVELS + refresh_level(v, lbase, 1.0f / lwidth)) * sizeof(unsigned)));
+            }
+        }
+        unsigned long long full = __ballot(cnt[c] > SQ_TRIGGER);
+        full = (full | (full >> 32));
+        full = (full | (full >> 16)) & 0xffffull;
+        if (full)
+            compact_where(c, (unsigned)full);
+    };
+
+    int nlist = 0;
+    const char *const D16c = (const char *)p.D16;
+    auto flush = [&]() {
+        asm volatile("s_waitcnt vmcnt(0) lgkmcnt(0)" ::: "memory");
+        if (nlist > 0) {
+            int ln = lane;
+            asm volatile("" : "+v"(ln));
+            const int n = ln & 15, g = ln >> 4;
+#pragma unroll
+            for (int c = 0; c < NSET; ++c) {
+                __builtin_amdgcn_sched_barrier(0);
+                h8 qf[8];
+                const h8 *src = p.qimg + ((size_t)(qbase / 16 + c) * 8) * 64 + ln;
+#pragma unroll
+                for (int s = 0; s < 8; ++s)
+                    qf[s] = src[s * 64];
+                const int end = 2 * nlist;
+                auto next_block = [&](int pos) {
+                    for (; pos < end; ++pos) {
+                        const unsigned e = (unsigned)__builtin_amdgcn_readfirstlane((int)list[pos >> 1]);
+                        if ((e >> (4 * (pos & 1) + c)) & 1u)
+                            break;
+                    }
+                    return pos;
+                };
+                int pos = next_block(0);
+#pragma unroll 1
+                while (pos < end) {
+                    h8 a[I8_RW][8];
+                    int at[I8_RW];
+#pragma unroll
+                    for (int j = 0; j < I8_RW; ++j) {
+                        at[j] = -1;
+                        if (pos < end) {
+                            at[j] = pos;
+                            const int tile = (int)((unsigned)__builtin_amdgcn_readfirstlane((int)list[pos >> 1]) >> 8);
+                            const int doc = min(tile * 32 + 16 * (pos & 1) + n, p.N - 1);
+                            const char *rp = D16c + (size_t)doc * 512 + 16 * g;
+#pragma unroll
+                            for (int s = 0; s < 8; ++s)
+                                a[j][s] = *(const h8 *)(rp + 64 * s);
+                            pos = next_block(pos + 1);
+                        }
+                    }
+#pragma unroll
+                    for (int j = 0; j < I8_RW; ++j) {
+                        if (at[j] < 0)
+                            continue;
+                        const int tile = (int)((unsigned)__builtin_amdgcn_readfirstlane((int)list[at[j] >> 1]) >> 8);
+                        f32x4 t = f32x4{negthr[c], negthr[c], negthr[c], negthr[c]};
+#pragma unroll
+                        for (int s = 0; s < 8; ++s)
+                            t = __builtin_amdgcn_mfma_f32_16x16x32_f16(a[j][s], qf[s], t, 0, 0, 0);
+                        const f32x4 none = f32x4{-INFINITY, -INFINITY, -INFINITY, -INFINITY};
+                        select_set(c, tile, (at[j] & 1) ? none : t, (at[j] & 1) ? t : none);
+                    }
+                }
+            }
+            nlist = 0;
+        }
+        refresh_thresholds();
+        load_q8();
+    };
+
+    const char *D = (const char *)p8.D8;
+    const char *rowp;
+    auto set_row = [&](int tile) {
+        const int row = 4 * w + (lane >> 4);
+        const int doc = min(tile * 32 + row, p.N - 1);
+        const int chunk16 = (lane & 15) ^ (row & 15);
+        rowp = D + (size_t)doc * 256 + chunk16 * 16;
+    };
+    auto dma_piece = [&](int stage) {
+        __builtin_amdgcn_global_load_lds((gbl_void *)rowp, (lds_void *)(ring + stage * I8_TILE_BYTES + w * 1024), 16, 0, 0);
+    };
+    int n_trip_blocks = 0, n_trip_tiles = 0, n_tiles_seen = 0, n_full = 0;
+    int left_t0 = 0, left_t1 = 0;
+    int win_blocks = 0, win_tiles = 0;
+    int seen_blocks = 0, seen_streamed = 0;
+    auto write_stats = [&](bool abandoned) {
+        if (p8.i8stats && wave_live && lane == 0) {
+            atomicAdd(p8.i8stats + 0, n_trip_blocks);
+            atomicAdd(p8.i8stats + 1, n_trip_tiles);
+            atomicAdd(p8.i8stats + 2, n_tiles_seen);
+            atomicAdd(p8.i8stats + 3, n_full);
+            if (abandoned && w == 0)
+                atomicAdd(p8.i8stats + 4, 1);
+        }
+    };
+
+    for (;;) {
+    if (t0 < t1) {
+#pragma unroll
+        for (int gi = 0; gi < SRING - STPB; ++gi) {
+            set_row(min(t0 + gi, t1 - 1));
+            dma_piece(gi);
+        }
+        int stage = 0;
+        const int rd_base = n * 256;
+        int cp_shift = refresh && t0 < p.static_tiles ? REFRESH_FIRST_SHIFT : 0;
+        auto next_checkpoint = [&](int from) {
+            while (cp_shift > 0) {
+                const int cp = t0 + (((t1 - t0) >> cp_shift) & ~(STPB - 1));
+                --cp_shift;
+                if (cp > from)
+                    return cp;
+            }
+            return t1;
+        };
+        int next_cp = next_checkpoint(t0);
+        for (int tile = t0;; ++tile) {
+            const bool at_cp = tile == next_cp;
+            if (at_cp)
+                next_cp = tile < t1 ? next_checkpoint(tile) : -1;
+            if (wave_live && (at_cp || nlist >= I8_LCAP)) {
+                if (!at_cp)
+                    ++n_full;
+                if (at_cp && lane == 0) {
+                    atomicAdd(&wg_blocks[0], win_blocks);
+                    atomicAdd(&wg_blocks[1], 8 * win_tiles);
+                }
+                if (at_cp)
+                    win_blocks = win_tiles = 0;
+                flush();
+            }
+            if (tile >= t1)
+                break;
+            if ((tile - t0) % STPB == 0) {
+                asm volatile("s_waitcnt vmcnt(%0)" ::"n"(SRING - 2 * STPB) : "memory");
+                __builtin_amdgcn_s_barrier();
+            }
+            if (at_cp) {
+                const int tb = __builtin_amdgcn_readfirstlane(*(volatile int *)&wg_blocks[0]);
+                const int sb = __builtin_amdgcn_readfirstlane(*(volatile int *)&wg_blocks[1]);
+                const bool abandon = I8_ABANDON_DIV * (tb - seen_blocks) > sb - seen_streamed;
+                seen_blocks = tb;
+                seen_streamed = sb;
+                if (abandon) {
+                    left_t0 = tile;
+                    left_t1 = t1;
+                    break;
+                }
+            }
+            const int fill_stage = (stage + SRING - STPB) % SRING;
+            set_row(min(tile + SRING - STPB, t1 - 1));
+            if (!wave_live)
+                dma_piece(fill_stage);
+            if (wave_live) {
+                const char *buf = ring + stage * I8_TILE_BYTES + rd_base;
+                i32x4 a0[4], a1[4];
+#pragma unroll
+                for (int s = 0; s < 4; ++s) {
+                    const int off = ((4 * s + g) ^ n) << 4;
+                    a0[s] = *(const i32x4 *)(buf + off);
+                    a1[s] = *(const i32x4 *)(buf + 16 * 256 + off);
+                }
+                dma_piece(fill_stage);
+                i32x4 acc[2][NSET];
+#pragma unroll
+                for (int s = 0; s < 4; ++s) {
+#pragma unroll
+                    for (int c = 0; c < NSET; ++c) {
+                        const i32x4 cin = i32x4{gate_c[c], gate_c[c], gate_c[c], gate_c[c]};
+                        acc[0][c] = __builtin_amdgcn_mfma_i32_16x16x64_i8(a0[s], q8reg[c][s], s == 0 ? cin : acc[0][c], 0, 0, 0);
+                        acc[1][c] = __builtin_amdgcn_mfma_i32_16x16x64_i8(a1[s], q8reg[c][s], s == 0 ? cin : acc[1][c], 0, 0, 0);
+                    }
+                }
+                int mall = INT_MIN;
+#pragma unroll
+                for (int u = 0; u < 2; ++u)
+#pragma unroll
+                    for (int c = 0; c < NSET; ++c)
+#pragma unroll
+                        for (int r = 0; r < 4; ++r)
+                            mall = max(mall, acc[u][c][r]);
+                ++n_tiles_seen;
+                if (__ballot(mall >= 0) != 0ull) {
+                    unsigned mask = 0u;
+#pragma unroll
+                    for (int u = 0; u < 2; ++u)
+#pragma unroll
+                        for (int c = 0; c < NSET; ++c) {
+                            const int m = max(max(acc[u][c][0], acc[u][c][1]), max(acc[u][c][2], acc[u][c][3]));
+                            if (__ballot(m >= 0) != 0ull)
+                                mask |= 1u << (4 * u + c);
+                        }
+                    if (lane == 0)
+                        list[nlist] = ((unsigned)tile << 8) | mask;
+                    ++nlist;
+                    ++n_trip_tiles;
+                    n_trip_blocks += __popc(mask);
+                    win_blocks += __popc(mask);
+                }
+                ++win_tiles;
+            }
+            stage = (stage + 1) % SRING;
+        }
+    }
+    asm volatile("s_waitcnt vmcnt(0)" ::: "memory");
+    __builtin_amdgcn_s_barrier();
+    if (p.tail_blocks == 0 || left_t0 < left_t1)
+        break;
+    if (threadIdx.x == 0)
+        next_block = atomicAdd(p.tail_ctr + qgroup, 1);
+    __syncthreads();
+    const int blk = next_block;
+    if (blk >= p.tail_blocks)
+        break;
+    t0 = p.static_tiles + blk * p.tail_g;
+    t1 = min(t0 + p.tail_g, p.n_tiles);
+    }
+    asm volatile("s_waitcnt vmcnt(0)" ::: "memory");
+    __builtin_amdgcn_s_barrier();
+
+    write_stats(left_t0 < left_t1);
+    if (threadIdx.x == 0) {
+        p.resume[4 * blockIdx.x + 0] = left_t0;
+        p.resume[4 * blockIdx.x + 1] = left_t1;
+    }
+    if (left_t0 < left_t1) {
+        int *mine = p.resume + 4 * (size_t)gridDim.x + 8 * ((size_t)blockIdx.x * (SW * 64) + threadIdx.x);
+#pragma unroll
+        for (int c = 0; c < NSET; ++c) {
+            mine[c] = cnt[c];
+            mine[4 + c] = __float_as_int(negthr[c]);
+        }
+        return;
+    }
+#pragma unroll
+    for (int c = 0; c < NSET; ++c) {
+        int tot = cnt[c] + __shfl_xor(cnt[c], 16);
+        tot += __shfl_xor(tot, 32);
+        const unsigned long long over = __ballot(tot > k) & 0xffffull;
+        if (over)
+            compact_where(c, (unsigned)over);
+        int packed = cnt[c] << (8 * g);
+        packed |= __shfl_xor(packed, 16);
+        packed |= __shfl_xor(packed, 32);
+        const int qrow = qbase + 16 * c + n;
+        if (g == 0 && qrow < p.B)
+            p.pcnt[(size_t)qrow * p.n_chunks + chunk] = packed;
+    }
+}
+
+__global__ __launch_bounds__(SW * 64, 2) void screen_resume_kernel(ScreenParams p)
+{
+    extern __shared__ __attribute__((aligned(16))) char ring[];
+    ScreenResume rs;
+    rs.t0 = p.resume[4 * blockIdx.x + 0];
+    rs.t1 = p.resume[4 * blockIdx.x + 1];
+    if (rs.t0 >= rs.t1)
+        return;
+    const int *mine = p.resume + 4 * (size_t)gridDim.x + 8 * ((size_t)blockIdx.x * (SW * 64) + threadIdx.x);
+#pragma unroll
+    for (int c = 0; c < 4; ++c) {
+        rs.cnt[c] = mine[c];
+        rs.negthr[c] = __int_as_float(mine[4 + c]);
+    }
+    screen_body<false, 4, false, false, false, true>(p, ring, rs);
+}
+
+__global__ __launch_bounds__(64) void debug_s8_kernel(const i32x4 *__restrict__ qimg8, const signed char *__restrict__ D8, int B,
+                                                      int N, int *__restrict__ out)
+{
+    const int lane = threadIdx.x, g = lane >> 4, n = lane & 15;
+    const int S = blockIdx.y;
+    const int doc = min((int)blockIdx.x * 16 + n, N - 1);
+    i32x4 acc = i32x4{0, 0, 0, 0};
+#pragma unroll
+    for (int s = 0; s < 4; ++s) {
+        const i32x4 a = *(const i32x4 *)(D8 + (size_t)doc * 256 + 64 * s + 16 * g);
+        acc = __builtin_amdgcn_mfma_i32_16x16x64_i8(a, qimg8[((size_t)S * 4 + s) * 64 + lane], acc, 0, 0, 0);
+    }
+    const int qrow = 16 * S + n;
+#pragma unroll
+    for (int r = 0; r < 4; ++r) {
+        const int d = (int)blockIdx.x * 16 + 4 * g + r;
+        if (qrow < B && d < N)
+            out[(size_t)qrow * N + d] = acc[r];
+    }
+}
+
 constexpr int TW = 4;
 constexpr int TSLAB_BYTES = 32 * 128;
 constexpr int TSTAGE = 4;
@@ -1205,6 +1760,49 @@
     }
 }
 
+__global__ __launch_bounds__(256) void build_i8_kernel(const _Float16 *__restrict__ D16, int64_t N, const float *__restrict__ stats16,
+                                                       signed char *__restrict__ out8, unsigned *__restrict__ stats8)
+{
+    __shared__ float red[8];
+    const int lane = threadIdx.x & 63, wave = threadIdx.x >> 6;
+    const float dd = (float)(_Float16)stats16[1] / 127.0f;
+    const bool ok = dd > 0.0f && dd < 3.0e38f;
+    const float inv = ok ? 1.0f / dd : 0.0f;
+    float emax = ok ? 0.0f : INFINITY, nmax = 0.0f;
+    for (int64_t row = (int64_t)blockIdx.x * 4 + wave; row < N; row += (int64_t)gridDim.x * 4) {
+        const h4 hv = *(const h4 *)(D16 + row * 256 + lane * 4);
+        float se = 0.0f, sn = 0.0f;
+        unsigned wd = 0u;
+#pragma unroll
+        for (int e = 0; e < 4; ++e) {
+            const float x = (float)hv[e];
+            const float qi = fminf(fmaxf(rintf(x * inv), -127.0f), 127.0f);
+            const float err = __fmaf_rn(-dd, qi, x);
+            se += err * err;
+            sn += (dd * qi) * (dd * qi);
+            wd |= ((unsigned)(int)qi & 0xffu) << (8 * e);
+        }
+        *(unsigned *)(out8 + row * 256 + lane * 4) = wd;
+#pragma unroll
+        for (int off = 32; off >= 1; off >>= 1) {
+            se += __shfl_xor(se, off);
+            sn += __shfl_xor(sn, off);
+        }
+        emax = fmaxf(emax, 1.0001f * sqrtf(se));
+        nmax = fmaxf(nmax, 1.0001f * sqrtf(sn));
+    }
+    if (lane == 0) {
+        red[wave] = emax;
+        red[4 + wave] = nmax;
+    }
+    __syncthreads();
+    if (threadIdx.x == 0) {
+        atomicMax(stats8, __float_as_uint(fmaxf(fmaxf(red[0], red[1]), fmaxf(red[2], red[3]))));
+        atomicMax(stats8 + 1, __float_as_uint(fmaxf(fmaxf(red[4], red[5]), fmaxf(red[6], red[7]))));
+        atomicMax(stats8 + 2, __float_as_uint(ok ? dd : INFINITY));
+    }
+}
+
 struct SPlan {
     bool stream;
     int nset;
@@ -1222,6 +1820,8 @@
     int s_vals;
     size_t cand_off, pcnt_off, smax_val_off, sthr_val_off, qimg_off, qnorm_off, stats_off, ws_bytes;
     int rows_pad;
+    bool i8;
+    size_t qimg8_off, qaux_off, i8stats_off, resume_off;
 };
 
 constexpr int64_t SAMPLE_MIN_N = 65536;
@@ -1285,6 +1885,12 @@
     pl.hist_off = pl.stream ? 0 : ws.take(rows * REFRESH_LEVELS * sizeof(unsigned));
     const int refresh_min = TT_AB_SWITCH(TT_SCREEN_REFRESH_MIN_TILES, REFRESH_MIN_TILES);
     pl.refresh = !pl.stream && TT_AB_SWITCH(TT_SCREEN_THR_REFRESH, 1) != 0 && c.tiles_per_chunk >= (refresh_min < 8 ? 8 : refresh_min);
+    pl.i8 = pl.refresh && pl.sample && pl.nset == 4 && pl.n_tiles < (1 << 24) && k <= TT_AB_SWITCH(TT_SCREEN_I8_MAX_K, I8_MAX_K) &&
+            TT_AB_SWITCH(TT_SCREEN_I8, 1) != 0;
+    pl.qimg8_off = ws.take(rows * 256);
+    pl.qaux_off = ws.take(rows * sizeof(float2));
+    pl.i8stats_off = ws.take(I8_NSTATS * sizeof(int));
+    pl.resume_off = ws.take(pl.nset == 4 && !pl.stream ? (size_t)n_tasks * (4 + 8 * SW * 64) * sizeof(int) : 0);
     pl.smax_val_off = pl.s_onchip ? pl.cand_off : ws.take(rows * (size_t)(pl.sample ? pl.s_tiles : 1) * sizeof(float));
     pl.ws_bytes = ws.off;
     return pl;
@@ -1408,6 +2014,8 @@
     bool bf16;
     int64_t N;
     const unsigned *keep;
+    const void *D8 = nullptr;
+    float dd = 0.0f, e8 = 0.0f, dn8 = 0.0f;
 };
 struct OutArgs { int64_t idx_offset; float *out_val; int64_t *out_idx; void *const *prof_events; };
 struct ScratchArgs { int32_t *fallback_flag; void *workspace; size_t workspace_bytes; hipStream_t stream; };
@@ -1416,6 +2024,7 @@
     Phase phase;
     int k_seed;
     float *seed;
+    bool gated(const SPlan &pl) const { return pl.i8 && D8 && phase == Phase::Whole && !keep && !bf16; }
 };
 
 RowArgs f32_rows(const float *D32, const void *D16, int64_t N, const unsigned *keep) { return {D16, D32, false, N, keep}; }
@@ -1442,6 +2051,8 @@
         return tt_fail(TT_ERR_BAD_SHAPE, "%s: k_seed=%d outside [1, k=%d]", who, c.k_seed, c.k);
     if ((uintptr_t)c.keep & 3)
         return tt_fail(TT_ERR_BAD_SHAPE, "%s: keep must be 4-byte aligned", who);
+    if (c.D8 && (((uintptr_t)c.D8 & 15) || !(c.dd > 0.0f) || !(c.e8 >= 0.0f) || !(c.dn8 >= 0.0f) || !(c.dd + c.e8 + c.dn8 < 3.0e38f)))
+        return tt_fail(TT_ERR_BAD_SHAPE, "%s: int8 shadow %p with dd=%g e8=%g dn8=%g", who, c.D8, c.dd, c.e8, c.dn8);
     *pl = make_splan(c.B, c.N, c.k);
     const size_t need = pl->ws_bytes + fallback_ws_bytes(c.B, c.N, c.d, c.k, c.bf16);
     if (!c.workspace || c.workspace_bytes < need || ((uintptr_t)c.workspace & 255) || (c.bf16 && ((uintptr_t)c.D16 & 15)))
@@ -1487,9 +2098,19 @@
 int query_image(const ScreenedCall &c, const SPlan &pl)
 {
     char *ws = (char *)c.workspace;
+    QImageI8 q8;
+    if (c.gated(pl)) {
+        q8.img8 = (i32x4 *)(ws + pl.qimg8_off);
+        q8.qaux = (float2 *)(ws + pl.qaux_off);
+        q8.i8stats = (int *)(ws + pl.i8stats_off);
+        q8.dd = c.dd;
+        q8.e8 = c.e8;
+        q8.dn8 = c.dn8;
+        q8.dmax = c.dmax_norm;
+    }
     hipLaunchKernelGGL(q_image_kernel, dim3(pl.rows_pad / 32), dim3(128), 0, c.stream, c.Q, c.B, (h8 *)(ws + pl.qimg_off),
                        (float *)(ws + pl.qnorm_off), c.fallback_flag, (c.B + 31) / 32, (int *)(ws + pl.tailctr_off),
-                       pl.n_qgroups, pl.hist_off ? (unsigned *)(ws + pl.hist_off) : nullptr);
+                       pl.n_qgroups, pl.hist_off ? (unsigned *)(ws + pl.hist_off) : nullptr, q8);
     TT_LAUNCH_CHECK();
     return TT_OK;
 }
@@ -1538,7 +2159,26 @@
     }
     if (c.prof_events)
         TT_HIP_CHECK(hipEventRecord((hipEvent_t)c.prof_events[0], c.stream));
-    TT_RC_CHECK(launch_screen(pl, sp, c.bf16, c.stream));
+    if (c.gated(pl)) {
+        char *ws = (char *)c.workspace;
+        I8Params p8;
+        p8.D8 = (const signed char *)c.D8;
+        p8.qimg8 = (const i32x4 *)(ws + pl.qimg8_off);
+        p8.qaux = (const float2 *)(ws + pl.qaux_off);
+        p8.i8stats = (int *)(ws + pl.i8stats_off);
+        p8.gate_lower = TT_AB_SWITCH(TT_SCREEN_I8_GATE_LOWER, 0);
+        const size_t lds = (size_t)SRING * I8_TILE_BYTES + (size_t)SW * I8_LCAP * sizeof(unsigned);
+        TT_HIP_CHECK(hipFuncSetAttribute((const void *)screen_i8_kernel, hipFuncAttributeMaxDynamicSharedMemorySize, (int)lds));
+        void *args[] = {&sp, &p8};
+        sp.resume = (int *)(ws + pl.resume_off);
+        TT_HIP_CHECK(hipLaunchKernel((const void *)screen_i8_kernel, dim3(pl.n_qgroups * sp.n_chunks), dim3(SW * 64), args, lds, c.stream));
+        const size_t lds16 = (size_t)SRING * STILE_BYTES;
+        TT_HIP_CHECK(hipFuncSetAttribute((const void *)screen_resume_kernel, hipFuncAttributeMaxDynamicSharedMemorySize, (int)lds16));
+        void *rargs[] = {&sp};
+        TT_HIP_CHECK(hipLaunchKernel((const void *)screen_resume_kernel, dim3(pl.n_qgroups * sp.n_chunks), dim3(SW * 64), rargs, lds16, c.stream));
+    } else {
+        TT_RC_CHECK(launch_screen(pl, sp, c.bf16, c.stream));
+    }
     if (c.prof_events)
         TT_HIP_CHECK(hipEventRecord((hipEvent_t)c.prof_events[1], c.stream));
     return TT_OK;
@@ -1639,6 +2279,48 @@
                  {idx_offset, out_val, out_idx, prof_events}, {fallback_flag, workspace, workspace_bytes, (hipStream_t)stream});
 }
 
+TT_EXPORT int tt_score_topk_screened_i8_f32(const float *Q, int B, int d, const float *D32, const void *D16, const void *D8,
+                                            int64_t N, int k, float dmax_norm, float delta_d, float e8, float dn8,
+                                            int64_t idx_offset, float *out_val, int64_t *out_idx, int32_t *fallback_flag,
+                                            void *workspace, size_t workspace_bytes, void *const *prof_events, tt_stream_t stream)
+{
+    RowArgs rows = f32_rows(D32, D16, N, nullptr);
+    rows.D8 = D8;
+    rows.dd = delta_d;
+    rows.e8 = e8;
+    rows.dn8 = dn8;
+    return whole_call("tt_score_topk_screened_i8_f32", {Q, B, d, k, dmax_norm}, rows, {idx_offset, out_val, out_idx, prof_events},
+                      {fallback_flag, workspace, workspace_bytes, (hipStream_t)stream});
+}
+
+TT_EXPORT size_t tt_score_topk_screened_i8_stats_offset(int B, int64_t N, int d, int k)
+{
+    (void)d;
+    return splan_query(B, N, k, &SPlan::i8stats_off, 0);
+}
+
+TT_EXPORT int tt_score_topk_screened_i8_eligible(int B, int64_t N, int d, int k)
+{
+    return B > 0 && N > 0 && d == 256 && k > 0 && k <= 64 && N < (int64_t)INT_MAX - 64 && make_splan(B, N, k).i8 ? 1 : 0;
+}
+
+TT_EXPORT int tt_index_build_i8(const void *D16, int64_t N, int d, const float *stats16, void *D8, float *stats8, tt_stream_t stream)
+{
+    if (N < 0 || d != 256)
+        return tt_fail(TT_ERR_BAD_SHAPE, "tt_index_build_i8: N=%lld d=%d", (long long)N, d);
+    if (!stats16 || !stats8 || (N > 0 && (!D16 || !D8)))
+        return tt_fail(TT_ERR_BAD_SHAPE, "tt_index_build_i8: null pointer");
+    hipStream_t st = (hipStream_t)stream;
+    TT_RC_CHECK(tt_zero_async(stats8, 3 * sizeof(float), st));
+    if (N == 0)
+        return TT_OK;
+    const int64_t want_blocks = (N + 3) / 4;
+    hipLaunchKernelGGL(build_i8_kernel, dim3((unsigned)(want_blocks > 8192 ? 8192 : want_blocks)), dim3(256), 0, st,
+                       (const _Float16 *)D16, N, stats16, (signed char *)D8, (unsigned *)stats8);
+    TT_LAUNCH_CHECK();
+    return TT_OK;
+}
+
 TT_EXPORT int tt_score_topk_screened_seed_f32(const float *Q, int B, int d, const void *D16, int64_t N, int k, int k_seed,
                                               float dmax_norm, int32_t *fallback_flag, float *seed, void *workspace,
                                               size_t workspace_bytes, tt_stream_t stream)
@@ -1791,7 +2473,7 @@
     sp.max_val = out_t;
     sp.dbg_thr = thr;
     hipLaunchKernelGGL(q_image_kernel, dim3(dp.s.rows_pad / 32), dim3(128), 0, s.stream, q.Q, q.B, (h8 *)(ws + dp.s.qimg_off),
-                       (float *)(ws + dp.s.qnorm_off), sp.flag, dp.s.rows_pad / 32, (int *)nullptr, 0, (unsigned *)nullptr);
+                       (float *)(ws + dp.s.qnorm_off), sp.flag, dp.s.rows_pad / 32, (int *)nullptr, 0, (unsigned *)nullptr, QImageI8{});
     TT_LAUNCH_CHECK();
     return launch_screen(dp.s, sp, rows.bf16, s.stream);
 }
@@ -1816,3 +2498,65 @@
     return debug_screen({Q, B, 256, 1, dmax_norm}, {D_bf16, nullptr, true, N, nullptr},
                         {nullptr, workspace, workspace_bytes, (hipStream_t)stream}, thr, form, out_t);
 }
+
+namespace {
+__global__ void debug_gate_kernel(const float2 *__restrict__ qaux, const float *__restrict__ thr, int B, int *__restrict__ out)
+{
+    const int q = blockIdx.x * 256 + threadIdx.x;
+    if (q < B)
+        out[q] = i8_gate_c(thr[q], qaux[q].y, qaux[q].x, true);
+}
+}
+
+namespace {
+struct DbgS8Plan { int rows_pad; size_t qimg_off, qnorm_off, flag_off, img8_off, ws_bytes; };
+DbgS8Plan make_dbg_s8_plan(int B)
+{
+    DbgS8Plan d;
+    d.rows_pad = (B + 31) / 32 * 32;
+    TTWorkspace ws;
+    d.qimg_off = ws.take((size_t)d.rows_pad * 256 * sizeof(_Float16));
+    d.qnorm_off = ws.take((size_t)d.rows_pad * sizeof(float));
+    d.flag_off = ws.take((size_t)(d.rows_pad / 32) * sizeof(int));
+    d.img8_off = ws.take((size_t)d.rows_pad * 256);
+    d.ws_bytes = ws.off;
+    return d;
+}
+}
+
+TT_EXPORT size_t tt_debug_screen_s8_workspace_bytes(int B) { return B > 0 ? make_dbg_s8_plan(B).ws_bytes + (size_t)((B + 31) / 32 * 32) * sizeof(float2) + 256 : 0; }
+
+TT_EXPORT int tt_debug_screen_s8(const float *Q, int B, const void *D8, int64_t N, float dmax_norm, float delta_d, float e8,
+                                 float dn8, const float *thr, int32_t *out_s8, float *out_aux, int32_t *out_gate, void *workspace,
+                                 size_t workspace_bytes, tt_stream_t stream)
+{
+    if (B <= 0 || N <= 0 || N >= (int64_t)INT_MAX - 64)
+        return tt_fail(TT_ERR_BAD_SHAPE, "tt_debug_screen_s8: B=%d N=%lld", B, (long long)N);
+    if (!Q || !D8 || !out_s8 || !out_aux || (thr != nullptr) != (out_gate != nullptr))
+        return tt_fail(TT_ERR_BAD_SHAPE, "tt_debug_screen_s8: null pointer");
+    const DbgS8Plan d = make_dbg_s8_plan(B);
+    const size_t aux_off = (d.ws_bytes + 255) & ~(size_t)255;
+    if (!workspace || workspace_bytes < tt_debug_screen_s8_workspace_bytes(B) || ((uintptr_t)workspace & 255))
+        return tt_fail(TT_ERR_WORKSPACE, "tt_debug_screen_s8: workspace %zu < %zu bytes", workspace_bytes, tt_debug_screen_s8_workspace_bytes(B));
+    char *ws = (char *)workspace;
+    hipStream_t st = (hipStream_t)stream;
+    QImageI8 q8;
+    q8.img8 = (i32x4 *)(ws + d.img8_off);
+    q8.qaux = (float2 *)(ws + aux_off);
+    q8.dd = delta_d;
+    q8.e8 = e8;
+    q8.dn8 = dn8;
+    q8.dmax = dmax_norm;
+    hipLaunchKernelGGL(q_image_kernel, dim3(d.rows_pad / 32), dim3(128), 0, st, Q, B, (h8 *)(ws + d.qimg_off), (float *)(ws + d.qnorm_off),
+                       (int *)(ws + d.flag_off), d.rows_pad / 32, (int *)nullptr, 0, (unsigned *)nullptr, q8);
+    TT_LAUNCH_CHECK();
+    hipLaunchKernelGGL(debug_s8_kernel, dim3((unsigned)((N + 15) / 16), d.rows_pad / 16), dim3(64), 0, st, (const i32x4 *)q8.img8,
+                       (const signed char *)D8, B, (int)N, (int *)out_s8);
+    TT_LAUNCH_CHECK();
+    if (thr) {
+        hipLaunchKernelGGL(debug_gate_kernel, dim3((B + 255) / 256), dim3(256), 0, st, (const float2 *)q8.qaux, thr, B, (int *)out_gate);
+        TT_LAUNCH_CHECK();
+    }
+    TT_HIP_CHECK(hipMemcpyAsync(out_aux, ws + aux_off, (size_t)B * sizeof(float2), hipMemcpyDeviceToDevice, st));
+    return TT_OK;
+}
diff --git a/twotowermlretrieval_amd/index.py b/twotowermlretrieval_amd/index.py
--- a/twotowermlretrieval_amd/index.py
+++ b/twotowermlretrieval_amd/index.py
@@ -1,5 +1,6 @@
 from __future__ import annotations
 
+import math
 from functools import lru_cache
 from typing import Callable, NamedTuple, Optional, Tuple
 
@@ -907,15 +908,34 @@
 SCREEN_MIN_DOCS = 65536
 
 
+SCREEN_I8 = True
+
+
 def _fp16_range_ok(dmax: float, amax: float) -> bool:
     return dmax == dmax and amax < 6.0e4 and dmax < 6.0e4
 
 
 class _Screen:
 
-    def __init__(self, rows: torch.Tensor, filt: torch.Tensor, bf16: bool, dmax_norm: float):
+    def __init__(self, rows: torch.Tensor, filt: torch.Tensor, bf16: bool, dmax_norm: float,
+                 filt8: Optional[torch.Tensor] = None, i8_consts: Tuple[float, float, float] = (0.0, 0.0, 0.0)):
         self.rows, self.filt, self.bf16, self.dmax_norm = rows, filt, bool(bf16), float(dmax_norm)
         self.n = rows.shape[0]
+        self.filt8, self.i8_consts = filt8, tuple(float(x) for x in i8_consts)
+        self.last_gated = False
+
+    @staticmethod
+    def _build_i8(filt: torch.Tensor, stats16: torch.Tensor):
+        N = filt.shape[0]
+        filt8 = torch.empty((N, 256), dtype=torch.int8, device=filt.device)
+        stats8 = torch.zeros(3, dtype=torch.float32, device=filt.device)
+        with torch.cuda.device(filt.device):
+            _lib.check(_lib.lib().tt_index_build_i8(filt.data_ptr(), N, 256, stats16.data_ptr(), filt8.data_ptr(),
+                                                    stats8.data_ptr(), _stream(filt)))
+        e8, dn8, dd = (float(x) for x in stats8.tolist())
+        if not (dd > 0.0 and math.isfinite(dd) and math.isfinite(e8) and math.isfinite(dn8)):
+            return None, (0.0, 0.0, 0.0)
+        return filt8, (dd, e8, dn8)
 
     @classmethod
     def for_f32(cls, docs: torch.Tensor) -> Optional["_Screen"]:
@@ -931,7 +951,13 @@
         with torch.cuda.device(docs.device):
             _lib.check(_lib.lib().tt_index_build_f16(rows.data_ptr(), N, 256, filt.data_ptr(), stats.data_ptr(), _stream(docs)))
         dmax, amax = (float(x) for x in stats.tolist())
-        return cls(rows, filt, False, dmax) if _fp16_range_ok(dmax, amax) else None
+        if not _fp16_range_ok(dmax, amax):
+            return None
+        filt8, consts = (None, (0.0, 0.0, 0.0))
+        with torch.cuda.device(docs.device):
+            if SCREEN_I8 and any(_lib.lib().tt_score_topk_screened_i8_eligible(B, N, 256, 10) for B in (512, 1024, 4096)):
+                filt8, consts = cls._build_i8(filt, stats)
+        return cls(rows, filt, False, dmax, filt8, consts)
 
     @classmethod
     def for_bf16(cls, docs: torch.Tensor) -> Optional["_Screen"]:
@@ -967,6 +993,14 @@
     def run(self, q: torch.Tensor, k: int, idx_offset: int, vals: torch.Tensor, idx: torch.Tensor, flags: torch.Tensor,
             ws: torch.Tensor, seed: Optional[torch.Tensor] = None, prof_events=None, keep: Optional[torch.Tensor] = None) -> None:
         B, d = q.shape
+        self.last_gated = False
+        if self.filt8 is not None and seed is None and keep is None and not self.bf16:
+            self.last_gated = bool(_lib.lib().tt_score_topk_screened_i8_eligible(B, self.n, 256, k))
+            _lib.check(_lib.lib().tt_score_topk_screened_i8_f32(
+                q.data_ptr(), B, d, self.rows.data_ptr(), self.filt.data_ptr(), self.filt8.data_ptr(), self.n, k, self.dmax_norm,
+                *self.i8_consts, idx_offset, vals.data_ptr(), idx.data_ptr(), flags.data_ptr(), ws.data_ptr(), ws.numel(),
+                prof_events, _stream(q)))
+            return
         fn = getattr(_lib.lib(), _screened_fn("whole" if seed is None else "seeded", self.bf16, keep is not None))
         corpus = (self.rows.data_ptr(),) if self.bf16 else (self.rows.data_ptr(), self.filt.data_ptr())
         mask = () if keep is None else (keep.data_ptr(),)
@@ -1029,6 +1063,15 @@
         with torch.cuda.device(self.docs.device):
             off = _lib.lib().tt_score_topk_screened_stats_offset(B, self.docs.shape[0], 256, k)
         return ws[off:off + 8 * B].view(torch.int32).view(B, 2).clone()
+
+    def search_stats_i8(self) -> Optional[torch.Tensor]:
+        sc = self._screen
+        if self._last_ws is None or sc is None or not sc.last_gated:
+            return None
+        ws, B, k = self._last_ws
+        with torch.cuda.device(self.docs.device):
+            off = _lib.lib().tt_score_topk_screened_i8_stats_offset(B, self.docs.shape[0], 256, k)
+        return ws[off:off + 20].view(torch.int32).clone()
 
     def search(self, q: torch.Tensor, k: int = 10, _prof_events=None, out=None, _seed_union=None,
                _k_seed: int = 0, _k_list: int = 0, keep: Optional[torch.Tensor] = None,
```

New measurement: 355,200 queries/s (median of 6 runs). 32.4% higher.
